# grayhong/self-diagnosing-gan

Measured on AMD Instinct MI355X. Metric: images/sec (G+D step), higher is better.
Workload: dtype f32

## Files before the change

include/diagan_hip.h:

```cpp
#ifndef DIAGAN_HIP_H
#define DIAGAN_HIP_H
#include <stdint.h>
#ifdef __cplusplus
extern "C" {
#endif

#define DIAGAN_OK 0
#define DIAGAN_EINVAL (-1)
#define DIAGAN_EHIP (-2)
#define DIAGAN_EUNSUP (-3)

const char* diagan_last_error(void);
int diagan_abi_version(void);
const char* diagan_target_arch(void);


int diagan_ldr_scores_f64(const double* rec, int T, int64_t N, int64_t row_stride, double* ldr,
                          double* ldrd, double* ldrv, double* ldrm, const double* t_vals, int n_t,
                          double* conf, double floor_val, double ratio, void* workspace,
                          void* stream);

int diagan_ldr_scores_f32(const float* rec, int T, int64_t N, int64_t row_stride, float* ldr,
                          float* ldrd, float* ldrv, float* ldrm, const float* t_vals, int n_t,
                          float* conf, float floor_val, float ratio, void* workspace, void* stream);

int diagan_logit_scatter(const float* logit, const int64_t* idx, int64_t n, void* rec_row,
                         int64_t N, int out_is_f64, int* oob_counter, void* stream);



int diagan_conv_gemm(const float* x, const float* w, float* y, const float* bias,
                     const float* residual, int res_relu, const float* mask_src, float mask_slope,
                     const float* pro_scale, const float* pro_shift, int pro_mode, float out_scale,
                     const float* scale0, const float* scale1, int scale_split,
                     int B, int Hi, int Wi, int Ci, int Ho, int Wo, int Co, int R, int S, int sy,
                     int dr, int off, int up, int Kp, int tile_cfg, float* splitk_ws, int64_t splitk_ws_floats,
                     float* stat_partials, int pro_group_rows, void* stream);
int diagan_conv_gemm_pick_ksplit(int M, int Co, int Kp, int cfg);

int diagan_conv3x3_co4_supported(int Ci, int Co, int R, int S, int sy, int dr, int off, int up);
int diagan_conv3x3_co4(const float* x, const float* w, float* y, const float* bias, const float* residual,
                       const float* pro_scale, const float* pro_shift, int pro_mode, int B, int H, int W, int Ci,
                       int dr, int off, int Kp, int group_imgs, void* stream);

int diagan_conv3x3_ci4_supported(int Ci, int Co, int R, int S, int sy, int dr, int off, int up);
int diagan_conv3x3_ci4(const float* x, const float* w, float* y, const float* bias, float out_scale, const float* scale0,
                       const float* scale1, int scale_split, int B, int H, int W, int Co, int Kp, void* stream);

int diagan_conv3x3_co4_wgrad_supported(int Ci, int Co, int R, int S, int sy, int dr, int off, int up);
int diagan_conv3x3_co4_wgrad_splits(int B, int H);
int diagan_conv3x3_co4_wgrad(const float* dy, const float* x, float* slab, int64_t slab_stride, int64_t bias_off,
                             const float* pro_scale, const float* pro_shift, int pro_mode, int B, int H, int W,
                             int Ci, int Kp, void* stream);

int diagan_conv_gemm_pick_cfg(int M, int Co, int Kp, int allow_split);
int diagan_conv_gemm_tile_rows(int cfg);
int diagan_conv_gemm_tile_cols(int cfg);
int diagan_conv_wino_supported(int Hi, int Wi, int Ci, int Ho, int Wo, int Co, int R, int S, int sy, int dr, int off,
                               int up);
int diagan_conv_wino_pool_supported(int B, int Hi, int Wi, int Ci, int Ho, int Wo, int Co, int R, int S, int sy, int dr,
                                    int off, int up, int pro_mode, int64_t ws_floats);
int diagan_conv_wino_unpool_supported(int B, int Hi, int Wi, int Ci, int Ho, int Wo, int Co, int R, int S, int sy, int dr,
                                      int off, int up, int64_t ws_floats);
int diagan_conv_gemm_set_wino(int mode);
int diagan_conv_gemm_get_wino(void);
int diagan_conv_gemm_set_wino4(int mode);
int diagan_conv_gemm_set_wino4x(int mode);
int diagan_conv_gemm_get_wino4x(void);
int diagan_conv_gemm_set_splitk_fused(int mode);
int diagan_conv_gemm_set_splitk_tickets(int* buf, int64_t slots);
typedef struct diagan_conv_opts {
  int32_t wino, wino4, wino4x, gemm_x3, gemm_x3b, splitk_fused, force_ksplit, tune;
  int32_t* tickets;
  int64_t ticket_slots;
} diagan_conv_opts;
int diagan_conv_gemm_next_opts(const diagan_conv_opts* opts);
int diagan_conv_gemm_pending_opts(diagan_conv_opts* opts);
int diagan_conv_gemm_last_cfg(void);
int diagan_conv_gemm_set_x3(int mode);
int diagan_conv_gemm_get_x3(void);
int diagan_conv_gemm_set_x3b(int mode);
int diagan_conv_gemm_get_x3b(void);
int diagan_conv_gemm_set_x3_pieces(int n);
int diagan_conv_gemm_get_x3_pieces(void);
int diagan_conv_gemm_x3b_force_form(int form);
int diagan_conv_gemm_out_map(int mul, int offy, int offx, int y0, int y1, int x0, int x1, int OH, int OW);
int diagan_conv_gemm_final_cfg(int B, int Hi, int Wi, int Ci, int Ho, int Wo, int Co, int R, int S, int sy, int dr, int off, int up,
                               int Kp, int allow_split, int64_t ws_floats, int pro_group_rows, int pro_mode, int plain_epilogue,
                               int want_stats);
int diagan_conv_wino4_pool_used(int B, int Ho, int Wo, int Ci, int Co, int64_t ws_floats);
int diagan_conv_wino4_upin_supported(int B, int Hi, int Wi, int Ci, int Ho, int Wo, int Co, int R, int S, int sy, int dr,
                                     int off, int up, int64_t ws_floats, int pro_group_rows);
int diagan_conv_gemm_weights_hint(const float* u, int kind, int flip, float scale);
int diagan_conv_gemm_last_weight_format(int* kind, int* flip, float* scale, int64_t* floats, int64_t* launches);
int64_t diagan_wino_weight_blocks(int Co, int Ci);
int diagan_wino_weights_batched(const void* jobs, int n, int blocks, void* stream);
int diagan_conv_gemm_pick_cfg_geom(int B, int Hi, int Wi, int Ci, int Ho, int Wo, int Co, int R, int S, int sy, int dr,
                                   int off, int up, int Kp, int allow_split, int64_t ws_floats);
int diagan_conv_gemm_pick_cfg_grouped(int B, int Hi, int Wi, int Ci, int Ho, int Wo, int Co, int R, int S, int sy, int dr,
                                      int off, int up, int Kp, int allow_split, int64_t ws_floats, int pro_group_rows);
int diagan_conv_gemm_set_stamp_buffer(unsigned long long* buf, int64_t slots);
int diagan_conv_gemm_tune(int force_ksplit, int flags, int lds_delta_bytes);

int diagan_conv_wgrad(const float* dy, const float* x, float* slab, int splits, int segments, int64_t slab_stride,
                      int64_t bias_off, const float* pro_scale, const float* pro_shift, int pro_mode, int B, int Hi, int Wi, int Ci, int Ho,
                      int Wo, int Co, int R, int S, int sy, int dr, int off, int up, int Kp,
                      void* stream);
int diagan_conv_wgrad_splits(int M, int Co, int Kp);
typedef struct {
  const float* dy;
  const float* x;
  float* slab;
  const float* pro_scale;
  const float* pro_shift;
  int64_t slab_stride, bias_off;
  int32_t splits, segments, pro_mode, B, Hi, Wi, Ci, Ho, Wo, Co, R, S, sy, dr, off, up, Kp, pad_;
} diagan_wgrad_job;
int diagan_conv_wgrad_batched(const diagan_wgrad_job* jobs, int n, void* stream);
int diagan_conv_wgrad_batch_max(void);
int diagan_conv_wgrad_batch_class(int Hi, int Wi, int Ci, int Ho, int Wo, int Co, int R, int S, int sy, int dr, int off, int up,
                                  int Kp, int pro_mode);
int diagan_conv_wgrad_uses_wino(int Hi, int Wi, int Ci, int Ho, int Wo, int Co, int R, int S, int sy, int dr, int off,
                                int up, int Kp);
int diagan_conv_wgrad_splits_geom(int B, int Hi, int Wi, int Ci, int Ho, int Wo, int Co, int R, int S, int sy, int dr,
                                  int off, int up, int Kp);
int diagan_conv_wgrad_uses_x3(int B, int Hi, int Wi, int Ci, int Ho, int Wo, int Co, int R, int S, int sy, int dr, int off,
                              int up, int Kp, int pro_mode, int64_t bias_off);
int diagan_conv_wgrad_set_x3(int on);

typedef struct {
  float* slab[2];
  const float* u[2];
  const float* v[2];
  const float* state[2];
  double* partials[2];
  float* grad;
  const float* W;
  int64_t stride;
  int splits, n_elem, n_w, Kp;
  int nctx, first_block;
} diagan_wgrad_layer;
int diagan_wgrad_finish_batched(const void* table_dev, int n_layers, int64_t total_blocks, int any_sn, void* stream);
int diagan_wgrad_finish_block_elems(int splits);

int diagan_wgrad_reduce(const float* slab, int splits, int64_t n_elem, float* out, int accumulate,
                        const float* w, double* dot_partials, void* stream);


int diagan_sn_power_iter(const float* W, float* u_buffer, float* sigma_buffer, float* u_out,
                         float* v_out, float* state, float* work, int Co, int Kp, float eps,
                         int update_buffers, void* stream);

typedef struct {
  const float* W;
  float* u_buf;
  float* sigma_buf;
  float* u_out;
  float* v_out;
  float* state;
  float* work;
  float* Wf;
  float* Wd;
  int Co, Ci, RS, Kp, Kd, pad;
} diagan_sn_layer;
int diagan_sn_prepare_batched(const void* table_dev, int n_layers, int max_Co, int max_Ci, int max_RS,
                              int max_Kp, float eps, int update_buffers, int write_wd, void* stream);
int diagan_pack_batched(const void* table_dev, int n_layers, int max_Co, int max_Ci, int max_RS, int write_wd,
                        void* stream);

int diagan_pack_weights(const float* W, const float* inv_sigma, float* Wf, float* Wd, int Co, int Ci,
                        int RS, int Kp, int Kd, void* stream);
int diagan_pack_oihw(const float* w, float scale, float* Wf, float* Wd, int Co_src, int Ci_src, int R, int S, int Co, int Ci, int Kp,
                     int Kd, void* stream);
int diagan_unpack_oihw(const float* gWp, float scale, float* gw, int Co_src, int Ci_src, int R, int S, int Ci, int Kp, void* stream);
int diagan_parity_weights(const float* w, float* buf, float* gw, int n, int R, int S, int C, int Kp, const int* kp, const int* off,
                          int adjoint, void* stream);


int diagan_sn_grad_fix(const float* G, const double* dot_partials, int nparts, const float* u,
                       const float* v, const float* state, float* grad, int Co, int Kp,
                       int accumulate, void* stream);


int diagan_nchw_to_nhwc(const float* src, float* dst, int B, int C, int H, int W, int Cp, void* stream);
int diagan_nhwc_to_nchw(const float* src, float* dst, int B, int C, int H, int W, int Cp, void* stream);

int diagan_tanh_fwd(const float* x, float* y, int64_t n, void* stream);
int diagan_tanh_bwd(const float* y, const float* g, float* gx, int64_t n, void* stream);

int64_t diagan_colred_workspace(int64_t M, int C);

int diagan_bn_stats(const float* x, int64_t M, int C, const float* gamma, const float* beta, float eps,
                    float momentum, float* running_mean, float* running_var, int training,
                    float* mean_out, float* invstd_out, float* scale_out, float* shift_out,
                    void* workspace, void* stream);
int diagan_bn_stats_grouped(const float* x, int64_t M, int C, int groups, const float* gamma, const float* beta, float eps,
                            float momentum, float* running_mean, float* running_var, float* mean_out, float* invstd_out,
                            float* scale_out, float* shift_out, void* workspace, void* stream);

int diagan_bn_stats_fused(const float* partials, int tiles, int64_t M, int C, const float* gamma, const float* beta,
                          float eps, float momentum, float* running_mean, float* running_var, float* mean_out,
                          float* invstd_out, float* scale_out, float* shift_out, int groups, double* workspace,
                          int64_t workspace_doubles, void* stream);
int diagan_bn_stats_fused_splits(int tiles, int C, int groups);

int diagan_bn_bwd(const float* g, const float* x, int64_t M, int C, const float* scale, const float* shift,
                  const float* mean, const float* invstd, int batch_stats, int relu, float slope,
                  const float* drop, float drop_scale, float* dgamma, float* dbeta,
                  int accumulate_param_grads, const float* residual, float* dx, float* coef,
                  void* workspace, void* stream);

int diagan_colsum(const float* x, int64_t M, int C, float* out, int accumulate, void* workspace, void* stream);

int diagan_upsample2x(const float* x, float* out, int B, int H, int W, int C, int pro_mode,
                      const float* scale, const float* shift, int group_imgs, void* stream);
int diagan_upsample2x_bwd(const float* g, float* out, int B, int H, int W, int C, const float* residual,
                          void* stream);

int diagan_avgpool2(const float* x, float* out, int B, int H, int W, int C, const float* residual, int relu_in,
                    void* stream);
int diagan_boxsum2(const float* x, float* out, int B, int H, int W, int C, int relu_in, void* stream);
int diagan_avgpool2_bwd(const float* g, float* out, int B, int H, int W, int C, const float* residual,
                        void* stream);

int diagan_head_fwd(const float* x, const float* w, const float* inv_sigma, const float* inv_sigma1, int split_b,
                    const float* bias, float* pooled, float* logit, int B, int HW, int C, void* stream);
int diagan_head_bwd(const float* dlogit, const float* w, const float* inv_sigma, const float* inv_sigma1, int split_b,
                    const float* x, const float* pooled, float* gx, float* G, double* dot, float* dbias,
                    int accumulate_bias, int B, int HW, int C, void* stream);

int diagan_act_fwd(const float* x, const float* scale, const float* shift, float slope, const float* drop, float drop_scale,
                   float* out, int64_t M, int C, void* stream);
int diagan_act_bwd(const float* g, const float* x, float slope, const float* drop, float drop_scale, float* out, int64_t n,
                   void* stream);
int diagan_linear1_fwd(const float* x, const float* w, const float* bias, float* logit, int B, int C, void* stream);
int diagan_linear1_wgrad(const float* dlogit, const float* x, float* dw, float* dbias, int B, int C, void* stream);
int diagan_linear1_bwd_input(const float* dlogit, const float* w, float* gx, int B, int C, void* stream);

int diagan_add(const float* a, const float* b, float* out, int64_t n, void* stream);


int diagan_loss_dis(const float* out_real, int n_real, const float* out_fake, int n_fake, int loss_type,
                    int gold, float* d_real, float* d_fake, float* out3, void* stream);
int diagan_loss_gen(const float* out_fake, int n, int k, int loss_type, float* d_fake, float* out1, void* stream);

int diagan_adam_step(float* p, const float* g, float* m, float* v, int64_t n, float lr, float beta1,
                     float beta2, float eps, float bias_correction1, float bias_correction2_sqrt, float grad_scale,
                     void* stream);
int diagan_adam_step_dev(float* p, const float* g, float* m, float* v, int64_t n, const float* hyper8, void* stream);

typedef struct diagan_ctx diagan_ctx;
int diagan_comm_unique_id(void* id128);
int diagan_ctx_create(diagan_ctx** out, const void* id128, int rank, int world, int device);
int diagan_ctx_destroy(diagan_ctx* ctx);
int diagan_ctx_rank(const diagan_ctx* ctx);
int diagan_ctx_world(const diagan_ctx* ctx);
int diagan_allreduce_grads(diagan_ctx* ctx, float* slab, int64_t n, void* stream);
int diagan_allgather_logits(diagan_ctx* ctx, const void* send, void* recv, int64_t n_per_rank, int elem_bytes,
                            void* stream);


int diagan_fused_bias_act(const float* x, const float* bias, const float* refer, float* out, int64_t n,
                          int64_t step_b, int size_b, int act, int grad, float alpha, float scale, void* stream);

int diagan_styled_bias_act(const float* x, const float* demod, const float* noise, const float* strength,
                           const float* bias, float* out, int B, int P, int C, int noise_per_image, float alpha,
                           float scale, void* stream);

int diagan_rowdot_chunks(int B, int P);
int diagan_rowdot(const float* a, const float* b, float* out, float* workspace, int B, int P, int C, void* stream);
int diagan_styled_bias_act_bwd(const float* gy, const float* y, const float* x, const float* demod, const float* noise,
                               float* gx, float* work_d, float* work_b, float* work_s, int B, int P, int C,
                               int noise_per_image, float alpha, float scale, void* stream);
int diagan_styled_bias_act_bwd_finish(const float* work_d, const float* work_b, const float* work_s, float* gd, float* gb, float* gs, int B,
                                      int P, int C, void* stream);

int diagan_small_linear_fwd(const float* x, const float* W, const float* bias, float* out, int B, int K, int C, float scale, float bias_mul,
                            void* stream);
int diagan_small_linear_bwd(const float* g, const float* x, const float* W, float* gW, float* gbias, float* gx, int B, int K, int C,
                            float scale, float bias_mul, void* stream);
int diagan_demod_fwd(const float* s, const float* w, float* d, float* wsq, int B, int Ci, int Co, int taps, float scale2, float eps,
                     void* stream);
int diagan_demod_bwd(const float* gd, const float* d, const float* s, const float* w, const float* wsq, float* gw, float* gs, int B, int Ci,
                     int Co, int taps, float scale2, void* stream);

int diagan_styled_bias_act_mod(const float* x, const float* demod, const float* noise, const float* strength, const float* bias,
                               const float* post, float* out, float* out_mod, int B, int P, int C, int noise_per_image, float alpha,
                               float scale, void* stream);
int diagan_styled_bias_act_mod_bwd(const float* gy, const float* gmod, const float* post, const float* y, const float* x,
                                   const float* demod, const float* noise, float* gx, float* work_d, float* work_b, float* work_s,
                                   float* work_p, int B, int P, int C, int noise_per_image, float alpha, float scale, void* stream);

int diagan_torgb_fwd(const float* x, const float* s, const float* w, const float* bias, float* out, int B, int P, int C, void* stream);
int diagan_torgb_bwd(const float* gy, const float* x, const float* s, const float* w, float* gx, float* work, float* gs, float* gw, int B,
                     int P, int C, void* stream);
int diagan_fromrgb_fwd(const float* x, const float* w, const float* bias, float* y, int B, int P, int C, float wscale, float alpha,
                       float scale, void* stream);
int diagan_fromrgb_bwd(const float* gy, const float* y, const float* x, const float* w, float* gx, float* work, int B, int P, int C,
                       float wscale, float alpha, float scale, void* stream);
int diagan_bias_act_fir(const float* input, const float* bias, const float* kernel, float* out, int major, int in_h, int in_w, int minor,
                        int kernel_h, int kernel_w, int pad_x0, int pad_x1, int pad_y0, int pad_y1, float alpha, float scale,
                        void* stream);
int diagan_bias_act_gate_bwd(const float* gy, const float* z, const float* bias, float* gx, float* work_b, int B, int P, int C,
                             float alpha, float scale, void* stream);
int diagan_fir_gate_bwd(const float* g, const float* kernel, const float* ref, const float* bias, float* gz, float* work_b, int major,
                        int in_h, int in_w, int minor, int kernel_h, int kernel_w, int pad_x0, int pad_x1, int pad_y0, int pad_y1,
                        float alpha, float scale, void* stream);
int diagan_upfirdn2d_add(const float* input, const float* kernel, const float* addend, float* out, int major, int in_h, int in_w, int minor,
                         int kernel_h, int kernel_w, int up_x, int up_y, int down_x, int down_y, int pad_x0, int pad_x1, int pad_y0,
                         int pad_y1, void* stream);
int diagan_bias_act_add(const float* x, const float* bias, const float* addend, float* out, int64_t n, int C, float alpha, float scale,
                        void* stream);
int diagan_fir_styled_act(const float* input, const float* kernel, float* out, int major, int in_h, int in_w, int minor, int kernel_h,
                          int kernel_w, int pad_x0, int pad_x1, int pad_y0, int pad_y1, const float* demod, const float* noise,
                          const float* strength, const float* bias, const float* post, int noise_per_image, float alpha, float scale,
                          void* stream);


int diagan_upfirdn2d(const float* input, const float* kernel, float* out, int major, int in_h, int in_w, int minor,
                     int kernel_h, int kernel_w, int up_x, int up_y, int down_x, int down_y, int pad_x0, int pad_x1,
                     int pad_y0, int pad_y1, int* out_h, int* out_w, void* stream);

int diagan_row_sqnorm(const float* x, float* out, int N, int D, int ld, void* stream);
int diagan_kth_smallest_rows(const float* T, const float* row_add, int rows, int cols, int ld, int k, float* out,
                             void* stream);
int diagan_any_lt_rows(const float* T, const float* row_add, const float* thr_col, const float* thr_row, int rows,
                       int cols, int ld, float* out, void* stream);
int diagan_any_lt_cols(const float* T, const float* row_add, const float* thr_col, const float* thr_row, int rows,
                       int cols, int ld, float* out, void* stream);

int diagan_gemm_f64(const double* A, const double* B, double* C, int M, int N, int K, int lda, int ldb, int ldc, int trans_a,
                    double alpha, double beta, double diag, double* trace_part, void* stream);
int diagan_gemm_f64_tile(void);
int diagan_sum_f64(const double* x, int64_t n, int square, double* out, void* stream);
int diagan_trace_f64(const double* S, int D, int ld, double* out, void* stream);
int diagan_sym_f64(double* S, int D, int ld, double scale, void* stream);
int diagan_scale_diag_f64(const double* src, double* dst, int D, int ld, double alpha, double d, void* stream);
int diagan_fid_term(const double* mu1, const double* mu2, const double* S1, const double* S2, int D, int ld, double* out,
                    void* stream);
int diagan_feat_colsum_chunks(int N);
int diagan_feat_moments(const void* x, int x_f64, int N, int D, int ld, double* mask, double* part, double* count, double* mean,
                        void* stream);
int diagan_feat_center(const void* x, int x_f64, const double* mask, const double* mean, int N, int D, int ld, double* xc, int ldc,
                       void* stream);
int diagan_moments_merge(double* n_run, double* mean_run, double* m2_run, int ld, const double* n_b, const double* mean_b,
                         const double* m2_b, int ldb, int D, void* stream);


int diagan_augment_params(void);
int diagan_augment_workspace(int B, int H, int W, int pad_x1, int pad_x2, int pad_y1, int pad_y2, int backward, int64_t* bytes);
int diagan_augment_forward(const float* img, const double* params, int B, int H, int W, int pad_x1, int pad_x2, int pad_y1,
                           int pad_y2, float* out, void* workspace, void* stream);
int diagan_augment_backward(const float* gout, const double* params, int B, int H, int W, int pad_x1, int pad_x2, int pad_y1,
                            int pad_y2, float* gimg, void* workspace, void* stream);

#ifdef __cplusplus
}
#endif
#endif
```

self-diagnosing-gan_amd/csrc/conv_common.h:

```cpp
#pragma once
#include "common.h"

namespace diagan {

typedef float f32x16 __attribute__((ext_vector_type(16)));
typedef float f32x4 __attribute__((ext_vector_type(4)));

enum ProMode : int {
  PRO_NONE = 0,
  PRO_RELU = 1,
  PRO_AFFINE_RELU = 2,
  PRO_LRELU = 3,
  PRO_AFFINE = 4,
  PRO_BOX = 5,
  PRO_BOX_RELU = 6,
};

struct ConvGeom {
  int B, Hi, Wi, Ci;
  int Ho, Wo, Co;
  int R, S;
  int sy, dr, off, up;
  int K;
  int Kp;
};

__device__ __forceinline__ f32x4 apply_pro(f32x4 v, int mode, const float* __restrict__ scale,
                                           const float* __restrict__ shift, int c) {
  if (mode == PRO_NONE) return v;
  if (mode == PRO_AFFINE_RELU || mode == PRO_AFFINE) {
    const f32x4 sc = *reinterpret_cast<const f32x4*>(scale + c);
    const f32x4 sh = *reinterpret_cast<const f32x4*>(shift + c);
    v = v * sc + sh;
    if (mode == PRO_AFFINE) return v;
  }
  if (mode == PRO_LRELU) {
#pragma unroll
    for (int e = 0; e < 4; ++e) v[e] = v[e] > 0.f ? v[e] : 0.2f * v[e];
    return v;
  }
#pragma unroll
  for (int e = 0; e < 4; ++e) v[e] = fmaxf(v[e], 0.f);
  return v;
}

struct FastDiv {
  unsigned mul, shift, d;
};
static inline FastDiv make_fastdiv(unsigned d) {
  FastDiv f;
  f.d = d;
  if (d == 1) { f.mul = 0; f.shift = 0; return f; }
  unsigned l = 0;
  while ((1u << l) < d) ++l;
  const unsigned long long m = ((1ull << (32 + l)) + d - 1) / d;
  f.mul = (unsigned)(m - (1ull << 32));
  f.shift = l;
  return f;
}
__device__ __forceinline__ f32x4 residual_up2(const float* __restrict__ r, int b, int oy, int ox, int H, int W, int C, int c) {
  const int jy = oy >> 1, jx = ox >> 1;
  const int y0 = (oy & 1) ? jy : max(jy - 1, 0), y1 = (oy & 1) ? min(jy + 1, H - 1) : jy;
  const int x0 = (ox & 1) ? jx : max(jx - 1, 0), x1 = (ox & 1) ? min(jx + 1, W - 1) : jx;
  const float wy0 = (oy & 1) ? 0.75f : 0.25f, wx0 = (ox & 1) ? 0.75f : 0.25f;
  const float wy1 = 1.f - wy0, wx1 = 1.f - wx0;
  const float* base = r + (long)b * H * W * C + c;
  const f32x4 a00 = *reinterpret_cast<const f32x4*>(base + ((long)y0 * W + x0) * C);
  const f32x4 a01 = *reinterpret_cast<const f32x4*>(base + ((long)y0 * W + x1) * C);
  const f32x4 a10 = *reinterpret_cast<const f32x4*>(base + ((long)y1 * W + x0) * C);
  const f32x4 a11 = *reinterpret_cast<const f32x4*>(base + ((long)y1 * W + x1) * C);
  const f32x4 top = wx0 * a00 + wx1 * a01;
  const f32x4 bot = wx0 * a10 + wx1 * a11;
  return wy0 * top + wy1 * bot;
}

__device__ __forceinline__ unsigned fdiv(unsigned n, const FastDiv& f) {
  if (f.d == 1) return n;
  const unsigned t = __umulhi(n, f.mul);
  return (t + ((n - t) >> 1)) >> (f.shift - 1);
}

struct OutMap {
  int mul, offy, offx, y0, y1, x0, x1, OH, OW;
};

struct ConvGemmArgs {
  const float* x;
  const float* w;
  float* y;
  const float* bias;
  const float* residual;
  const float* mask_src;
  const float* pro_scale;
  const float* pro_shift;
  int pro_group_rows;
  float mask_slope;
  float out_scale;
  const float* scale0;
  const float* scale1;
  int scale_split;
  float* stat_partials;
  float* slab;
  int* tickets;
  int ksplit;
  int res_relu;
  int res_up;
  int pro_mode;
  int M;
  ConvGeom g;
  FastDiv dWo, dHo;
  unsigned long long* stamps;
  int tune;
};

struct WgradArgs {
  const float* dy;
  const float* x;
  float* slab;
  const float* pro_scale;
  const float* pro_shift;
  int pro_mode;
  int M;
  int steps_per_split;
  int seg_steps;
  int splits_per_seg;
  long slab_stride;
  long bias_off;
  ConvGeom g;
  FastDiv dWo, dHo;
  int adv_b, adv_y, adv_x;
  int lgW, lgHW;
  int tiles;
  int same;
};

constexpr int WG_BATCH_MAX = 8;
struct WgradBatchArgs {
  int n;
  int blk0[WG_BATCH_MAX];
  int cnt[WG_BATCH_MAX];
  WgradArgs a[WG_BATCH_MAX];
};

constexpr int WT_LDS_F4 = 9 * 8 * 65;
__device__ __forceinline__ bool wino_stage_taps(const float* __restrict__ w, int co0, int c0, int Co, int Ci, int Kp, int flip,
                                                f32x4* __restrict__ sg, f32x4 (&g)[3][3]) {
  const int tid = threadIdx.x;
  {
    const int col = tid >> 3, q = tid & 7;
    const bool ok = co0 + col < Co && c0 + q * 4 < Ci;
    const float* src = w + (long)(co0 + col) * Kp + c0 + q * 4;
    f32x4 v[9];
#pragma unroll
    for (int t = 0; t < 9; ++t) v[t] = ok ? *reinterpret_cast<const f32x4*>(src + (flip ? 8 - t : t) * Ci) : f32x4{0.f, 0.f, 0.f, 0.f};
#pragma unroll
    for (int t = 0; t < 9; ++t) sg[(t * 8 + q) * 65 + col] = v[t];
  }
  __syncthreads();
  const int col = tid & 63, q = tid >> 6;
#pragma unroll
  for (int t = 0; t < 9; ++t) g[t / 3][t % 3] = sg[(t * 8 + q) * 65 + col];
  return c0 + q * 4 < Ci;
}

enum WinoKind : int { WK_F2 = 2, WK_F4 = 40, WK_F4_POOL = 41, WK_F4X = 42, WK_F4X_POOL = 43, WK_GX3 = 50 };
struct WinoJob {
  const float* w;
  float* u;
  int Co, Ci, Kp, kind, flip, blk0;
  float scale;
  int pad_;
};
const float* wino_weights_ready(int kind, int flip, float scale, long floats);

__device__ __forceinline__ int xcd_remap(int bid, int nwg) {
  const int q = nwg >> 3, r = nwg & 7, xcd = bid & 7, slot = bid >> 3;
  return (xcd < r ? xcd * (q + 1) : r * (q + 1) + (xcd - r) * q) + slot;
}

}
```

self-diagnosing-gan_amd/csrc/conv_gemm.hip:

```cpp
#include "conv_common.h"
#include <type_traits>
#include <stdlib.h>
#include <string.h>

extern "C" int diagan_conv_gemm_tile_rows(int cfg);
extern "C" int diagan_conv_gemm_tile_cols(int cfg);
extern "C" int diagan_conv_gemm_pick_ksplit(int M, int Co, int Kp, int cfg);
extern "C" int diagan_conv_gemm_pick_cfg_geom(int B, int Hi, int Wi, int Ci, int Ho, int Wo, int Co, int R, int S, int sy,
                                              int dr, int off, int up, int Kp, int allow_split, int64_t ws_floats);
extern "C" int diagan_conv_gemm_pick_cfg_grouped(int B, int Hi, int Wi, int Ci, int Ho, int Wo, int Co, int R, int S, int sy,
                                                 int dr, int off, int up, int Kp, int allow_split, int64_t ws_floats,
                                                 int pro_group_rows);
extern "C" int diagan_conv_wino_supported(int Hi, int Wi, int Ci, int Ho, int Wo, int Co, int R, int S, int sy, int dr,
                                          int off, int up);

namespace diagan {
int launch_gemm_x3(const ConvGemmArgs& a, float* ws, hipStream_t st);
bool gemm_x3_geom_ok(const ConvGemmArgs& a);
long gemm_x3_ws_floats(int Co, int Kp);
int launch_gemm_x3b(const ConvGemmArgs& a, const OutMap& map, float* ws, hipStream_t st);
bool gemm_x3b_geom_ok(const ConvGemmArgs& a);
long gemm_x3b_ws_floats(int Co, int Kp);
void gemm_x3b_force_form(int form);
int launch_wino(ConvGemmArgs a, float* ws, hipStream_t st);
long wino_ws_floats(int Co, int Ci);
int wino_ksplit(int B, int Ho, int Wo, int Ci, int Co, int allow_split, long ws_floats, int min_wgs);
int launch_wino4(ConvGemmArgs a, float* ws, hipStream_t st);
long wino4_ws_floats(int Co, int Ci);
bool wino4_geom_ok(int Ho, int Wo, int Ci);
int wino4_ksplit(int B, int Ho, int Wo, int Ci, int Co, int allow_split, long ws_floats);
bool wino4_pool_ok(int B, int Ho, int Wo, int Ci, int Co, long ws_floats, bool force);
int launch_wino4_pool(ConvGemmArgs a, float* ws, hipStream_t st);
int launch_wino4_unpool(ConvGemmArgs a, float* ws, hipStream_t st);
bool wino4_upin_ok(int B, int Ho, int Wo, int Ci, int Co, long ws_floats, bool force);
int launch_wino_weights_batched(const WinoJob* jobs, int n, int blocks, hipStream_t st);
int launch_wino4_upin(ConvGemmArgs a, float* ws, hipStream_t st);
void wino4_set_x3(int mode);
int wino4_get_x3();
int launch_wino_pool(ConvGemmArgs a, float* ws, hipStream_t st);
int launch_wino_unpool(ConvGemmArgs a, float* ws, hipStream_t st);
int wino_pool_ksplit(int B, int Ho, int Wo, int Ci, int Co, long slab_floats, int min_wgs);


template <int BM, int BN, int WM, int WN, int BK = 32, int PRO = -1, bool STAMP = false, bool FP = false, int KG = 1>
__global__ __launch_bounds__(256 * KG) void conv_gemm_kernel(const ConvGemmArgs a) {
  constexpr int CH = BK / 4;
  constexpr int RP = 256 / CH;
  constexpr int TM = BM / WM / 32, TN = BN / WN / 32;
  constexpr int AJ = BM / RP, BJ = BN / RP;
  auto swz = [](int row, int q) {
    return BK == 64 ? (q ^ (row & 15)) : BK == 32 ? (q ^ ((row >> 1) & 7)) : (q ^ ((row >> 2) & 3));
  };
  static_assert(WM * WN == 4, "4 waves");
  extern __shared__ __attribute__((aligned(16))) float smem_all[];
  constexpr int STAGE_FLOATS = 2 * (BM + BN) * BK;
  const int kg = KG > 1 ? __builtin_amdgcn_readfirstlane((int)threadIdx.x >> 8) : 0;
  float* const smem = smem_all + kg * STAGE_FLOATS;
  float* As = smem;
  float* Bs = smem + 2 * BM * BK;

  unsigned long long st_t[6] = {0, 0, 0, 0, 0, 0}, st_r0 = 0;
  auto stamp = [&](int i) {
    if constexpr (STAMP) {
      __builtin_amdgcn_sched_barrier(0);
      st_t[i] = __builtin_amdgcn_s_memtime();
      __builtin_amdgcn_sched_barrier(0);
    }
  };
  if constexpr (STAMP) st_r0 = __builtin_amdgcn_s_memrealtime();
  if (a.tune & 1) __builtin_amdgcn_s_setprio(3);
  stamp(0);
  const ConvGeom& g = a.g;
  const int pro_mode = PRO >= 0 ? PRO : a.pro_mode;
  const int tid = KG > 1 ? (threadIdx.x & 255) : threadIdx.x, lane = tid & 63, wave = tid >> 6;
  const int wm = wave / WN, wn = wave % WN;
  const int tiles_n = (g.Co + BN - 1) / BN;
  const int nwg = gridDim.x;
  const int tile = xcd_remap(blockIdx.x, nwg);
  const int m0 = (tile / tiles_n) * BM, n0 = (tile % tiles_n) * BN;

  const int lrow = tid / CH, lq = tid % CH;
  const int ush = g.up >> 1, upm = g.up - 1;
  const int pstep = (g.Ci * 4) >> ush;
  int base[AJ];
  unsigned vmask[AJ];
#pragma unroll
  for (int j = 0; j < AJ; ++j) {
    const int m = m0 + lrow + RP * j;
    base[j] = 0;
    vmask[j] = 0;
    if (m < a.M) {
      const unsigned t = fdiv((unsigned)m, a.dWo);
      const int ox = m - (int)t * g.Wo;
      const unsigned b = fdiv(t, a.dHo);
      const int oy = (int)t - (int)b * g.Ho;
      const int iy0 = oy * g.sy + g.off, ix0 = ox * g.sy + g.off;
      base[j] = (int)b * g.Hi * g.Wi * g.Ci * 4 + (iy0 * g.Wi + ix0) * pstep;
      unsigned mk = 0;
      if (g.up == 1) {
        const int ylo = g.dr > 0 ? max(0, -iy0) : max(0, iy0 - g.Hi + 1);
        const int yhi = g.dr > 0 ? min(g.R - 1, g.Hi - 1 - iy0) : min(g.R - 1, iy0);
        const int xlo = g.dr > 0 ? max(0, -ix0) : max(0, ix0 - g.Wi + 1);
        const int xhi = g.dr > 0 ? min(g.S - 1, g.Wi - 1 - ix0) : min(g.S - 1, ix0);
        if (yhi >= ylo) mk |= (2u << yhi) - (1u << ylo);
        if (xhi >= xlo) mk |= ((2u << xhi) - (1u << xlo)) << 16;
      } else {
        for (int r = 0; r < g.R; ++r) {
          const int yn = iy0 + r * g.dr;
          if (yn >= 0 && (yn & upm) == 0 && (yn >> ush) < g.Hi) mk |= 1u << r;
        }
        for (int q = 0; q < g.S; ++q) {
          const int xn = ix0 + q * g.dr;
          if (xn >= 0 && (xn & upm) == 0 && (xn >> ush) < g.Wi) mk |= 0x10000u << q;
        }
      }
      vmask[j] = mk;
    }
  }
  const int nk_all = g.Kp / BK;
  const int k_per = (nk_all + a.ksplit * KG - 1) / (a.ksplit * KG);
  const int k_begin = min((int)(blockIdx.y * KG + kg) * k_per, nk_all), k_end = min(k_begin + k_per, nk_all);
  int kc, kr, ks;
  {
    const int kflat = k_begin * BK + lq * 4, tap = kflat / g.Ci;
    kc = kflat - tap * g.Ci;
    kr = tap / g.S;
    ks = tap - kr * g.S;
  }
  const int rowstep = g.dr * g.Wi * pstep, colstep = g.dr * pstep;

  const __amdgpu_buffer_rsrc_t xsrc = __builtin_amdgcn_make_buffer_rsrc(
      const_cast<float*>(a.x), 0, (int)((unsigned)g.B * g.Hi * g.Wi * g.Ci * 4u), 0x00020000);
  const __amdgpu_buffer_rsrc_t wsrc = __builtin_amdgcn_make_buffer_rsrc(
      const_cast<float*>(a.w), 0, (int)((unsigned)g.Co * g.Kp * 4u), 0x00020000);
  const bool affine = pro_mode == PRO_AFFINE_RELU || pro_mode == PRO_AFFINE;
  const int pro_group_off = a.pro_group_rows > 0 ? (m0 / a.pro_group_rows) * g.Ci : 0;
  unsigned wbase[BJ];
#pragma unroll
  for (int j = 0; j < BJ; ++j) wbase[j] = ((unsigned)(n0 + lrow + RP * j) * g.Kp + lq * 4) * 4u;

  f32x4 ra[AJ], rb[BJ], psc = {1.f, 1.f, 1.f, 1.f}, psh = {0.f, 0.f, 0.f, 0.f};
  unsigned a_ok = 0;

  const bool ut = (g.Ci % BK) == 0;
  int ukr = 0, uks = 0, ukc = 0;
  unsigned avo[AJ], tap_ok = 0;
  auto tap_setup = [&]() {
    const int toff = ukr * rowstep + uks * colstep + lq * 16;
    const int r_ = min(ukr, 15), s_ = 16 + uks;
    tap_ok = 0;
#pragma unroll
    for (int j = 0; j < AJ; ++j) {
      const unsigned okb = (vmask[j] >> r_) & (vmask[j] >> s_) & 1u;
      avo[j] = (unsigned)(base[j] + toff) | ((okb ^ 1u) << 31);
      tap_ok |= okb << j;
    }
  };
  if (ut) {
    const int kflat0 = k_begin * BK, tap0 = kflat0 / g.Ci;
    ukc = kflat0 - tap0 * g.Ci;
    ukr = tap0 / g.S;
    uks = tap0 - ukr * g.S;
    tap_setup();
  }
  const float* const pro_sc_lane = a.pro_scale ? a.pro_scale + pro_group_off + lq * 4 : nullptr;
  const float* const pro_sh_lane = a.pro_shift ? a.pro_shift + pro_group_off + lq * 4 : nullptr;

  int tapoff = 0, krs = 0, kss = 0;
  auto load_piece = [&](int kk, int p, auto utc) {
    if constexpr (decltype(utc)::value) {
      if (p == 0) {
        a_ok = tap_ok;
        if (affine) {
          psc = *reinterpret_cast<const f32x4*>(pro_sc_lane + ukc);
          psh = *reinterpret_cast<const f32x4*>(pro_sh_lane + ukc);
        }
      }
      if (p < AJ) {
        ra[p] = __builtin_bit_cast(f32x4, __builtin_amdgcn_raw_buffer_load_b128(xsrc, avo[p], ukc * 4, 0));
      } else {
        rb[p - AJ] = __builtin_bit_cast(f32x4, __builtin_amdgcn_raw_buffer_load_b128(wsrc, wbase[p - AJ], kk * (BK * 4), 0));
      }
      if (p == AJ + BJ - 1) {
        ukc += BK;
        if (ukc >= g.Ci) {
          ukc = 0;
          if (++uks == g.S) {
            uks = 0;
            ++ukr;
          }
          tap_setup();
        }
      }
      return;
    }
    if (p == 0) {
      tapoff = kr * rowstep + ks * colstep + kc * 4;
      krs = min(kr, 15);
      kss = 16 + ks;
      a_ok = 0;
      if (affine) {
        const int kcs = min(kc, g.Ci - 4);
        psc = *reinterpret_cast<const f32x4*>(a.pro_scale + pro_group_off + kcs);
        psh = *reinterpret_cast<const f32x4*>(a.pro_shift + pro_group_off + kcs);
      }
    }
    if (p < AJ) {
      const int j = p;
      const unsigned okb = (vmask[j] >> krs) & (vmask[j] >> kss) & 1u;
      const unsigned off = (unsigned)(base[j] + tapoff) | ((okb ^ 1u) << 31);
      ra[j] = __builtin_bit_cast(f32x4, __builtin_amdgcn_raw_buffer_load_b128(xsrc, off, 0, 0));
      a_ok |= okb << j;
    } else {
      const int j = p - AJ;
      rb[j] = __builtin_bit_cast(f32x4, __builtin_amdgcn_raw_buffer_load_b128(wsrc, wbase[j] + (unsigned)kk * (BK * 4u), 0, 0));
    }
    if (p == AJ + BJ - 1) {
      kc += BK;
      if (g.Ci >= BK) {
        const bool w = kc >= g.Ci;
        kc -= w ? g.Ci : 0;
        ks += w ? 1 : 0;
        const bool r = ks == g.S;
        ks = r ? 0 : ks;
        kr += r ? 1 : 0;
      } else {
        const int kflat = (kk + 1) * BK + lq * 4, tap = kflat / g.Ci;
        kc = kflat - tap * g.Ci;
        kr = tap / g.S;
        ks = tap - kr * g.S;
      }
    }
  };
  auto load_tiles = [&](int kk) {
    if (ut) {
#pragma unroll
      for (int p = 0; p < AJ + BJ; ++p) load_piece(kk, p, std::true_type{});
    } else {
#pragma unroll
      for (int p = 0; p < AJ + BJ; ++p) load_piece(kk, p, std::false_type{});
    }
  };
  auto store_piece = [&](int buf, int p) {
    if (p < AJ) {
      const int j = p;
      const int row = lrow + RP * j;
      f32x4 v = ra[j];
      if (pro_mode != PRO_NONE) {
        if (affine) v = v * psc + psh;
        if (pro_mode == PRO_LRELU) {
#pragma unroll
          for (int e = 0; e < 4; ++e) v[e] = v[e] > 0.f ? v[e] : 0.2f * v[e];
        } else if (pro_mode != PRO_AFFINE) {
#pragma unroll
          for (int e = 0; e < 4; ++e) v[e] = fmaxf(v[e], 0.f);
        }
        if (affine) {
          const float keep = (float)((a_ok >> j) & 1u);
          v *= keep;
        }
      }
      *reinterpret_cast<f32x4*>(As + buf * BM * BK + row * BK + (swz(row, lq) << 2)) = v;
    } else {
      const int j = p - AJ;
      const int row = lrow + RP * j;
      *reinterpret_cast<f32x4*>(Bs + buf * BN * BK + row * BK + (swz(row, lq) << 2)) = rb[j];
    }
  };
  auto store_tiles = [&](int buf) {
#pragma unroll
    for (int p = 0; p < AJ + BJ; ++p) store_piece(buf, p);
  };

  f32x16 acc[TM][TN];
#pragma unroll
  for (int i = 0; i < TM; ++i)
#pragma unroll
    for (int j = 0; j < TN; ++j)
#pragma unroll
      for (int e = 0; e < 16; ++e) acc[i][j][e] = 0.f;

  const int fi = lane & 31, fh = lane >> 5;
  int fao[BK / 8], fbo[BK / 8];
#pragma unroll
  for (int u = 0; u < BK / 8; ++u) {
    const int ra_ = wm * (TM * 32) + fi, rb_ = wn * (TN * 32) + fi;
    fao[u] = ra_ * BK + (swz(ra_, 2 * u + fh) << 2);
    fbo[u] = 2 * BM * BK + rb_ * BK + (swz(rb_, 2 * u + fh) << 2);
  }
  const int sto = lrow * BK + (swz(lrow, lq) << 2);

  stamp(1);
  if (k_begin < k_end) {
    load_tiles(k_begin);
    store_tiles(0);
  }
  __syncthreads();

  constexpr int NE = (BK / 8) * 4, NP = AJ + BJ;
  constexpr int PPE = (2 * NP + NE - 1) / NE;
  constexpr int LE = (NP + PPE - 1) / PPE;
  static_assert(2 * LE <= NE, "load and store pieces of a tile must not share an e-step");
  auto kstep = [&](int kk, auto has_next) {
    const int cur = (kk - k_begin) & 1;
    const float* Ac = As + cur * BM * BK;
    const float* Bc = Bs + cur * BN * BK;
    f32x4 fa[2][TM], fb[2][TN];
    auto read_frags = [&](int slot, int u) {
      const int q = 2 * u + fh;
#pragma unroll
      for (int i = 0; i < TM; ++i) {
        const int row = wm * (TM * 32) + i * 32 + fi;
        fa[slot][i] = *reinterpret_cast<const f32x4*>(Ac + row * BK + (swz(row, q) << 2));
      }
#pragma unroll
      for (int j = 0; j < TN; ++j) {
        const int row = wn * (TN * 32) + j * 32 + fi;
        fb[slot][j] = *reinterpret_cast<const f32x4*>(Bc + row * BK + (swz(row, q) << 2));
      }
    };
    if constexpr (FP) read_frags(0, 0);
#pragma unroll
    for (int u = 0; u < BK / 8; ++u) {
      const int fs = FP ? (u & 1) : 0;
      if constexpr (FP) {
        if (u + 1 < BK / 8) read_frags((u + 1) & 1, u + 1);
      } else {
        read_frags(0, u);
      }
#pragma unroll
      for (int e = 0; e < 4; ++e) {
        const int es = u * 4 + e;
        if (decltype(has_next)::value && es < LE) {
#pragma unroll
          for (int pp = 0; pp < PPE; ++pp)
            if (es * PPE + pp < NP) load_piece(kk + 1, es * PPE + pp, std::false_type{});
        }
        if (decltype(has_next)::value && es >= NE - LE) {
          __builtin_amdgcn_sched_barrier(0);
#pragma unroll
          for (int pp = 0; pp < PPE; ++pp)
// ... 281 lines not shown
}
static thread_local OutMap g_map_next = {0, 0, 0, 0, 0, 0, 0, 0, 0};
struct CallOpts {
  int wino, wino4, wino4x, gemm_x3, gemm_x3b, splitk_fused, force_ksplit, tune;
  int* tickets;
  long ticket_slots;
};
static const CallOpts kNoOpts = {-1, -1, -1, -1, -1, -1, 0, -1, nullptr, 0};
static thread_local CallOpts g_opts_next = kNoOpts, g_opts_now = kNoOpts;
static thread_local int g_last_cfg = 0;
int call_opt_wino4x() { return g_opts_now.wino4x; }
static int sel_wino() {
  static const int env = getenv("DIAGAN_WINO") ? atoi(getenv("DIAGAN_WINO")) : 1;
  return g_opts_now.wino >= 0 ? g_opts_now.wino : (g_wino >= 0 ? g_wino : env);
}
static int sel_wino4() { return g_opts_now.wino4 >= 0 ? g_opts_now.wino4 : g_wino4; }
static int sel_force_ksplit() { return g_opts_now.force_ksplit > 0 ? g_opts_now.force_ksplit : g_force_ksplit; }
static bool gemm_x3_on() {
  static const int env = getenv("DIAGAN_GEMM_X3") ? atoi(getenv("DIAGAN_GEMM_X3")) : 1;
  return (g_opts_now.gemm_x3 >= 0 ? g_opts_now.gemm_x3 : (g_gemm_x3 >= 0 ? g_gemm_x3 : env)) != 0;
}
static bool gemm_x3b_on() {
  static const int env = getenv("DIAGAN_GEMM_X3B") ? atoi(getenv("DIAGAN_GEMM_X3B")) : 1;
  return (g_opts_now.gemm_x3b >= 0 ? g_opts_now.gemm_x3b : (g_gemm_x3b >= 0 ? g_gemm_x3b : env)) != 0;
}
static bool x3b_takes(const ConvGemmArgs& a, int cfg, int64_t ws_floats) {
  if (!gemm_x3b_on() || !(cfg == 1 || cfg == 3 || cfg == 5 || cfg == 7 || cfg == 8)) return false;
  const ConvGeom& g = a.g;
  return gemm_x3b_geom_ok(a) && g.Kp >= 128 && g.Co >= 64 && (long)cdiv(a.M, 128) * cdiv(g.Co, 128) >= x3b_min_tiles() &&
         (double)a.M * g.Co * g.Kp >= 4e9 && gemm_x3b_ws_floats(g.Co, g.Kp) <= ws_floats;
}
static int g_splitk_fused = -1;
static int* g_tickets = nullptr;
static long g_ticket_slots = 0;
static int* splitk_tickets(long tiles) {
  static const int env = getenv("DIAGAN_SPLITK_FUSED") ? atoi(getenv("DIAGAN_SPLITK_FUSED")) : 0;
  if (!(g_opts_now.splitk_fused >= 0 ? g_opts_now.splitk_fused : (g_splitk_fused >= 0 ? g_splitk_fused : env))) return nullptr;
  if (g_opts_now.tickets) return tiles <= g_opts_now.ticket_slots ? g_opts_now.tickets : nullptr;
  return (g_tickets && tiles <= g_ticket_slots) ? g_tickets : nullptr;
}

template <int BM, int BN, int WM, int WN, int BK, int PRO, bool STAMP = false, bool FP = false, int KG = 1>
static int launch_one(const ConvGemmArgs& a, hipStream_t st) {
  const int tiles = cdiv(a.M, BM) * cdiv(a.g.Co, BN);
  const size_t lds = (size_t)((long)((size_t)2 * KG * (BM + BN) * BK * sizeof(float)) + g_lds_delta);
  auto kern = conv_gemm_kernel<BM, BN, WM, WN, BK, PRO, STAMP, FP, KG>;
  static FuncAttrLatch latch;
  DG_LDS(latch, kern, lds);
  hipLaunchKernelGGL(kern, dim3(tiles, a.ksplit), dim3(256 * KG), lds, st, a);
  if (a.ksplit > 1) {
    long blocks = ((long)a.M * (a.g.Co / 4) + 255) / 256;
    if (blocks > 4096) blocks = 4096;
    hipLaunchKernelGGL(splitk_epilogue_kernel, dim3((int)blocks), dim3(256), 0, st, a);
  }
  return check_launch("conv_gemm");
}

template <int BM, int BN, int WM, int WN, int BK = 32, bool SPEC = false, bool FP = false, int KG = 1>
static int launch_cfg(const ConvGemmArgs& a, hipStream_t st) {
  if (a.stamps && KG > 1) return set_err(DIAGAN_EUNSUP, "conv_gemm: no stamped build of the two-group kernel");
  if (a.stamps) {
    if (a.pro_mode == PRO_NONE) return launch_one<BM, BN, WM, WN, BK, PRO_NONE, true, FP>(a, st);
    if (a.pro_mode == PRO_RELU) return launch_one<BM, BN, WM, WN, BK, PRO_RELU, true, FP>(a, st);
    return set_err(DIAGAN_EUNSUP, "conv_gemm: the stamped diagnostic kernels exist for prologue modes 0 and 1");
  }
  if (SPEC) {
    switch (a.pro_mode) {
      case PRO_NONE: return launch_one<BM, BN, WM, WN, BK, SPEC ? PRO_NONE : -1, false, FP, KG>(a, st);
      case PRO_RELU: return launch_one<BM, BN, WM, WN, BK, SPEC ? PRO_RELU : -1, false, FP, KG>(a, st);
      case PRO_AFFINE_RELU: return launch_one<BM, BN, WM, WN, BK, SPEC ? PRO_AFFINE_RELU : -1, false, FP, KG>(a, st);
      case PRO_LRELU: return launch_one<BM, BN, WM, WN, BK, SPEC ? PRO_LRELU : -1, false, FP, KG>(a, st);
      default: return launch_one<BM, BN, WM, WN, BK, SPEC ? PRO_AFFINE : -1, false, FP, KG>(a, st);
    }
  }
  return launch_one<BM, BN, WM, WN, BK, -1, false, FP, KG>(a, st);
}

}

using namespace diagan;

static bool split128_enabled() {
  static const bool on = getenv("DIAGAN_SPLIT128") && atoi(getenv("DIAGAN_SPLIT128")) > 0;
  return on;
}

DIAGAN_API int diagan_conv_gemm_pick_cfg(int M, int Co, int Kp, int allow_split) {
  const int small = 7;
  if (Kp <= 256) return small;
  const long t128 = (long)cdiv(M, 128) * cdiv(Co, 128), t64 = (long)cdiv(M, 64) * cdiv(Co, 64);
  if (split128_enabled() && allow_split && (Co & 127) == 0 && t128 <= 256 && diagan_conv_gemm_pick_ksplit(M, Co, Kp, 1) > 1) return 1;
  if (Co <= 64 && Kp >= 256) return M >= 65536 ? 5 : (M >= 32768 ? 8 : 7);
  const long s128 = 256 * 2, s64 = 256 * 4;
  const double q128 = (double)t128 / (double)(cdiv(t128, s128) * s128);
  const double q64 = (double)t64 / (double)(cdiv(t64, s64) * s64);
  const double waste128 = (double)M * Co / ((double)t128 * 128 * 128);
  const double waste64 = (double)M * Co / ((double)t64 * 64 * 64);
  const double bias = 1.08;
  if (bias * q128 * waste128 > q64 * waste64) return 1;
  static const int kg2 = getenv("DIAGAN_KG2") ? atoi(getenv("DIAGAN_KG2")) : 1;
  if (kg2 && t64 <= 256 && Kp >= 16 * 32 && diagan_conv_gemm_pick_ksplit(M, Co, Kp, small) == 1) return 14;
  return small;
}

DIAGAN_API int diagan_conv_gemm_pick_ksplit(int M, int Co, int Kp, int cfg) {
  static const int env_forced = getenv("DIAGAN_KSPLIT") ? atoi(getenv("DIAGAN_KSPLIT")) : 0;
  const int forced = sel_force_ksplit() > 0 ? sel_force_ksplit() : env_forced;
  if (forced > 0 && !(Co & 3)) return forced < Kp / 64 ? forced : (Kp / 64 > 0 ? Kp / 64 : 1);
  if (Co & 3) return 1;
  const int nk = Kp / 32;
  if (cfg == 1) {
    if (!split128_enabled()) return 1;
    const long t128 = (long)cdiv(M, 128) * cdiv(Co, 128);
    if (t128 > 256 || nk < 64) return 1;
    int s = t128 <= 128 ? 4 : 2;
    while (s > 1 && nk / s < 16) --s;
    return s;
  }
  if (cfg != 3 && cfg != 7) return 1;
  const long tiles = (long)cdiv(M, 64) * cdiv(Co, 64);
  if (nk < 16) return 1;
  if (tiles <= 320) {
    if (nk < 64) return 1;
    int s = nk / 24;
    return s > 4 ? 4 : s;
  }
  if (tiles > 512) return 1;
  long sp = 1024 / tiles;
  if (sp > nk / 8) sp = nk / 8;
  return sp < 2 ? 1 : (int)sp;
}

const float* diagan::wino_weights_ready(int kind, int flip, float scale, long floats) {
  g_fmt_last = WinoFormat{nullptr, kind, flip, scale, floats};
  if (g_hint_now.u && g_hint_now.kind == kind && g_hint_now.flip == flip && g_hint_now.scale == scale) return g_hint_now.u;
  ++g_weight_launches;
  return nullptr;
}

DIAGAN_API int diagan_conv_gemm_weights_hint(const float* u, int kind, int flip, float scale) {
  g_hint_next = WinoFormat{u, kind, flip, scale, 0};
  return DIAGAN_OK;
}
DIAGAN_API int diagan_conv_gemm_last_weight_format(int* kind, int* flip, float* scale, int64_t* floats, int64_t* launches) {
  if (kind) *kind = g_fmt_last.kind;
  if (flip) *flip = g_fmt_last.flip;
  if (scale) *scale = g_fmt_last.scale;
  if (floats) *floats = g_fmt_last.floats;
  if (launches) *launches = g_weight_launches;
  return DIAGAN_OK;
}
DIAGAN_API int64_t diagan_wino_weight_blocks(int Co, int Ci) { return (int64_t)cdiv(Ci, 32) * cdiv(Co, 64); }
DIAGAN_API int diagan_wino_weights_batched(const void* jobs, int n, int blocks, void* stream) {
  DG_REQUIRE(jobs && n > 0 && blocks > 0, "wino_weights_batched: bad job table");
  return launch_wino_weights_batched((const WinoJob*)jobs, n, blocks, (hipStream_t)stream);
}

DIAGAN_API int diagan_conv_gemm(const float* x, const float* w, float* y, const float* bias,
                                const float* residual, int res_relu, const float* mask_src, float mask_slope,
                                const float* pro_scale, const float* pro_shift, int pro_mode,
                                float out_scale, const float* scale0, const float* scale1, int scale_split,
                                int B, int Hi, int Wi, int Ci, int Ho, int Wo, int Co,
                                int R, int S, int sy, int dr, int off, int up, int Kp, int tile_cfg,
                                float* splitk_ws, int64_t splitk_ws_floats, float* stat_partials, int pro_group_rows,
                                void* stream) {
  g_hint_now = g_hint_next;
  g_hint_next = WinoFormat{nullptr, 0, 0, 0.f, 0};
  g_fmt_last = WinoFormat{nullptr, 0, 0, 0.f, 0};
  const OutMap map = g_map_next;
  g_map_next = OutMap{0, 0, 0, 0, 0, 0, 0, 0, 0};
  struct OptsScope {
    OptsScope() { g_opts_now = g_opts_next; g_opts_next = kNoOpts; }
    ~OptsScope() { g_opts_now = kNoOpts; }
  } opts_scope;
  g_last_cfg = 0;
  DG_REQUIRE(x && w && y, "conv_gemm: null tensor");
  DG_REQUIRE(B > 0 && Hi > 0 && Wi > 0 && Ho > 0 && Wo > 0 && Co > 0 && R > 0 && S > 0, "conv_gemm: bad dims");
  DG_REQUIRE(Ci > 0 && (Ci & 3) == 0, "conv_gemm: Ci=%d must be a positive multiple of 4 (pad the tensor)", Ci);
  DG_REQUIRE(up == 1 || up == 2, "conv_gemm: up=%d unsupported (1 or 2)", up);
  DG_REQUIRE(dr == 1 || dr == -1, "conv_gemm: dr must be +-1");
  DG_REQUIRE(R <= 15 && S <= 15, "conv_gemm: filter %dx%d larger than 15x15", R, S);
  DG_REQUIRE(Kp % 32 == 0 && Kp >= R * S * Ci, "conv_gemm: Kp=%d must be a multiple of 32 and >= R*S*Ci=%d", Kp, R * S * Ci);
  DG_REQUIRE(pro_mode >= 0 && pro_mode <= 4, "conv_gemm: bad pro_mode %d", pro_mode);
  DG_REQUIRE(!(pro_mode == PRO_AFFINE_RELU || pro_mode == PRO_AFFINE) || (pro_scale && pro_shift),
             "conv_gemm: affine prologue needs scale/shift");
  DG_REQUIRE((long)B * Ho * Wo * Co * 4 < (1L << 31) && (long)B * Hi * Wi * Ci * 4 < (1L << 31) &&
                 (long)Co * Kp * 4 < (1L << 31),
             "conv_gemm: tensors must be smaller than 2 GiB (32-bit buffer offsets)");
  ConvGemmArgs a;
  a.x = x; a.w = w; a.y = y; a.bias = bias; a.residual = residual; a.mask_src = mask_src;
  a.pro_scale = pro_scale; a.pro_shift = pro_shift; a.mask_slope = mask_slope; a.out_scale = out_scale;
  a.scale0 = scale0; a.scale1 = scale1; a.scale_split = scale_split;
  DG_REQUIRE(!scale0 || scale1, "conv_gemm: scale0 and scale1 must be given together");
  DG_REQUIRE(!(stat_partials && mask_src), "conv_gemm: stat_partials (forward statistics) and mask_src (backward mask) are exclusive");
  a.pro_mode = pro_mode; a.M = B * Ho * Wo; a.res_relu = res_relu & 1; a.res_up = (res_relu & 2) ? 1 : (res_relu & 4) ? 2 : 0;
  DG_REQUIRE((res_relu & ~7) == 0 && (res_relu & 6) != 6, "conv_gemm: res_relu=%d (bit 0: relu(residual), bit 1: half-resolution residual, "
             "up-sampled; bit 2: half-resolution residual, un-pooled)", res_relu);
  DG_REQUIRE(a.res_up != 1 || (residual && !(Ho & 1) && !(Wo & 1) && !mask_src && !a.res_relu),
             "conv_gemm: a half-resolution residual needs the tensor, even Ho / Wo, no backward mask and no ReLU on it");
  DG_REQUIRE(a.res_up != 2 || (residual && !(Ho & 1) && !(Wo & 1) && !a.res_relu && !stat_partials),
             "conv_gemm: an un-pooled half-resolution residual needs the tensor, even Ho / Wo, no ReLU on it, no statistics");
  a.g = ConvGeom{B, Hi, Wi, Ci, Ho, Wo, Co, R, S, sy, dr, off, up, R * S * Ci, Kp};
  a.dWo = make_fastdiv((unsigned)Wo);
  a.dHo = make_fastdiv((unsigned)Ho);
  a.stat_partials = stat_partials;
  a.pro_group_rows = pro_group_rows;
  hipStream_t st = (hipStream_t)stream;
  int cfg = tile_cfg != 0 ? tile_cfg
                          : diagan_conv_gemm_pick_cfg_grouped(B, Hi, Wi, Ci, Ho, Wo, Co, R, S, sy, dr, off, up, Kp,
                                                              (splitk_ws && !stat_partials) ? 1 : 0,
                                                              splitk_ws ? splitk_ws_floats : 0, pro_group_rows);
  if (tile_cfg == 0 && splitk_ws && x3b_takes(a, cfg, splitk_ws_floats)) cfg = 17;
  g_last_cfg = cfg;
  if (map.mul != 0) {
    DG_REQUIRE(map.mul > 0 && map.OH > 0 && map.OW > 0 && map.y0 >= 0 && map.x0 >= 0 && map.y1 <= Ho && map.x1 <= Wo &&
                   map.offy >= 0 && map.offx >= 0 && (map.y1 <= map.y0 || map.mul * (map.y1 - 1 - map.y0) + map.offy < map.OH) &&
                   (map.x1 <= map.x0 || map.mul * (map.x1 - 1 - map.x0) + map.offx < map.OW) &&
                   (long)B * map.OH * map.OW * Co * 4 < (1L << 31),
               "conv_gemm: output map (mul %d, off %d/%d, window [%d,%d) x [%d,%d), target %d x %d) does not fit", map.mul, map.offy,
               map.offx, map.y0, map.y1, map.x0, map.x1, map.OH, map.OW);
    DG_REQUIRE(cfg == 17, "conv_gemm: an output map is written by the split-operand kernel only (tile_cfg 17; ask "
               "diagan_conv_gemm_final_cfg first)");
  }
  const int bm = diagan_conv_gemm_tile_rows(cfg);
  DG_REQUIRE(bm > 0, "conv_gemm: unknown tile_cfg %d (0 = auto, 1 = 128x128, 3 = 64x64, 5 = 256x64, 7 = 64x64 with fragment "
             "prefetch, 8 = 128x64 with fragment prefetch, 9 = Winograd F(2x2,3x3), 11 / 12 = Winograd + average pool and its data-gradient, 13 = Winograd F(4x4,3x3), 15 = the same on the bilinear x2 of a half-resolution input; 2, 4, 6, 10 were retired)", tile_cfg);
  DG_REQUIRE(pro_group_rows >= 0 && (pro_group_rows == 0 || (pro_group_rows % bm == 0 && a.M % pro_group_rows == 0)),
             "conv_gemm: pro_group_rows=%d must be a multiple of the %d-row tile and divide M=%d", pro_group_rows, bm, a.M);
  a.slab = splitk_ws;
  a.tickets = nullptr;
  a.ksplit = 1;
  a.tune = g_opts_now.tune >= 0 ? g_opts_now.tune : (g_tune_flags >= 0 ? g_tune_flags : kDefaultTune);
  a.stamps = nullptr;
  if (g_stamps) {
    const long wgs = (long)cdiv(a.M, bm) * cdiv(Co, diagan_conv_gemm_tile_cols(cfg)) * 16;
    DG_REQUIRE(wgs <= g_stamp_slots, "conv_gemm: stamp buffer has %ld slots, this launch may need %ld", g_stamp_slots, wgs);
    a.stamps = g_stamps;
  }
  if (splitk_ws && !stat_partials) {
    const int ks = diagan_conv_gemm_pick_ksplit(a.M, Co, Kp, cfg);
    if (ks > 1 && (int64_t)ks * a.M * Co <= splitk_ws_floats) a.ksplit = ks;
  }
  if (cfg == 11) {
    DG_REQUIRE(diagan_conv_wino_supported(Hi, Wi, Ci, Ho, Wo, Co, R, S, sy, dr, off, up) && dr == 1 && Co % 64 == 0 &&
                   (pro_mode == PRO_NONE || pro_mode == PRO_RELU) && !mask_src && !stat_partials && !a.res_up && pro_group_rows == 0,
               "conv_gemm: tile_cfg 11 (Winograd + average pool) needs a forward 3x3 / stride 1 / pad 1 geometry with even H, W, "
               "Ci %% 8 == 0, Co %% 64 == 0, prologue none / ReLU, no mask, statistics or half-resolution residual");
    if (sel_wino4() != 0 && splitk_ws && wino4_pool_ok(B, Ho, Wo, Ci, Co, (long)splitk_ws_floats, sel_wino4() == 2)) {
      a.ksplit = 1;
      return launch_wino4_pool(a, splitk_ws, st);
    }
    const long wfl = wino_ws_floats(Co, Ci);
    DG_REQUIRE(splitk_ws && splitk_ws_floats >= wfl, "conv_gemm: tile_cfg 11 needs %ld floats of workspace for the transformed weights", wfl);
    int ks = wino_pool_ksplit(B, Ho, Wo, Ci, Co, (long)splitk_ws_floats - wfl, 192);
    if (ks < 1) ks = 1;
    a.ksplit = ks;
    a.slab = splitk_ws + wfl;
    int rc = launch_wino_pool(a, splitk_ws, st);
    if (rc == DIAGAN_OK && ks > 1) {
      ConvGemmArgs e = a;
      e.M = B * (Ho >> 1) * (Wo >> 1);
      e.scale_split = a.scale_split >> 2;
      e.out_scale = a.out_scale;
      long blocks = ((long)e.M * (Co / 4) + 255) / 256;
      if (blocks > 4096) blocks = 4096;
      hipLaunchKernelGGL(splitk_epilogue_kernel, dim3((int)blocks), dim3(256), 0, st, e);
      rc = check_launch("conv_wino_pool split-K epilogue");
    }
    return rc;
  }
  if (cfg == 12) {
    DG_REQUIRE(diagan_conv_wino_supported(Hi, Wi, Ci, Ho, Wo, Co, R, S, sy, dr, off, up) && dr == -1 && Co % 64 == 0 &&
                   pro_mode == PRO_NONE && !stat_partials && !a.res_up && pro_group_rows == 0,
               "conv_gemm: tile_cfg 12 (data-gradient through an average pool, Winograd) needs the data-gradient geometry of a "
               "3x3 / stride 1 / pad 1 layer with even H, W, Ci %% 8 == 0, Co %% 64 == 0, no prologue, statistics or half-resolution residual");
    if (sel_wino4() != 0 && splitk_ws && wino4_pool_ok(B, Ho, Wo, Ci, Co, (long)splitk_ws_floats, sel_wino4() == 2)) {
      a.ksplit = 1;
      return launch_wino4_unpool(a, splitk_ws, st);
    }
    const long wfl = wino_ws_floats(Co, Ci);
    DG_REQUIRE(splitk_ws && splitk_ws_floats >= wfl, "conv_gemm: tile_cfg 12 needs %ld floats of workspace for the transformed weights", wfl);
    long slab_tiles = ((long)splitk_ws_floats - wfl) / 4;
    int ks = wino_pool_ksplit(B, Ho, Wo, Ci, Co, slab_tiles, 192);
    if (ks < 1) ks = 1;
    a.ksplit = ks;
    a.slab = splitk_ws + wfl;
    int rc = launch_wino_unpool(a, splitk_ws, st);
    if (rc == DIAGAN_OK && ks > 1) {
      long blocks = ((long)a.M * (Co / 4) + 255) / 256;
      if (blocks > 4096) blocks = 4096;
      hipLaunchKernelGGL(splitk_epilogue_kernel, dim3((int)blocks), dim3(256), 0, st, a);
      rc = check_launch("conv_wino_unpool split-K epilogue");
    }
    return rc;
  }
  if (cfg == 15) {
    DG_REQUIRE(diagan_conv_wino_supported(Hi, Wi, Ci, Ho, Wo, Co, R, S, sy, dr, off, up) && dr == 1 && wino4_geom_ok(Ho, Wo, Ci) &&
                   !mask_src && (pro_group_rows == 0 || pro_group_rows % 512 == 0),
               "conv_gemm: tile_cfg 15 (Winograd F(4x4,3x3) on an up-sampled input) needs a forward 3x3 / stride 1 / pad 1 geometry, "
               "H and W multiples of 4, Ci %% 8 == 0, no backward mask, prologue groups of whole 512-row tiles");
    const long wfl = wino4_ws_floats(Co, Ci);
    DG_REQUIRE(splitk_ws && splitk_ws_floats >= wfl, "conv_gemm: tile_cfg 15 needs %ld floats of workspace for the transformed weights", wfl);
    a.ksplit = 1;
    return launch_wino4_upin(a, splitk_ws, st);
  }
  if (cfg == 13) {
    DG_REQUIRE(diagan_conv_wino_supported(Hi, Wi, Ci, Ho, Wo, Co, R, S, sy, dr, off, up) && wino4_geom_ok(Ho, Wo, Ci),
               "conv_gemm: tile_cfg 13 (Winograd F(4x4,3x3)) needs a 3x3 / stride 1 / pad 1 geometry, H and W multiples of 4, Ci %% 8 == 0");
    const long wfl = wino4_ws_floats(Co, Ci);
    DG_REQUIRE(splitk_ws && splitk_ws_floats >= wfl, "conv_gemm: tile_cfg 13 needs %ld floats of workspace for the transformed weights", wfl);
    int ks = 1;
    if (tile_cfg == 0 && !stat_partials) {
      ks = wino4_ksplit(B, Ho, Wo, Ci, Co, 1, (long)splitk_ws_floats);
      if (ks < 1) ks = 1;
    } else if (sel_force_ksplit() > 1 && !stat_partials && wfl + (long)sel_force_ksplit() * a.M * Co <= splitk_ws_floats && Ci / 8 / sel_force_ksplit() >= 1) {
      ks = sel_force_ksplit();
    }
    a.ksplit = ks;
    a.slab = splitk_ws + wfl;
    int rc = launch_wino4(a, splitk_ws, st);
    if (rc == DIAGAN_OK && ks > 1) {
      long blocks = ((long)a.M * (Co / 4) + 255) / 256;
      if (blocks > 4096) blocks = 4096;
      hipLaunchKernelGGL(splitk_epilogue_kernel, dim3((int)blocks), dim3(256), 0, st, a);
      rc = check_launch("conv_wino4 split-K epilogue");
    }
    return rc;
  }
  if (cfg == 9) {
    DG_REQUIRE(diagan_conv_wino_supported(Hi, Wi, Ci, Ho, Wo, Co, R, S, sy, dr, off, up),
               "conv_gemm: tile_cfg 9 (Winograd F(2x2,3x3)) needs a 3x3 / stride 1 / pad 1 geometry, even H and W, Ci %% 8 == 0");
    DG_REQUIRE(splitk_ws && splitk_ws_floats >= wino_ws_floats(Co, Ci),
               "conv_gemm: tile_cfg 9 needs %ld floats of workspace for the transformed weights", wino_ws_floats(Co, Ci));
    const long wfl = wino_ws_floats(Co, Ci);
    int ks = 1;
    if (tile_cfg == 0 && !stat_partials) {
      ks = wino_ksplit(B, Ho, Wo, Ci, Co, 1, (long)splitk_ws_floats, 192);
      if (ks < 1) ks = 1;
    } else if (sel_force_ksplit() > 1 && !stat_partials && wfl + (long)sel_force_ksplit() * a.M * Co <= splitk_ws_floats &&
               Ci / 16 / sel_force_ksplit() >= 1) {
      ks = sel_force_ksplit();
    }
    a.ksplit = ks;
    a.slab = splitk_ws + wfl;
    if (ks > 1) a.tickets = splitk_tickets((long)cdiv(a.M / 4, 64) * cdiv(Co, 64));
    int rc = launch_wino(a, splitk_ws, st);
    if (rc == DIAGAN_OK && ks > 1 && !a.tickets) {
      long blocks = ((long)a.M * (Co / 4) + 255) / 256;
      if (blocks > 4096) blocks = 4096;
      hipLaunchKernelGGL(splitk_epilogue_kernel, dim3((int)blocks), dim3(256), 0, st, a);
      rc = check_launch("conv_wino split-K epilogue");
    }
    return rc;
  }
  DG_REQUIRE(!a.res_up, "conv_gemm: a half-resolution residual is added by the Winograd kernel only (tile_cfg 9; ask "
             "diagan_conv_gemm_pick_cfg_geom first)");
  if (cfg == 16 || (cfg == 14 && tile_cfg == 0 && R == 3 && S == 3 && gemm_x3_on() && gemm_x3_geom_ok(a) && splitk_ws &&
                    gemm_x3_ws_floats(Co, Kp) <= splitk_ws_floats)) {
    DG_REQUIRE(gemm_x3_geom_ok(a) && splitk_ws && gemm_x3_ws_floats(Co, Kp) <= splitk_ws_floats,
               "conv_gemm: tile_cfg 16 (split-operand implicit GEMM) needs stride 1, no up-sampling, Ci %% 32 == 0, an even number of "
               "32-channel K-steps, Kp == R*S*Ci, prologue none / ReLU, no statistics, and %ld floats of workspace", gemm_x3_ws_floats(Co, Kp));
    a.ksplit = 1;
    g_last_cfg = 16;
    return launch_gemm_x3(a, splitk_ws, st);
  }
  if (cfg == 17) {
    DG_REQUIRE(gemm_x3b_geom_ok(a) && splitk_ws && gemm_x3b_ws_floats(Co, Kp) <= splitk_ws_floats,
               "conv_gemm: tile_cfg 17 (split-operand implicit GEMM, 128 x 128 tiles) needs a gather without up-sampling, Ci %% 32 == 0, "
               "Kp == R*S*Ci, prologue none / ReLU / leaky ReLU, a plain epilogue (out_scale, bias, residual) and %ld floats of workspace",
               gemm_x3b_ws_floats(Co, Kp));
    a.ksplit = 1;
    return launch_gemm_x3b(a, map, splitk_ws, st);
  }
  switch (cfg) {
    case 1: return launch_cfg<128, 128, 2, 2, 32, true>(a, st);
    case 3: return launch_cfg<64, 64, 2, 2, 32, true>(a, st);
    case 5: return launch_cfg<256, 64, 4, 1, 32, true>(a, st);
    case 7: return launch_cfg<64, 64, 2, 2, 32, true, true>(a, st);
    case 8: return launch_cfg<128, 64, 2, 2, 32, true, true>(a, st);
    case 14: return launch_cfg<64, 64, 2, 2, 32, true, true, 2>(a, st);
    default: return set_err(DIAGAN_EINVAL, "conv_gemm: unknown tile_cfg %d", tile_cfg);
  }
}

DIAGAN_API int diagan_conv_gemm_tile_rows(int cfg) {
  switch (cfg) { case 1: case 8: case 17: return 128; case 3: case 7: case 14: case 16: return 64; case 5: case 9: case 11: case 12: return 256; case 13: case 15: return 512; default: return 0; }
}
DIAGAN_API int diagan_conv_gemm_tile_cols(int cfg) {
  switch (cfg) { case 1: case 11: case 12: case 17: return 128; case 3: case 5: case 7: case 8: case 9: case 13: case 14: case 15: case 16: return 64; default: return 0; }
}

DIAGAN_API int diagan_conv_wino_supported(int Hi, int Wi, int Ci, int Ho, int Wo, int Co, int R, int S, int sy, int dr,
                                          int off, int up) {
  return R == 3 && S == 3 && sy == 1 && up == 1 && ((dr == 1 && off == -1) || (dr == -1 && off == 1)) && Hi == Ho &&
         Wi == Wo && !(Ho & 1) && !(Wo & 1) && (Ci & 7) == 0 && (Co & 3) == 0;
}

DIAGAN_API int diagan_conv_wino_pool_supported(int B, int Hi, int Wi, int Ci, int Ho, int Wo, int Co, int R, int S, int sy,
                                               int dr, int off, int up, int pro_mode, int64_t ws_floats) {
  static const int pool_env = getenv("DIAGAN_WINO_POOL") ? atoi(getenv("DIAGAN_WINO_POOL")) : 1;
  const int wino = sel_wino();
  if (!wino || !pool_env || dr != 1 || Co % 64 != 0 || Ci < 16 || !(pro_mode == PRO_NONE || pro_mode == PRO_RELU)) return 0;
  if (!diagan_conv_wino_supported(Hi, Wi, Ci, Ho, Wo, Co, R, S, sy, dr, off, up)) return 0;
  const long wfl = wino_ws_floats(Co, Ci);
  if (ws_floats < wfl) return 0;
  return wino_pool_ksplit(B, Ho, Wo, Ci, Co, (long)ws_floats - wfl, 192) > 0 ? 1 : 0;
}

DIAGAN_API int diagan_conv_wino_unpool_supported(int B, int Hi, int Wi, int Ci, int Ho, int Wo, int Co, int R, int S, int sy,
                                                 int dr, int off, int up, int64_t ws_floats) {
  static const int pool_env = getenv("DIAGAN_WINO_POOL") ? atoi(getenv("DIAGAN_WINO_POOL")) : 1;
  const int wino = sel_wino();
  if (!wino || !pool_env || dr != -1 || Co % 64 != 0 || Ci < 16) return 0;
  if (!diagan_conv_wino_supported(Hi, Wi, Ci, Ho, Wo, Co, R, S, sy, dr, off, up)) return 0;
  const long wfl = wino_ws_floats(Co, Ci);
  if (ws_floats < wfl) return 0;
  return wino_pool_ksplit(B, Ho, Wo, Ci, Co, ((long)ws_floats - wfl) / 4, 192) > 0 ? 1 : 0;
}

static int pick_cfg_geom_impl(int B, int Hi, int Wi, int Ci, int Ho, int Wo, int Co, int R, int S, int sy, int dr, int off,
                              int up, int Kp, int allow_split, int64_t ws_floats, bool allow_w4);
DIAGAN_API int diagan_conv_gemm_pick_cfg_geom(int B, int Hi, int Wi, int Ci, int Ho, int Wo, int Co, int R, int S, int sy,
                                              int dr, int off, int up, int Kp, int allow_split, int64_t ws_floats) {
  return pick_cfg_geom_impl(B, Hi, Wi, Ci, Ho, Wo, Co, R, S, sy, dr, off, up, Kp, allow_split, ws_floats, true);
}
static int pick_cfg_geom_impl(int B, int Hi, int Wi, int Ci, int Ho, int Wo, int Co, int R, int S, int sy, int dr, int off,
                              int up, int Kp, int allow_split, int64_t ws_floats, bool allow_w4) {
  const int wino = sel_wino();
  static const int min_wgs = getenv("DIAGAN_WINO_MIN_WGS") ? atoi(getenv("DIAGAN_WINO_MIN_WGS")) : 192;
  if (wino && diagan_conv_wino_supported(Hi, Wi, Ci, Ho, Wo, Co, R, S, sy, dr, off, up) &&
      ws_floats >= wino_ws_floats(Co, Ci) && Ci >= 16) {
    static const int wsplit = getenv("DIAGAN_WINO_SPLIT") ? atoi(getenv("DIAGAN_WINO_SPLIT")) : 1;
    static const int w4_env = getenv("DIAGAN_WINO4") ? atoi(getenv("DIAGAN_WINO4")) : 1;
    static const int w4_min_ci = getenv("DIAGAN_WINO4_MIN_CI") ? atoi(getenv("DIAGAN_WINO4_MIN_CI")) : 64;
    if (allow_w4 && w4_env && sel_wino4() != 0 && wino4_geom_ok(Ho, Wo, Ci) && Ci >= w4_min_ci && ws_floats >= wino4_ws_floats(Co, Ci) &&
        wino4_ksplit(B, Ho, Wo, Ci, Co, wsplit ? allow_split : 0, (long)ws_floats) > 0)
      return 13;
    if (wino_ksplit(B, Ho, Wo, Ci, Co, wsplit ? allow_split : 0, (long)ws_floats, min_wgs) > 0) return 9;
  }
  return diagan_conv_gemm_pick_cfg(B * Ho * Wo, Co, Kp, allow_split);
}

DIAGAN_API int diagan_conv_gemm_pick_cfg_grouped(int B, int Hi, int Wi, int Ci, int Ho, int Wo, int Co, int R, int S, int sy,
                                                 int dr, int off, int up, int Kp, int allow_split, int64_t ws_floats,
                                                 int pro_group_rows) {
  int cfg = diagan_conv_gemm_pick_cfg_geom(B, Hi, Wi, Ci, Ho, Wo, Co, R, S, sy, dr, off, up, Kp, allow_split, ws_floats);
  if (cfg == 13 && pro_group_rows > 0 && pro_group_rows % 512 != 0)
    cfg = pick_cfg_geom_impl(B, Hi, Wi, Ci, Ho, Wo, Co, R, S, sy, dr, off, up, Kp, allow_split, ws_floats, false);
  if (pro_group_rows > 0 && pro_group_rows % diagan_conv_gemm_tile_rows(cfg) != 0) {
    cfg = diagan_conv_gemm_pick_cfg(B * Ho * Wo, Co, Kp, allow_split);
    if (pro_group_rows % diagan_conv_gemm_tile_rows(cfg) != 0) cfg = 3;
  }
  return cfg;
}

DIAGAN_API int diagan_conv_gemm_get_wino(void) { return g_wino; }
DIAGAN_API int diagan_conv_gemm_set_wino(int mode) {
  DG_REQUIRE(mode >= -1 && mode <= 1, "set_wino: -1, 0 or 1");
  g_wino = mode;
  return DIAGAN_OK;
}

DIAGAN_API int diagan_conv_wino4_pool_used(int B, int Ho, int Wo, int Ci, int Co, int64_t ws_floats) {
  return sel_wino4() != 0 && wino4_pool_ok(B, Ho, Wo, Ci, Co, (long)ws_floats, sel_wino4() == 2) ? 1 : 0;
}

DIAGAN_API int diagan_conv_wino4_upin_supported(int B, int Hi, int Wi, int Ci, int Ho, int Wo, int Co, int R, int S, int sy, int dr,
                                                int off, int up, int64_t ws_floats, int pro_group_rows) {
  const int wino = sel_wino();
  if (!wino || sel_wino4() == 0 || dr != 1 || !diagan_conv_wino_supported(Hi, Wi, Ci, Ho, Wo, Co, R, S, sy, dr, off, up)) return 0;
  if (pro_group_rows > 0 && pro_group_rows % 512 != 0) return 0;
  return wino4_upin_ok(B, Ho, Wo, Ci, Co, (long)ws_floats, sel_wino4() == 2) ? 1 : 0;
}

DIAGAN_API int diagan_conv_gemm_set_wino4(int mode) {
  DG_REQUIRE(mode >= -1 && mode <= 2, "set_wino4: -1, 0, 1 or 2 (2: also the pooled launches of any size -- tests)");
  g_wino4 = mode;
  return DIAGAN_OK;
}

DIAGAN_API int diagan_conv_gemm_set_wino4x(int mode) {
  DG_REQUIRE(mode >= -1 && mode <= 1, "set_wino4x: -1, 0 or 1");
  wino4_set_x3(mode);
  return DIAGAN_OK;
}
DIAGAN_API int diagan_conv_gemm_get_wino4x(void) { return wino4_get_x3(); }
DIAGAN_API int diagan_conv_gemm_set_x3(int mode) {
  DG_REQUIRE(mode >= -1 && mode <= 1, "set_x3: -1, 0 or 1");
  g_gemm_x3 = mode;
  return DIAGAN_OK;
}
DIAGAN_API int diagan_conv_gemm_get_x3(void) { return gemm_x3_on() ? 1 : 0; }
DIAGAN_API int diagan_conv_gemm_set_x3b(int mode) {
  DG_REQUIRE(mode >= -1 && mode <= 1, "set_x3b: -1, 0 or 1");
  g_gemm_x3b = mode;
  return DIAGAN_OK;
}
DIAGAN_API int diagan_conv_gemm_get_x3b(void) { return gemm_x3b_on() ? 1 : 0; }
namespace diagan { void x3_set_pieces(int n); int x3_pieces(); }
DIAGAN_API int diagan_conv_gemm_set_x3_pieces(int n) {
  diagan::x3_set_pieces(n);
  return DIAGAN_OK;
}
DIAGAN_API int diagan_conv_gemm_get_x3_pieces(void) { return diagan::x3_pieces(); }
DIAGAN_API int diagan_conv_gemm_x3b_force_form(int form) {
  DG_REQUIRE(form >= 0 && form <= 2, "x3b_force_form: 0, 1 or 2");
  gemm_x3b_force_form(form);
  return DIAGAN_OK;
}
DIAGAN_API int diagan_conv_gemm_out_map(int mul, int offy, int offx, int y0, int y1, int x0, int x1, int OH, int OW) {
  g_map_next = OutMap{mul, offy, offx, y0, y1, x0, x1, OH, OW};
  return DIAGAN_OK;
}
DIAGAN_API int diagan_conv_gemm_final_cfg(int B, int Hi, int Wi, int Ci, int Ho, int Wo, int Co, int R, int S, int sy, int dr,
                                          int off, int up, int Kp, int allow_split, int64_t ws_floats, int pro_group_rows,
                                          int pro_mode, int plain_epilogue, int want_stats) {
  struct PendingScope {
    CallOpts saved;
    PendingScope() : saved(g_opts_now) { g_opts_now = g_opts_next; }
    ~PendingScope() { g_opts_now = saved; }
  } pending_scope;
  int cfg = diagan_conv_gemm_pick_cfg_grouped(B, Hi, Wi, Ci, Ho, Wo, Co, R, S, sy, dr, off, up, Kp, allow_split, ws_floats,
                                              pro_group_rows);
  ConvGemmArgs a = {};
  a.pro_mode = pro_mode;
  a.M = B * Ho * Wo;
  a.g = ConvGeom{B, Hi, Wi, Ci, Ho, Wo, Co, R, S, sy, dr, off, up, R * S * Ci, Kp};
  a.pro_group_rows = pro_group_rows;
  static float dummy;
  a.stat_partials = want_stats ? &dummy : nullptr;
  a.mask_src = plain_epilogue ? nullptr : &dummy;
  if (ws_floats > 0 && x3b_takes(a, cfg, ws_floats)) return 17;
  a.mask_src = nullptr;
  if (cfg == 14 && R == 3 && S == 3 && gemm_x3_on() && gemm_x3_geom_ok(a) && ws_floats >= gemm_x3_ws_floats(Co, Kp)) return 16;
  return cfg;
}
DIAGAN_API int diagan_conv_gemm_set_splitk_fused(int mode) {
  DG_REQUIRE(mode >= -1 && mode <= 1, "set_splitk_fused: -1, 0 or 1");
  g_splitk_fused = mode;
  return DIAGAN_OK;
}
DIAGAN_API int diagan_conv_gemm_set_splitk_tickets(int* buf, int64_t slots) {
  DG_REQUIRE((buf && slots > 0) || (!buf && slots == 0), "set_splitk_tickets: a buffer with its slot count, or NULL and 0");
  g_tickets = buf;
  g_ticket_slots = (long)slots;
  return DIAGAN_OK;
}
struct diagan_conv_opts {
  int32_t wino, wino4, wino4x, gemm_x3, gemm_x3b, splitk_fused, force_ksplit, tune;
  int32_t* tickets;
  int64_t ticket_slots;
};
static_assert(sizeof(diagan_conv_opts) == 48, "diagan_conv_opts layout");
DIAGAN_API int diagan_conv_gemm_next_opts(const diagan_conv_opts* o) {
  if (!o) {
    g_opts_next = kNoOpts;
    return DIAGAN_OK;
  }
  DG_REQUIRE(o->wino >= -1 && o->wino <= 1 && o->wino4 >= -1 && o->wino4 <= 2 && o->wino4x >= -1 && o->wino4x <= 1 && o->gemm_x3 >= -1 &&
                 o->gemm_x3 <= 1 && o->gemm_x3b >= -1 && o->gemm_x3b <= 1 && o->splitk_fused >= -1 && o->splitk_fused <= 1 &&
                 o->force_ksplit >= 0 && o->tune >= -1,
             "conv_gemm_next_opts: a field out of range (-1 = process default; force_ksplit 0 = the launch policy)");
  DG_REQUIRE(!o->tickets || o->ticket_slots > 0, "conv_gemm_next_opts: a ticket buffer needs its slot count");
  g_opts_next = CallOpts{o->wino, o->wino4, o->wino4x, o->gemm_x3, o->gemm_x3b, o->splitk_fused, o->force_ksplit, o->tune, o->tickets,
                         (long)o->ticket_slots};
  return DIAGAN_OK;
}
DIAGAN_API int diagan_conv_gemm_pending_opts(diagan_conv_opts* o) {
  DG_REQUIRE(o, "conv_gemm_pending_opts: null");
  const CallOpts& c = g_opts_next;
  *o = diagan_conv_opts{c.wino, c.wino4, c.wino4x, c.gemm_x3, c.gemm_x3b, c.splitk_fused, c.force_ksplit, c.tune, c.tickets,
                        (int64_t)c.ticket_slots};
  return DIAGAN_OK;
}
DIAGAN_API int diagan_conv_gemm_last_cfg(void) { return g_last_cfg; }

DIAGAN_API int diagan_conv_gemm_set_stamp_buffer(unsigned long long* buf, int64_t slots) {
  g_stamps = buf;
  g_stamp_slots = buf ? (long)slots : 0;
  return DIAGAN_OK;
}
DIAGAN_API int diagan_conv_gemm_tune(int force_ksplit, int flags, int lds_delta_bytes) {
  g_force_ksplit = force_ksplit;
  g_tune_flags = flags;
  g_lds_delta = lds_delta_bytes;
  return DIAGAN_OK;
}
```

self-diagnosing-gan_amd/csrc/conv_wino4.hip:

```cpp
#include "conv_common.h"
#include <type_traits>
#include "wino_weights.h"

namespace diagan {

typedef float f32x2 __attribute__((ext_vector_type(2)));

constexpr int W4T = 32;
constexpr int W4N = 64;
constexpr int W4K = 8;
constexpr int W4_PS = 132;
constexpr int W4_VSTAGE = 84 * W4_PS;
constexpr int W4_U = 72 * 256;
#ifndef W4_ROW_AT
#define W4_ROW_AT 3
#endif
#ifndef W4_COL_AT
#define W4_COL_AT 5
#endif
#ifndef W4_DMA_IMM
#define W4_DMA_IMM 1
#endif
#ifndef W4_ULOAD_POOLED
#define W4_ULOAD_POOLED 0
#endif
#ifndef W4_PRO_LDS
#define W4_PRO_LDS 1
#endif
#ifndef W4_ULOAD
#define W4_ULOAD 1
#endif
#ifndef W4_PRIO_B
#define W4_PRIO_B 0
#endif
#ifndef W4_PRIO_ALT
#define W4_PRIO_ALT 0
#endif
#ifndef W4_ROW_AT2
#define W4_ROW_AT2 W4_ROW_AT
#endif
#ifndef W4_COL_AT2
#define W4_COL_AT2 W4_COL_AT
#endif
static_assert((2 * W4_VSTAGE + W4_U) * 4 <= 163840 && 36 * 32 * 32 <= 2 * W4_VSTAGE + W4_U,
              "162 432 bytes of the CU's 163 840; the epilogue's 36 x 32 x 32 floats fit inside");

#ifndef X3_ABL
#define X3_ABL 0
#endif
constexpr int X3_SP = 512;
constexpr int X3_SI = 3 * X3_SP + 16;
constexpr int X3_SJ = 6 * X3_SI + 16;
constexpr int X3_VSTAGE = 6 * X3_SJ;
constexpr int X3_RING = 4 * X3_UNIT;
constexpr int X3_LDS = 2 * X3_VSTAGE + 8 * X3_RING;
static_assert(X3_LDS <= 163840 && 36 * 32 * 32 * 4 <= X3_LDS, "161 088 bytes of the CU's 163 840; the epilogue's exchange image fits inside");
constexpr int x3_gmax(int u) { return (3 * (u + 1)) / 2 + 5; }
constexpr int x3_gneed(int v) { return (3 * (v + 1) + 1) / 2 - 1; }
constexpr int x3_vm_younger(int NS, int ph, bool hn, int NX, int load_at, int row_at, int kind, int s) {
  int seq[256] = {};
  for (int i = 0; i < 256; ++i) seq[i] = -1000;
  int n = 0, seqx = -1000;
  const int t = 4 + ph;
  for (int tt = t - 2; tt <= t; ++tt) {
    const bool h = tt < t ? true : hn;
    const int last = x3_gneed(NS * tt + NS - 1);
    if (tt == t && kind == 0 && s == -1) return n - seq[x3_gneed(NS * tt) - x3_gmax(NS * (t - 2) - 1)] - 1;
    for (int ss = 0; ss < NS; ++ss) {
      const int u = NS * tt + ss;
      if (h && ss == load_at) {
        n += NX;
        seqx = n - 1;
      }
      if (ss + 1 < NS && tt == t && kind == 0 && s == ss) return n - seq[x3_gneed(u + 1) - x3_gmax(NS * (t - 2) - 1)] - 1;
      for (int g = x3_gmax(u - 1) + 1; g <= x3_gmax(u); ++g)
        if (h || g <= last) seq[g - x3_gmax(NS * (t - 2) - 1)] = n++;
      if (ss == row_at && h && tt == t && kind == 1) return n - seqx - 1;
    }
  }
  return -1;
}
template <int I, int N, typename F>
__device__ __forceinline__ void static_for(F&& f) {
  if constexpr (I < N) {
    f(std::integral_constant<int, I>{});
    static_for<I + 1, N>(f);
  }
}
template <int... V>
constexpr int x3_seq_at(std::integer_sequence<int, V...>, int i) {
  const int v[] = {V...};
  return v[i];
}
template <int N>
__device__ __forceinline__ void x3_wait_vm() {
  static_assert(N >= 0 && N < 48, "vmcnt bookkeeping of the X3 schedule");
  asm volatile("s_waitcnt vmcnt(%0)" ::"n"(N) : "memory");
}

template <int MODE>
__global__ __launch_bounds__(512) void wino4_weight_kernel(const float* __restrict__ w, float* __restrict__ ug, int Co, int Ci,
                                                           int Kp, int flip, float wscale) {
  __shared__ f32x4 sg[WT_LDS_F4];
  wino4_weight_body<MODE>(w, ug, Co, Ci, Kp, flip, wscale, blockIdx.x, blockIdx.y, sg);
}
template <int MODE>
__global__ __launch_bounds__(512) void wino4x_weight_kernel(const float* __restrict__ w, float* __restrict__ ug, int Co, int Ci,
                                                            int Kp, int flip, float wscale) {
  __shared__ f32x4 sg[WT_LDS_F4];
  wino4x_weight_body<MODE>(w, ug, Co, Ci, Kp, flip, wscale, blockIdx.x, blockIdx.y, sg);
}

__global__ __launch_bounds__(512) void wino_weights_batched_kernel(const WinoJob* __restrict__ jobs, int n) {
  __shared__ f32x4 sg[WT_LDS_F4];
  int j = 0;
  while (j + 1 < n && (int)blockIdx.x >= jobs[j + 1].blk0) ++j;
  const WinoJob job = jobs[j];
  const int lb = blockIdx.x - job.blk0, nbx = (job.Ci + 31) >> 5;
  if (job.kind == WK_GX3) gx3_weight_job(job.w, job.u, job.Co, job.Kp, lb, nbx * ((job.Co + 63) >> 6));
  else if (job.kind == WK_F4X) wino4x_weight_body<0>(job.w, job.u, job.Co, job.Ci, job.Kp, job.flip, job.scale, lb % nbx, lb / nbx, sg);
  else if (job.kind == WK_F4X_POOL) wino4x_weight_body<1>(job.w, job.u, job.Co, job.Ci, job.Kp, job.flip, job.scale, lb % nbx, lb / nbx, sg);
  else if (job.kind == WK_F4) wino4_weight_body<0>(job.w, job.u, job.Co, job.Ci, job.Kp, job.flip, job.scale, lb % nbx, lb / nbx, sg);
  else if (job.kind == WK_F4_POOL) wino4_weight_body<1>(job.w, job.u, job.Co, job.Ci, job.Kp, job.flip, job.scale, lb % nbx, lb / nbx, sg);
  else wino_weight_body(job.w, job.u, job.Co, job.Ci, job.Kp, job.flip, lb % nbx, lb / nbx, sg);
}

struct W4Consts {
  float m1, p1, m2, p2, m4, p4, m5, p3;
};
__device__ __forceinline__ W4Consts w4_consts() {
  W4Consts k = {-1.f, 1.f, -2.f, 2.f, -4.f, 4.f, -5.f, 3.f};
  asm volatile("" : "+s"(k.m1), "+s"(k.p1), "+s"(k.m2), "+s"(k.p2), "+s"(k.m4), "+s"(k.p4), "+s"(k.m5), "+s"(k.p3));
  return k;
}
template <typename V>
__device__ __forceinline__ void w4_bt(V* d, const W4Consts& k) {
  const V t0 = d[0] * k.p4 + (d[2] * k.m5 + d[4]);
  const V t5 = d[1] * k.p4 + (d[3] * k.m5 + d[5]);
  const V a = d[2] * k.m4 + d[4], b = d[1] * k.m4 + d[3], c = d[2] * k.m1 + d[4], e = d[1] * k.m1 + d[3];
  d[0] = t0;
  d[1] = b * k.p1 + a;
  d[2] = b * k.m1 + a;
  d[3] = e * k.p2 + c;
  d[4] = e * k.m2 + c;
  d[5] = t5;
}

__device__ __forceinline__ void w4_bt_dup(const f32x4* d, f32x4* t, const W4Consts& k) {
  const f32x4 e = d[1] * k.m1 + d[2], f = d[1] * k.m4 + d[2];
  t[0] = d[0] * k.p4 + (d[1] * k.m5 + d[2]);
  t[1] = f * k.p2;
  t[2] = f32x4{0.f, 0.f, 0.f, 0.f};
  t[3] = e * k.p2 + e;
  t[4] = e * k.m1;
  t[5] = d[1] * k.p4 + (d[2] * k.m5 + d[3]);
}

template <typename V>
__device__ __forceinline__ void w4_up(const V* d, V* t, const W4Consts& k, float f0, float f5) {
  t[0] = (d[0] * k.p3 + d[1]) * f0;
  t[1] = d[1] * k.p3 + d[0];
  t[2] = d[1] * k.p3 + d[2];
  t[3] = d[2] * k.p3 + d[1];
  t[4] = d[2] * k.p3 + d[3];
  t[5] = (d[3] * k.p3 + d[2]) * f5;
  w4_bt(t, k);
}

#ifdef DIAGAN_WINO_ABLATE
#define W4_ON(bit) (!(a.tune & (bit)))
#else
#define W4_ON(bit) true
#endif

template <int PRO, int MODE = 0, bool X3 = false, int LEFT = 0>
__global__ __launch_bounds__(512) void conv_wino4_kernel(const ConvGemmArgs a, const float* __restrict__ ug) {
  using MD = W4M<MODE>;
  constexpr int NS = MD::NS, NI = MD::NI;
#ifdef DIAGAN_W4_STAMP
  const unsigned long long t_kernel = __builtin_amdgcn_s_memtime();
#endif
  constexpr bool POOL = MODE == 1, UNPOOL = MODE == 2, UPIN = MODE == 3;
  extern __shared__ __attribute__((aligned(16))) float smem[];
  const ConvGeom& g = a.g;
  const int tid = threadIdx.x, lane = tid & 63, wave = __builtin_amdgcn_readfirstlane(tid >> 6);
  if (W4_PRIO_B > 0 && wave >= 4) __builtin_amdgcn_s_setprio(W4_PRIO_B);
  const int tiles_n = (g.Co + W4N - 1) / W4N;
  const int tile = xcd_remap(blockIdx.x, gridDim.x);
  const int t0 = (tile / tiles_n) * W4T, nb = tile % tiles_n, n0 = nb * W4N;
  const int TW = g.Wo >> 2, TH = g.Ho >> 2;
  const int MT = g.B * TH * TW;
  const int nk = g.Ci / W4K;
  const int k_per = (nk + a.ksplit - 1) / a.ksplit;
  const int k_begin = blockIdx.y * k_per, k_end = min(k_begin + k_per, nk);
  constexpr bool affine = PRO == PRO_AFFINE_RELU || PRO == PRO_AFFINE;

  const int lr = tid & 7, lq = (tid >> 3) & 1, lt = tid >> 4;
  const int ur = lr >> 1, uc = lr & 1;
  const bool ract = UPIN || lr < (UNPOOL ? 4 : 6);
  const bool cact = lr < 6 && !(MD::pooled && lr == 2);
  unsigned off[NI];
  int kbound[NI];
  float ex0 = 1.f, ex5 = 1.f, ey0 = 1.f, ey5 = 1.f;
  {
    const int gt = t0 + lt;
    const bool tv = gt < MT && ract;
    const unsigned q1 = fdiv((unsigned)(tv ? gt : 0), a.dWo);
    const int tx = (tv ? gt : 0) - (int)q1 * TW;
    const unsigned b = fdiv(q1, a.dHo);
    const int ty = (int)q1 - (int)b * TH;
    const bool half = UNPOOL || UPIN;
    const int Hx = half ? g.Hi >> 1 : g.Hi, Wx = half ? g.Wi >> 1 : g.Wi;
    if (UPIN) {
      const int iy = min(max(2 * ty - 1 + ur, 0), Hx - 1);
      const int rowbase = ((int)b * Hx + iy) * Wx;
#pragma unroll
      for (int c = 0; c < NI; ++c) {
        const int ix = min(max(2 * tx - 1 + c, 0), Wx - 1);
        off[c] = tv ? (unsigned)((rowbase + ix) * g.Ci * 4 + lq * 16 + uc * 8) : 0x80000000u;
        kbound[c] = 0x7fffffff;
      }
      ex0 = tx == 0 ? 0.f : 1.f;
      ex5 = tx == TW - 1 ? 0.f : 1.f;
      ey0 = ty == 0 ? 0.f : 1.f;
      ey5 = ty == TH - 1 ? 0.f : 1.f;
    } else {
    const int iy = (UNPOOL ? 2 : 4) * ty - 1 + lr, ix0 = (UNPOOL ? 2 : 4) * tx - 1;
    const bool rv = tv && iy >= 0 && iy < Hx;
    const int rowbase = (((int)b * Hx + iy) * Wx + ix0) * g.Ci * 4 + lq * 16;
#pragma unroll
    for (int c = 0; c < NI; ++c) {
      const bool ok = rv && ix0 + c >= 0 && ix0 + c < Wx;
      off[c] = ok ? (unsigned)(rowbase + c * ((X3_ABL & 128) ? 32 : g.Ci * 4)) : 0x80000000u;
      kbound[c] = ok ? 0x7fffffff : 0;
    }
    }
  }
  typedef int i32x4 __attribute__((ext_vector_type(4)));
  i32x4 xsrc;
  {
    const unsigned long long xb = (unsigned long long)a.x;
    xsrc[0] = __builtin_amdgcn_readfirstlane((int)(unsigned)xb);
    xsrc[1] = __builtin_amdgcn_readfirstlane((int)((unsigned)(xb >> 32) & 0xffffu));
    xsrc[2] = __builtin_amdgcn_readfirstlane((int)((unsigned)g.B * g.Hi * g.Wi * g.Ci * ((UNPOOL || UPIN) ? 1u : 4u)));
    xsrc[3] = 0x00020000;
  }
  const int pro_group_off = a.pro_group_rows > 0 ? ((t0 * 16) / a.pro_group_rows) * g.Ci : 0;
  i32x4 scsrc = xsrc, shsrc = xsrc;
  const unsigned poff = (unsigned)(pro_group_off + lq * 4 + (UPIN ? uc * 2 : 0)) * 4u;
  if (affine) {
    const unsigned long long sb = (unsigned long long)a.pro_scale, hb = (unsigned long long)a.pro_shift;
    scsrc[0] = __builtin_amdgcn_readfirstlane((int)(unsigned)sb);
    scsrc[1] = __builtin_amdgcn_readfirstlane((int)((unsigned)(sb >> 32) & 0xffffu));
    shsrc[0] = __builtin_amdgcn_readfirstlane((int)(unsigned)hb);
    shsrc[1] = __builtin_amdgcn_readfirstlane((int)((unsigned)(hb >> 32) & 0xffffu));
    scsrc[2] = shsrc[2] = 0x7fffffff;
  }
  float* const vrow = smem + (UPIN ? (lq * 42 + ur) * W4_PS + lt * 4 + uc * 2
                                   : (ract ? (lq * 42 + lr) * W4_PS + lt * 4 : (1 << 22)));
  float* const vcol = smem + (cact ? (lq * 42 + 7 * lr) * W4_PS + lt * 4 : (1 << 22));
  char* const sm8 = reinterpret_cast<char*>(smem);
  const unsigned vrow3 = UPIN ? ur * X3_SI + lt * 16 + lq * 8 + uc * X3_SP
                              : (ract ? lr * X3_SI + lt * 16 + lq * 8 : (1u << 24));
  const unsigned vcol3 = cact ? lr * X3_SJ + lt * 16 + lq * 8 : (1u << 24);

  float* const ulds = smem + 2 * W4_VSTAGE;
  const float* ublock = ug + (long)nb * nk * MD::U_FLOATS + ((wave & 3) * 2 + (wave >> 2)) * NS * 256;
  float* const uslot = ulds + wave * NS * 256;

#if W4_DMA_IMM
#define W4_DMA_CASE(u)                                                                                                   \
  case u:                                                                                                                \
    __builtin_amdgcn_global_load_lds((const __attribute__((address_space(1))) void*)(up + 4 * 256),                     \
                                     (__attribute__((address_space(3))) void*)(uslot + 4 * 256), 16, ((u) - 4) * 1024, 0); \
    break;
  f32x4 uprobe = {0.f, 0.f, 0.f, 0.f};
  auto issue_u = [&](int kk, int s) {
    const float* up = ublock + (long)kk * MD::U_FLOATS + lane * 4;
    if (X3_ABL & 512) {
      asm volatile("global_load_dwordx4 %0, %1, off" : "+v"(uprobe) : "v"(up + s * 256) : "memory");
      return;
    }
    switch (s) {
      W4_DMA_CASE(0) W4_DMA_CASE(1) W4_DMA_CASE(2) W4_DMA_CASE(3) W4_DMA_CASE(4) W4_DMA_CASE(5) W4_DMA_CASE(6) W4_DMA_CASE(7)
      default:
        __builtin_amdgcn_global_load_lds((const __attribute__((address_space(1))) void*)(up + s * 256),
                                         (__attribute__((address_space(3))) void*)(uslot + s * 256), 16, 0, 0);
    }
  };
#undef W4_DMA_CASE
#else
  auto issue_u = [&](int kk, int s) {
    const float* up = ublock + (long)kk * MD::U_FLOATS + s * 256 + lane * 4;
    __builtin_amdgcn_global_load_lds((const __attribute__((address_space(1))) void*)up,
                                     (__attribute__((address_space(3))) void*)(uslot + s * 256), 16, 0, 0);
  };
#endif
  const W4Consts kc = w4_consts();
  constexpr bool PRO_LDS = W4_ULOAD && W4_PRO_LDS && !X3 && (!MD::pooled || LEFT > 0) && affine;
  float* const pls = smem + 2 * W4_VSTAGE;
  int x_kk = 0;
  f32x4 ra[6], psc = {1.f, 1.f, 1.f, 1.f}, psh = {0.f, 0.f, 0.f, 0.f};
  f32x2 rb[4], psc2 = {1.f, 1.f}, psh2 = {0.f, 0.f};
#pragma unroll
  for (int c = NI; c < 6; ++c) ra[c] = f32x4{0.f, 0.f, 0.f, 0.f};
  auto issue_x = [&](int kk) __attribute__((always_inline)) {
    const int soff = __builtin_amdgcn_readfirstlane(kk * (W4K * 4));
    x_kk = kk;
    if (UPIN) {
#pragma unroll
      for (int c = 0; c < 4; ++c)
        asm volatile("buffer_load_dwordx2 %0, %1, %2, %3 offen" : "=v"(rb[c]) : "v"(off[c]), "s"(xsrc), "s"(soff) : "memory");
      if (affine && !PRO_LDS) {
        asm volatile("buffer_load_dwordx2 %0, %1, %2, %3 offen" : "=v"(psc2) : "v"(poff), "s"(scsrc), "s"(soff) : "memory");
        asm volatile("buffer_load_dwordx2 %0, %1, %2, %3 offen" : "=v"(psh2) : "v"(poff), "s"(shsrc), "s"(soff) : "memory");
      }
      return;
    }
#pragma unroll
    for (int c = 0; c < NI; ++c)
      asm volatile("buffer_load_dwordx4 %0, %1, %2, %3 offen" : "=v"(ra[c]) : "v"(off[c]), "s"(xsrc), "s"(soff) : "memory");
    if (affine && !PRO_LDS) {
      asm volatile("buffer_load_dwordx4 %0, %1, %2, %3 offen" : "=v"(psc) : "v"(poff), "s"(scsrc), "s"(soff) : "memory");
      asm volatile("buffer_load_dwordx4 %0, %1, %2, %3 offen" : "=v"(psh) : "v"(poff), "s"(shsrc), "s"(soff) : "memory");
    }
  };
#define W4_WAIT_IN(n)                                                                                            \
  case n:                                                                                                        \
    if (UPIN)                                                                                                    \
      asm volatile("s_waitcnt vmcnt(" #n ")"                                                                     \
                   : "+v"(rb[0]), "+v"(rb[1]), "+v"(rb[2]), "+v"(rb[3]), "+v"(psc2), "+v"(psh2)::"memory");        \
    else                                                                                                         \
      asm volatile("s_waitcnt vmcnt(" #n ")"                                                                     \
                   : "+v"(ra[0]), "+v"(ra[1]), "+v"(ra[2]), "+v"(ra[3]), "+v"(ra[4]), "+v"(ra[5]), "+v"(psc), "+v"(psh)::"memory"); \
    break;
  auto wait_inputs = [&](int n) {
    switch (n) {
      W4_WAIT_IN(0) W4_WAIT_IN(1) W4_WAIT_IN(2) W4_WAIT_IN(3) W4_WAIT_IN(4) W4_WAIT_IN(5) W4_WAIT_IN(6) W4_WAIT_IN(7) W4_WAIT_IN(8)
      W4_WAIT_IN(9)
      default:
        if (UPIN) asm volatile("s_waitcnt vmcnt(0)" : "+v"(rb[0]), "+v"(rb[1]), "+v"(rb[2]), "+v"(rb[3]), "+v"(psc2), "+v"(psh2)::"memory");
        else asm volatile("s_waitcnt vmcnt(0)" : "+v"(ra[0]), "+v"(ra[1]), "+v"(ra[2]), "+v"(ra[3]), "+v"(ra[4]), "+v"(ra[5]), "+v"(psc), "+v"(psh)::"memory");
    }
  };
#undef W4_WAIT_IN
  auto row_pass = [&](int stage) __attribute__((always_inline)) {
    if (PRO_LDS) {
      const float* pr = pls + x_kk * W4K + lq * 4 + (UPIN ? uc * 2 : 0);
      if (UPIN) {
        psc2 = *reinterpret_cast<const f32x2*>(pr);
        psh2 = *reinterpret_cast<const f32x2*>(pr + g.Ci);
      } else {
        psc = *reinterpret_cast<const f32x4*>(pr);
        psh = *reinterpret_cast<const f32x4*>(pr + g.Ci);
      }
    }
    if (UPIN) {
#pragma unroll
      for (int c = 0; c < 4; ++c) {
        f32x2 v = rb[c];
        if (affine) v = v * psc2 + psh2;
        if (PRO == PRO_RELU || PRO == PRO_AFFINE_RELU) {
#pragma unroll
          for (int e = 0; e < 2; ++e) v[e] = __int_as_float(max(__float_as_int(v[e]), 0));
        } else if (PRO == PRO_LRELU) {
#pragma unroll
          for (int e = 0; e < 2; ++e) {
            const float q = v[e], q2 = 0.2f * q;
            asm("v_max_f32 %0, %1, %2" : "=v"(v[e]) : "v"(q), "v"(q2));
          }
        }
        rb[c] = v;
      }
      f32x2 t[6];
      w4_up(rb, t, kc, ex0, ex5);
      if (X3) {
        unsigned o = vrow3 + stage * X3_VSTAGE;
#pragma unroll
        for (int j = 0; j < 6; ++j) {
          *reinterpret_cast<f32x2*>(sm8 + o) = t[j];
          o += X3_SJ;
          asm volatile("" : "+v"(o));
        }
        return;
      }
      float* vs = vrow + stage * W4_VSTAGE;
#pragma unroll
      for (int j = 0; j < 6; ++j) *reinterpret_cast<f32x2*>(vs + j * 7 * W4_PS) = t[j];
      return;
    }
#pragma unroll
    for (int c = 0; c < NI; ++c) {
      f32x4 v = ra[c];
      if (PRO != PRO_NONE) {
        if (affine) v = v * psc + psh;
#pragma unroll
        for (int e = 0; e < 4; ++e) {
          const float q = v[e];
          float r;
          if (PRO == PRO_LRELU) {
            const float q2 = 0.2f * q;
            asm("v_max_f32 %0, %1, %2" : "=v"(r) : "v"(q), "v"(q2));
          } else if (PRO == PRO_RELU) {
            r = __int_as_float(max(__float_as_int(q), 0));
          } else if (PRO == PRO_AFFINE_RELU) {
            asm("v_med3_i32 %0, %1, 0, %2" : "=v"(r) : "v"(q), "v"(kbound[c]));
          } else {
            r = kbound[c] ? q : 0.f;
          }
          v[e] = r;
        }
      }
      ra[c] = v;
    }
    f32x4 t[6];
    if (UNPOOL) w4_bt_dup(ra, t, kc);
    else {
#pragma unroll
      for (int c = 0; c < 6; ++c) t[c] = ra[c];
      w4_bt(t, kc);
    }
    if (X3) {
      unsigned o = vrow3 + stage * X3_VSTAGE;
#pragma unroll
// ... 396 lines not shown
  };
  if constexpr (X3) {
    using I0 = std::integral_constant<int, 0>;
    using I1 = std::integral_constant<int, 1>;
    using I2 = std::integral_constant<int, 2>;
    using I3 = std::integral_constant<int, 3>;
    auto kloop3 = [&](auto place) __attribute__((always_inline)) {
      int kk = k_begin;
      for (; kk + 4 < k_end; kk += 4) {
        kstep3(kk, I0{}, std::true_type{}, ugrp, place);
        kstep3(kk + 1, I1{}, std::true_type{}, ugrp, place);
        kstep3(kk + 2, I2{}, std::true_type{}, ugrp, place);
        kstep3(kk + 3, I3{}, std::true_type{}, ugrp, place);
        ugrp += 4 * NS * X3_UNIT;
      }
      if (k_begin < k_end) {
        kstep3(kk, I0{}, std::true_type{}, ugrp, place);
        kstep3(kk + 1, I1{}, std::true_type{}, ugrp, place);
        kstep3(kk + 2, I2{}, std::true_type{}, ugrp, place);
        kstep3(kk + 3, I3{}, std::false_type{}, ugrp, place);
      }
    };
    if (std::is_same<PlA, PlB>::value || wave < 4) kloop3(PlA{});
    else kloop3(PlB{});
  } else if constexpr (ULOAD) {
    using P0 = std::integral_constant<int, 0>;
    using P1 = std::integral_constant<int, 1>;
    using P2 = std::integral_constant<int, 2>;
    if (NS % 3 == 0) {
      for (int kk = k_begin; kk + 1 < k_end; ++kk) kstep_ul(kk, std::true_type{}, P0{});
      if (k_begin < k_end) kstep_ul(k_end - 1, std::false_type{}, P0{});
    } else {
      int kk = k_begin;
      for (; kk + 3 < k_end; kk += 3) {
        kstep_ul(kk, std::true_type{}, P0{});
        kstep_ul(kk + 1, std::true_type{}, P1{});
        kstep_ul(kk + 2, std::true_type{}, P2{});
      }
      if (LEFT == 1) kstep_ul(kk, std::false_type{}, P0{});
      else {
        kstep_ul(kk, std::true_type{}, P0{});
        kstep_ul(kk + 1, std::false_type{}, P1{});
      }
    }
  } else {
  using RowA = std::integral_constant<int, W4_ROW_AT>;
  using ColA = std::integral_constant<int, W4_COL_AT>;
  using RowB = std::integral_constant<int, W4_ROW_AT2>;
  using ColB = std::integral_constant<int, W4_COL_AT2>;
  using PN = std::integral_constant<int, -1>;
  using PA = std::integral_constant<int, (W4_PRIO_ALT > 0) ? 0 : -1>;
  using PB = std::integral_constant<int, (W4_PRIO_ALT > 0) ? 1 : -1>;
  if ((W4_ROW_AT2 == W4_ROW_AT && W4_COL_AT2 == W4_COL_AT && W4_PRIO_ALT == 0) || wave < 4) {
    for (int kk = k_begin; kk + 1 < k_end; ++kk) kstep(kk, std::true_type{}, RowA{}, ColA{}, PA{});
  } else {
    for (int kk = k_begin; kk + 1 < k_end; ++kk) kstep(kk, std::true_type{}, RowB{}, ColB{}, PB{});
  }
  if (W4_PRIO_ALT > 0) __builtin_amdgcn_s_setprio(0);
  if (k_begin < k_end) kstep(k_end - 1, std::false_type{}, RowA{}, ColA{}, PN{});
  }

#ifdef DIAGAN_W4_STAMP
  if (a.stamps && lane == 0) {
    unsigned long long* o = a.stamps + (((size_t)blockIdx.y * gridDim.x + blockIdx.x) * 8 + wave) * 16;
    for (int i = 0; i < 12; ++i) o[i] = tacc[i];
    o[12] = __builtin_amdgcn_s_memtime() - t_entry;
    o[13] = k_end - k_begin;
    o[14] = t_entry - t_kernel;
  }
  const unsigned long long t_epi = __builtin_amdgcn_s_memtime();
#endif
#ifdef DIAGAN_WINO_ABLATE
  if (a.tune & 512) {
    if (acc[0][0] == 123.456f) a.y[0] = acc[1][3] + acc[5][5] + acc[8][7];
    return;
  }
#endif
  if (X3_ABL & 512) {
    asm volatile("s_waitcnt vmcnt(0)" : "+v"(uprobe)::"memory");
    if (uprobe[0] == 123.456f) a.y[0] = uprobe[1];
  }
  const float sc0 = a.scale0 ? a.scale0[0] : a.out_scale, sc1 = a.scale1 ? a.scale1[0] : a.out_scale;
  const int split = a.scale0 ? (POOL ? a.scale_split >> 2 : a.scale_split) : 0x7fffffff;
  const bool raw = a.ksplit > 1;
  const bool hr = !raw && a.residual != nullptr, hm = !raw && a.mask_src != nullptr, hs = !raw && a.stat_partials != nullptr;
  const int Mout = POOL ? a.M >> 2 : a.M;
  float* ydst = raw ? a.slab + (long)blockIdx.y * Mout * g.Co : a.y;
  const float rfloor = a.res_relu ? 0.f : -__builtin_huge_valf();
  const int et = tid >> 4, eq = (tid >> 1) & 7, eh = tid & 1;
  const int gt = t0 + et;
  const bool tv = gt < MT;
  const unsigned q1 = fdiv((unsigned)(tv ? gt : 0), a.dWo);
  const int tx = (tv ? gt : 0) - (int)q1 * TW;
  const unsigned eb = fdiv(q1, a.dHo);
  const int ty = (int)q1 - (int)eb * TH;
  const int Hy = POOL ? g.Ho >> 1 : g.Ho, Wy = POOL ? g.Wo >> 1 : g.Wo;
  const int oy0 = (POOL ? 2 * ty + eh : 4 * ty + 2 * eh), ox0 = (POOL ? 2 : 4) * tx;
  const int prow0 = ((int)eb * Hy + oy0) * Wy + ox0;
  const float scv = (prow0 < split ? sc0 : sc1) * (MD::pooled ? 0.25f : 1.f);
  const int ybytes = (int)((unsigned)Mout * (unsigned)g.Co * 4u);
  const __amdgpu_buffer_rsrc_t ysrc = __builtin_amdgcn_make_buffer_rsrc(ydst, 0, ybytes, 0x00020000);
  const __amdgpu_buffer_rsrc_t rsrc =
      __builtin_amdgcn_make_buffer_rsrc(const_cast<float*>(a.residual), 0, hr && !a.res_up ? ybytes : 0, 0x00020000);
  const __amdgpu_buffer_rsrc_t msrc = __builtin_amdgcn_make_buffer_rsrc(const_cast<float*>(a.mask_src), 0, hm ? ybytes : 0, 0x00020000);
  const int pixb = g.Co * 4, rowb = Wy * pixb;
#ifdef DIAGAN_W4_STAMP
  unsigned eacc[10] = {0, 0, 0, 0, 0, 0, 0, 0, 0, 0};
  unsigned long long elast = t_epi;
  auto etick = [&](int i) {
    const unsigned long long now = __builtin_amdgcn_s_memtime();
    eacc[i] += (unsigned)(now - elast);
    elast = now;
  };
#define W4_ETICK(i) etick(i)
#else
#define W4_ETICK(i)
#endif
  float* ss = smem;
  f32x4 cs1[2] = {{0.f, 0.f, 0.f, 0.f}, {0.f, 0.f, 0.f, 0.f}}, cs2[2] = {{0.f, 0.f, 0.f, 0.f}, {0.f, 0.f, 0.f, 0.f}};
  const f32x4 z4 = {0.f, 0.f, 0.f, 0.f};
  auto xidx = [&](int i, int j) { return MD::pooled ? 5 * (i < 2 ? i : i - 1) + (j < 2 ? j : j - 1) : 6 * i + j; };
#pragma unroll
  for (int p = 0; p < 2; ++p) {
    W4_ETICK(p == 0 ? 0 : 9);
    if (nh == p) {
#pragma unroll
      for (int s = 0; s < NS; ++s) {
        const int fx = MD::pooled ? w4p_start(grp) + s : 6 * (fi0 + s / 3) + fj0 + s % 3;
        if (!MD::pooled || s < w4p_count(grp)) {
#pragma unroll
          for (int e = 0; e < 16; ++e) {
            const int m = 8 * (e >> 2) + 4 * kh + (e & 3);
            ss[(fx * 32 + m) * 32 + fi] = acc[s][e];
          }
        }
      }
    }
#ifdef DIAGAN_W4_STAMP
    asm volatile("s_waitcnt lgkmcnt(0)" ::: "memory");
#endif
    W4_ETICK(1 + 4 * p);
    __syncthreads();
    W4_ETICK(2 + 4 * p);
    const int n = n0 + p * 32 + eq * 4;
    const bool ok = tv && n < g.Co;
    const unsigned voff = ok ? (unsigned)(prow0 * g.Co + n) * 4u : 0x80000000u;
    f32x4 bv = z4;
    if (!raw && a.bias && ok) bv = *reinterpret_cast<const f32x4*>(a.bias + n);
    if (POOL) {
      f32x4 sj[6];
#pragma unroll
      for (int j = 0; j < 6; ++j) {
        if (j == 2) continue;
        f32x4 m[6];
#pragma unroll
        for (int i = 0; i < 6; ++i)
          if (i != 2) m[i] = *reinterpret_cast<const f32x4*>(ss + (xidx(i, j) * 32 + et) * 32 + eq * 4);
        sj[j] = eh ? (2.f * m[1] + 12.f * m[3]) + (m[5] - 4.f * m[4]) : (m[0] + 2.f * m[1]) + (3.f * m[3] - m[4]);
      }
      f32x4 y2[2];
      y2[0] = (sj[0] + 2.f * sj[1]) + (3.f * sj[3] - sj[4]);
      y2[1] = (2.f * sj[1] + 12.f * sj[3]) + (sj[5] - 4.f * sj[4]);
#pragma unroll
      for (int bc = 0; bc < 2; ++bc) {
        const int soff = bc * pixb;
        f32x4 y = raw ? y2[bc] * 0.25f : y2[bc] * scv + bv;
        if (hr) {
          f32x4 r = __builtin_bit_cast(f32x4, __builtin_amdgcn_raw_buffer_load_b128(rsrc, voff, soff, 0));
#pragma unroll
          for (int e = 0; e < 4; ++e) r[e] = fmaxf(r[e], rfloor);
          y += r;
        }
        __builtin_amdgcn_raw_buffer_store_b128(__builtin_bit_cast(__attribute__((ext_vector_type(4))) unsigned, y), ysrc, voff, soff, 0);
      }
    } else {
    f32x4 sr[2][6];
#pragma unroll
    for (int j = 0; j < 6; ++j) {
      if (UNPOOL && j == 2) {
        sr[0][j] = sr[1][j] = z4;
        continue;
      }
      f32x4 m[6];
#pragma unroll
      for (int i = 0; i < 6; ++i)
        m[i] = (UNPOOL && i == 2) ? z4 : *reinterpret_cast<const f32x4*>(ss + (xidx(i, j) * 32 + et) * 32 + eq * 4);
      const f32x4 pp = m[1] + m[2], qq = m[1] - m[2], rr = m[3] + m[4], tt = m[3] - m[4];
      if (eh == 0) {
        sr[0][j] = m[0] + pp + rr;
        sr[1][j] = qq + 2.f * tt;
      } else {
        sr[0][j] = pp + 4.f * rr;
        sr[1][j] = qq + 8.f * tt + m[5];
      }
    }
#pragma unroll
    for (int ar = 0; ar < 2; ++ar) {
      const f32x4* s6 = sr[ar];
      const f32x4 pp = s6[1] + s6[2], qq = s6[1] - s6[2], rr = s6[3] + s6[4], tt = s6[3] - s6[4];
      f32x4 y4[4];
      y4[0] = s6[0] + pp + rr;
      y4[1] = qq + 2.f * tt;
      y4[2] = pp + 4.f * rr;
      y4[3] = qq + 8.f * tt + s6[5];
      f32x4 rup[8];
      if (hr && a.res_up == 2 && ok) {
        const float* rb = a.residual + (((long)eb * (g.Ho >> 1) + (oy0 >> 1)) * (g.Wo >> 1) + (ox0 >> 1)) * g.Co + n;
        rup[0] = 0.25f * *reinterpret_cast<const f32x4*>(rb);
        rup[1] = 0.25f * *reinterpret_cast<const f32x4*>(rb + g.Co);
      } else if (hr && a.res_up && ok) {
        const int Hh = g.Ho >> 1, Wh = g.Wo >> 1, jy = oy0 >> 1, jx = ox0 >> 1;
        const int y0 = ar ? jy : max(jy - 1, 0), y1 = ar ? min(jy + 1, Hh - 1) : jy;
        const int xx[4] = {max(jx - 1, 0), jx, jx + 1, min(jx + 2, Wh - 1)};
        const float* rb = a.residual + ((long)eb * Hh * Wh) * g.Co + n;
#pragma unroll
        for (int q = 0; q < 4; ++q) {
          rup[q] = *reinterpret_cast<const f32x4*>(rb + ((long)y0 * Wh + xx[q]) * g.Co);
          rup[4 + q] = *reinterpret_cast<const f32x4*>(rb + ((long)y1 * Wh + xx[q]) * g.Co);
        }
      }
#pragma unroll
      for (int bc = 0; bc < 4; ++bc) {
        const int soff = ar * rowb + bc * pixb;
        f32x4 y = raw ? (UNPOOL ? y4[bc] * 0.25f : y4[bc]) : y4[bc] * scv + bv;
        if (hr) {
          f32x4 r;
          if (a.res_up == 2) {
            r = rup[bc >> 1];
          } else if (a.res_up) {
            const int c0 = bc == 0 ? 0 : (bc == 3 ? 2 : 1);
            const float wy0 = ar ? 0.75f : 0.25f, wx0 = (bc & 1) ? 0.75f : 0.25f, wy1 = 1.f - wy0, wx1 = 1.f - wx0;
            const f32x4 top = wx0 * rup[c0] + wx1 * rup[c0 + 1];
            const f32x4 bot = wx0 * rup[4 + c0] + wx1 * rup[4 + c0 + 1];
            r = wy0 * top + wy1 * bot;
          } else {
            r = __builtin_bit_cast(f32x4, __builtin_amdgcn_raw_buffer_load_b128(rsrc, voff, soff, 0));
#pragma unroll
            for (int e = 0; e < 4; ++e) r[e] = fmaxf(r[e], rfloor);
          }
          y += r;
        }
        if (hm) {
          const f32x4 mk = __builtin_bit_cast(f32x4, __builtin_amdgcn_raw_buffer_load_b128(msrc, voff, soff, 0));
#pragma unroll
          for (int e = 0; e < 4; ++e) y[e] = mk[e] > 0.f ? y[e] : y[e] * a.mask_slope;
        }
#ifdef DIAGAN_WINO_ABLATE
        if (!W4_ON(1024)) {
          if (y[0] == 123.456f) ydst[0] = y[1];
        } else
#endif
        __builtin_amdgcn_raw_buffer_store_b128(__builtin_bit_cast(__attribute__((ext_vector_type(4))) unsigned, y), ysrc, voff, soff, 0);
        if (hs && ok) {
          cs1[p] += y;
          cs2[p] += y * y;
        }
      }
    }
    }
    W4_ETICK(3 + 4 * p);
    __syncthreads();
    W4_ETICK(4 + 4 * p);
  }
  if (hs) {
    float* red = smem;
#pragma unroll
    for (int p = 0; p < 2; ++p) {
#pragma unroll
      for (int e = 0; e < 4; ++e) {
        float v1 = cs1[p][e], v2 = cs2[p][e];
        v1 += __shfl_xor(v1, 1, 64);
        v2 += __shfl_xor(v2, 1, 64);
        v1 += __shfl_xor(v1, 16, 64);
        v2 += __shfl_xor(v2, 16, 64);
        v1 += __shfl_xor(v1, 32, 64);
        v2 += __shfl_xor(v2, 32, 64);
        cs1[p][e] = v1;
        cs2[p][e] = v2;
      }
      if ((lane & 0x31) == 0) {
        *reinterpret_cast<f32x4*>(red + ((wave * 2 + p) * 2 + 0) * 32 + eq * 4) = cs1[p];
        *reinterpret_cast<f32x4*>(red + ((wave * 2 + p) * 2 + 1) * 32 + eq * 4) = cs2[p];
      }
    }
    __syncthreads();
    if (tid < 128) {
      const int which = tid >> 6, col = tid & 63, p = col >> 5, c32 = col & 31;
      float t = 0.f;
#pragma unroll
      for (int w = 0; w < 8; ++w) t += red[((w * 2 + p) * 2 + which) * 32 + c32];
      if (n0 + col < g.Co) a.stat_partials[(long)(tile / tiles_n) * 2 * g.Co + which * g.Co + n0 + col] = t;
    }
  }
#ifdef DIAGAN_W4_STAMP
  if (a.stamps && lane == 0) {
    unsigned long long* o = a.stamps + (((size_t)blockIdx.y * gridDim.x + blockIdx.x) * 8 + wave) * 16;
    o[15] = __builtin_amdgcn_s_memtime() - t_epi;
    unsigned long long* o2 = a.stamps + ((size_t)gridDim.y * gridDim.x * 8 + ((size_t)blockIdx.y * gridDim.x + blockIdx.x) * 8 + wave) * 16;
    for (int i = 0; i < 10; ++i) o2[i] = eacc[i];
  }
#endif
}

template <int PRO, int MODE = 0, bool X3 = false, int LEFT = 0>
static int launch_wino4_pro(const ConvGemmArgs& a, const float* ug, hipStream_t st) {
  const int MT = a.g.B * (a.g.Ho >> 2) * (a.g.Wo >> 2);
  const int wgs = cdiv(MT, W4T) * cdiv(a.g.Co, W4N);
  const size_t lds = X3 ? (size_t)X3_LDS : (size_t)(2 * W4_VSTAGE + W4M<MODE>::U_FLOATS) * sizeof(float);
  auto kern = conv_wino4_kernel<PRO, MODE, X3, LEFT>;
  static FuncAttrLatch latch;
  DG_LDS(latch, kern, lds);
  hipLaunchKernelGGL(kern, dim3(wgs, a.ksplit), dim3(512), lds, st, a, ug);
  return check_launch("conv_wino4");
}

static int g_wino4x = -1;
void wino4_set_x3(int mode) { g_wino4x = mode; }
int call_opt_wino4x();
int wino4_get_x3() {
  static const int env = getenv("DIAGAN_WINO4_X3") ? atoi(getenv("DIAGAN_WINO4_X3")) : 0;
  const int c = call_opt_wino4x();
  return c >= 0 ? c : (g_wino4x >= 0 ? g_wino4x : env);
}
static long x3_floats(long fp32_floats) { return wino4_get_x3() > 0 ? fp32_floats + fp32_floats / 2 : fp32_floats; }
long wino4_ws_floats(int Co, int Ci) { return x3_floats((long)cdiv(Co, W4N) * W4N * Ci * 36); }
static bool wino4_x3_ok(const ConvGemmArgs& a) {
  const int nk = a.g.Ci / W4K, ks = a.ksplit > 0 ? a.ksplit : 1;
  return wino4_get_x3() > 0 && (a.g.Ci % 32) == 0 && nk % ks == 0 && (nk / ks) % 4 == 0;
}

template <int WM>
static const float* wino4_weights(const ConvGemmArgs& a, float* ws, int flip, float scale, long floats, hipStream_t st, bool x3 = false) {
  const int kind = x3 ? (WM ? WK_F4X_POOL : WK_F4X) : (WM ? WK_F4_POOL : WK_F4);
  if (const float* ready = wino_weights_ready(kind, flip, scale, floats)) return ready;
  const ConvGeom& g = a.g;
  if (x3)
    hipLaunchKernelGGL(wino4x_weight_kernel<WM>, dim3(cdiv(g.Ci, 32), cdiv(g.Co, W4N)), dim3(512), 0, st, a.w, ws, g.Co, g.Ci, g.Kp, flip,
                       scale);
  else
  hipLaunchKernelGGL(wino4_weight_kernel<WM>, dim3(cdiv(g.Ci, 32), cdiv(g.Co, W4N)), dim3(512), 0, st, a.w, ws, g.Co, g.Ci, g.Kp, flip,
                     scale);
  return ws;
}

int launch_wino_weights_batched(const WinoJob* jobs, int n, int blocks, hipStream_t st) {
  hipLaunchKernelGGL(wino_weights_batched_kernel, dim3(blocks), dim3(512), 0, st, jobs, n);
  return check_launch("wino_weights_batched");
}

bool wino4_geom_ok(int Ho, int Wo, int Ci) { return !(Ho & 3) && !(Wo & 3) && (Ci & 7) == 0; }

static int wino4_ksplit_impl(int B, int Ho, int Wo, int Ci, int Co, int allow_split, long ws_floats, double bar);
int wino4_ksplit(int B, int Ho, int Wo, int Ci, int Co, int allow_split, long ws_floats) {
  return wino4_ksplit_impl(B, Ho, Wo, Ci, Co, allow_split, ws_floats, 1.05);
}
static int wino4_ksplit_impl(int B, int Ho, int Wo, int Ci, int Co, int allow_split, long ws_floats, double bar) {
  const long wgs4 = (long)cdiv((long)B * (Ho >> 2) * (Wo >> 2), W4T) * cdiv(Co, W4N);
  const long wgs2 = (long)cdiv((long)B * (Ho >> 1) * (Wo >> 1), 64) * cdiv(Co, 64);
  auto fill = [](long w) { return (double)w / (256.0 * ((w + 255) / 256)); };
  if (wgs4 >= 192) {
    const bool can2 = allow_split && wgs4 <= 512 && Ci >= 512 && wino4_ws_floats(Co, Ci) + 2L * B * Ho * Wo * Co <= ws_floats;
    const double f1 = fill(wgs4), f2 = can2 ? 0.93 * fill(2 * wgs4) : 0.0;
    const double f = f2 > f1 ? f2 : f1;
    if (1.27 * f / (wgs2 >= 192 ? fill(wgs2) : 1.0) < bar) return 0;
    return f2 > f1 ? 2 : 1;
  }
  if (allow_split && wgs4 * 2 >= 192 && Ci >= 256 && wino4_ws_floats(Co, Ci) + 2L * B * Ho * Wo * Co <= ws_floats) return 2;
  return 0;
}

int launch_wino4(ConvGemmArgs a, float* ws, hipStream_t st) {
  const ConvGeom& g = a.g;
  a.dWo = make_fastdiv((unsigned)(g.Wo >> 2));
  a.dHo = make_fastdiv((unsigned)(g.Ho >> 2));
  const long f32 = (long)cdiv(g.Co, W4N) * W4N * g.Ci * 36;
  if (wino4_x3_ok(a)) {
    const float* ug = wino4_weights<0>(a, ws, g.dr < 0 ? 1 : 0, 1.f, f32 + f32 / 2, st, true);
    switch (a.pro_mode) {
      case PRO_NONE: return launch_wino4_pro<PRO_NONE, 0, true>(a, ug, st);
      case PRO_RELU: return launch_wino4_pro<PRO_RELU, 0, true>(a, ug, st);
      case PRO_AFFINE_RELU: return launch_wino4_pro<PRO_AFFINE_RELU, 0, true>(a, ug, st);
      case PRO_LRELU: return launch_wino4_pro<PRO_LRELU, 0, true>(a, ug, st);
      default: return launch_wino4_pro<PRO_AFFINE, 0, true>(a, ug, st);
    }
  }
  const float* ug = wino4_weights<0>(a, ws, g.dr < 0 ? 1 : 0, 1.f, f32, st);
  switch (a.pro_mode) {
    case PRO_NONE: return launch_wino4_pro<PRO_NONE>(a, ug, st);
    case PRO_RELU: return launch_wino4_pro<PRO_RELU>(a, ug, st);
    case PRO_AFFINE_RELU: return launch_wino4_pro<PRO_AFFINE_RELU>(a, ug, st);
    case PRO_LRELU: return launch_wino4_pro<PRO_LRELU>(a, ug, st);
    default: return launch_wino4_pro<PRO_AFFINE>(a, ug, st);
  }
}

bool wino4_pool_ok(int B, int Ho, int Wo, int Ci, int Co, long ws_floats, bool force) {
  static const int env = getenv("DIAGAN_WINO4_POOL") ? atoi(getenv("DIAGAN_WINO4_POOL")) : 1;
  static const int w4 = getenv("DIAGAN_WINO4") ? atoi(getenv("DIAGAN_WINO4")) : 1;
  static const int min_wgs = getenv("DIAGAN_WINO4_POOL_MIN_WGS") ? atoi(getenv("DIAGAN_WINO4_POOL_MIN_WGS")) : 192;
  if (!env || !w4 || !wino4_geom_ok(Ho, Wo, Ci) || (Co & 3) || Ci < 32) return false;
  const long wgs = (long)cdiv((long)B * (Ho >> 2) * (Wo >> 2), W4T) * cdiv(Co, W4N);
  return (force || wgs >= min_wgs) && x3_floats((long)cdiv(Co, W4N) * W4N * Ci * 28) <= ws_floats;
}

int launch_wino4_pool(ConvGemmArgs a, float* ws, hipStream_t st) {
  const ConvGeom& g = a.g;
  a.dWo = make_fastdiv((unsigned)(g.Wo >> 2));
  a.dHo = make_fastdiv((unsigned)(g.Ho >> 2));
  const float* ug = wino4_weights<1>(a, ws, 0, 1.f, (long)cdiv(g.Co, W4N) * W4N * g.Ci * 28, st);
#if W4_ULOAD && W4_ULOAD_POOLED
  const int left = (g.Ci / W4K) % 3;
  if (left == 1) return a.pro_mode == PRO_RELU ? launch_wino4_pro<PRO_RELU, 1, false, 1>(a, ug, st) : launch_wino4_pro<PRO_NONE, 1, false, 1>(a, ug, st);
  if (left == 2) return a.pro_mode == PRO_RELU ? launch_wino4_pro<PRO_RELU, 1, false, 2>(a, ug, st) : launch_wino4_pro<PRO_NONE, 1, false, 2>(a, ug, st);
#endif
  return a.pro_mode == PRO_RELU ? launch_wino4_pro<PRO_RELU, 1>(a, ug, st) : launch_wino4_pro<PRO_NONE, 1>(a, ug, st);
}

int launch_wino4_unpool(ConvGemmArgs a, float* ws, hipStream_t st) {
  const ConvGeom& g = a.g;
  a.dWo = make_fastdiv((unsigned)(g.Wo >> 2));
  a.dHo = make_fastdiv((unsigned)(g.Ho >> 2));
  const float* ug = wino4_weights<1>(a, ws, 1, 1.f, (long)cdiv(g.Co, W4N) * W4N * g.Ci * 28, st);
#if W4_ULOAD && W4_ULOAD_POOLED
  const int left = (g.Ci / W4K) % 3;
  if (left == 1) return launch_wino4_pro<PRO_NONE, 2, false, 1>(a, ug, st);
  if (left == 2) return launch_wino4_pro<PRO_NONE, 2, false, 2>(a, ug, st);
#endif
  return launch_wino4_pro<PRO_NONE, 2>(a, ug, st);
}

bool wino4_upin_ok(int B, int Ho, int Wo, int Ci, int Co, long ws_floats, bool force) {
  static const int env = getenv("DIAGAN_WINO4_UPIN") ? atoi(getenv("DIAGAN_WINO4_UPIN")) : 1;
  static const int w4 = getenv("DIAGAN_WINO4") ? atoi(getenv("DIAGAN_WINO4")) : 1;
  if (!env || !w4 || !wino4_geom_ok(Ho, Wo, Ci) || (Co & 3) || wino4_ws_floats(Co, Ci) > ws_floats) return false;
  return force || (Ci >= 64 && wino4_ksplit_impl(B, Ho, Wo, Ci, Co, 0, ws_floats, 0.93) == 1);
}

int launch_wino4_upin(ConvGemmArgs a, float* ws, hipStream_t st) {
  const ConvGeom& g = a.g;
  a.dWo = make_fastdiv((unsigned)(g.Wo >> 2));
  a.dHo = make_fastdiv((unsigned)(g.Ho >> 2));
  const long f32 = (long)cdiv(g.Co, W4N) * W4N * g.Ci * 36;
  if (wino4_x3_ok(a)) {
    const float* ug = wino4_weights<0>(a, ws, 0, 0.0625f, f32 + f32 / 2, st, true);
    switch (a.pro_mode) {
      case PRO_NONE: return launch_wino4_pro<PRO_NONE, 3, true>(a, ug, st);
      case PRO_RELU: return launch_wino4_pro<PRO_RELU, 3, true>(a, ug, st);
      case PRO_AFFINE_RELU: return launch_wino4_pro<PRO_AFFINE_RELU, 3, true>(a, ug, st);
      case PRO_LRELU: return launch_wino4_pro<PRO_LRELU, 3, true>(a, ug, st);
      default: return launch_wino4_pro<PRO_AFFINE, 3, true>(a, ug, st);
    }
  }
  const float* ug = wino4_weights<0>(a, ws, 0, 0.0625f, f32, st);
  switch (a.pro_mode) {
    case PRO_NONE: return launch_wino4_pro<PRO_NONE, 3>(a, ug, st);
    case PRO_RELU: return launch_wino4_pro<PRO_RELU, 3>(a, ug, st);
    case PRO_AFFINE_RELU: return launch_wino4_pro<PRO_AFFINE_RELU, 3>(a, ug, st);
    case PRO_LRELU: return launch_wino4_pro<PRO_LRELU, 3>(a, ug, st);
    default: return launch_wino4_pro<PRO_AFFINE, 3>(a, ug, st);
  }
}

}
```

self-diagnosing-gan_amd/csrc/wino_weights.h:

```cpp
#pragma once
#include "conv_common.h"

namespace diagan {

__device__ __forceinline__ void wino_weight_body(const float* __restrict__ w, float* __restrict__ ug, int Co, int Ci, int Kp, int flip,
                                                 int bx, int by, f32x4* __restrict__ sg) {
  f32x4 g[3][3];
  if (!wino_stage_taps(w, by * 64, bx * 32, Co, Ci, Kp, flip, sg, g)) return;
  const int col = threadIdx.x & 63, c = bx * 32 + (threadIdx.x >> 6) * 4;
  f32x4 t[4][3];
#pragma unroll
  for (int s = 0; s < 3; ++s) {
    t[0][s] = g[0][s];
    t[1][s] = 0.5f * (g[0][s] + g[1][s] + g[2][s]);
    t[2][s] = 0.5f * (g[0][s] - g[1][s] + g[2][s]);
    t[3][s] = g[2][s];
  }
  const int ks = c >> 3, kq = (c >> 2) & 1;
  float* base = ug + ((long)by * (Ci >> 3) + ks) * (16 * 2 * 64 * 4);
#pragma unroll
  for (int i = 0; i < 4; ++i) {
    f32x4 u[4];
    u[0] = t[i][0];
    u[1] = 0.5f * (t[i][0] + t[i][1] + t[i][2]);
    u[2] = 0.5f * (t[i][0] - t[i][1] + t[i][2]);
    u[3] = t[i][2];
    const float sg = i == 3 ? -1.f : 1.f;
#pragma unroll
    for (int j = 0; j < 4; ++j) {
      float* plane = base + ((i * 4 + j) * 2 + kq) * 256;
      const f32x4 v = u[j] * sg;
      *reinterpret_cast<f32x4*>(plane + col * 4) = v;
    }
  }
}


template <int MODE> struct W4M {
  static constexpr bool pooled = MODE == 1 || MODE == 2;
  static constexpr bool upin = MODE == 3;
  static constexpr int NS = pooled ? 7 : 9;
  static constexpr int U_FLOATS = 8 * NS * 256;
  static constexpr int NI = (MODE == 2 || MODE == 3) ? 4 : 6;
};
__host__ __device__ __forceinline__ int w4p_start(int g) { return g == 0 ? 0 : 7 + 6 * (g - 1); }
__host__ __device__ __forceinline__ int w4p_count(int g) { return g == 0 ? 7 : 6; }
__host__ __device__ __forceinline__ int w4p_freq(int v) { return v < 2 ? v : v + 1; }

typedef unsigned u32x2 __attribute__((ext_vector_type(2)));
constexpr int X3_UNIT = 1536;
__device__ __forceinline__ void x3_split(const f32x4& v, u32x2& p0, u32x2& p1, u32x2& p2) {
  unsigned x[4], r[4], q[4];
#pragma unroll
  for (int e = 0; e < 4; ++e) x[e] = __float_as_uint(v[e]);
  p0[0] = __builtin_amdgcn_perm(x[1], x[0], 0x07060302u);
  p0[1] = __builtin_amdgcn_perm(x[3], x[2], 0x07060302u);
#pragma unroll
  for (int e = 0; e < 4; ++e) r[e] = __float_as_uint(v[e] - __uint_as_float(x[e] & 0xffff0000u));
  p1[0] = __builtin_amdgcn_perm(r[1], r[0], 0x07060302u);
  p1[1] = __builtin_amdgcn_perm(r[3], r[2], 0x07060302u);
#pragma unroll
  for (int e = 0; e < 4; ++e) q[e] = __float_as_uint(__uint_as_float(r[e]) - __uint_as_float(r[e] & 0xffff0000u));
  p2[0] = __builtin_amdgcn_perm(q[1], q[0], 0x07060302u);
  p2[1] = __builtin_amdgcn_perm(q[3], q[2], 0x07060302u);
}

__device__ __forceinline__ void gx3_split_quad(const float* __restrict__ w, unsigned short* __restrict__ wx, long quad, long plane) {
  const f32x4 v = *reinterpret_cast<const f32x4*>(w + quad * 4);
  u32x2 p0, p1, p2;
  x3_split(v, p0, p1, p2);
  *reinterpret_cast<u32x2*>(wx + quad * 4) = p0;
  *reinterpret_cast<u32x2*>(wx + plane + quad * 4) = p1;
  *reinterpret_cast<u32x2*>(wx + 2 * plane + quad * 4) = p2;
}

__device__ __forceinline__ void gx3_weight_job(const float* __restrict__ w, float* __restrict__ u, int Co, int Kp, int lb, int nblk) {
  const long quads = (long)Co * Kp / 4, plane = quads * 4;
  const long per = (quads + nblk - 1) / nblk;
  const long q1 = min(quads, (long)(lb + 1) * per);
  for (long i = (long)lb * per + threadIdx.x; i < q1; i += 512) gx3_split_quad(w, reinterpret_cast<unsigned short*>(u), i, plane);
}


template <int MODE>
__device__ __forceinline__ void wino4x_weight_body(const float* __restrict__ w, float* __restrict__ ug, int Co, int Ci, int Kp, int flip,
                                                   float wscale, int bx, int by, f32x4* __restrict__ sg) {
  f32x4 g[3][3];
  const int nb = by;
  if (!wino_stage_taps(w, nb * 64, bx * 32, Co, Ci, Kp, flip, sg, g)) return;
  if (wscale != 1.f) {
#pragma unroll
    for (int t = 0; t < 9; ++t) g[t / 3][t % 3] *= wscale;
  }
  const int col = threadIdx.x & 63, c = bx * 32 + (threadIdx.x >> 6) * 4;
  constexpr float k4 = 0.25f, k6 = 1.f / 6.f, k12 = 1.f / 12.f, k24 = 1.f / 24.f;
  auto gt = [&](const f32x4& g0, const f32x4& g1, const f32x4& g2, f32x4* o) {
    o[0] = k4 * g0;
    o[1] = -k6 * (g0 + g1 + g2);
    o[2] = -k6 * (g0 - g1 + g2);
    o[3] = k24 * g0 + k12 * g1 + k6 * g2;
    o[4] = k24 * g0 - k12 * g1 + k6 * g2;
    o[5] = g2;
  };
  f32x4 t[3][6];
#pragma unroll
  for (int s = 0; s < 3; ++s) gt(g[0][s], g[1][s], g[2][s], t[s]);
  constexpr int NS = W4M<MODE>::NS;
  const int nk = Ci >> 3, ks = c >> 3, kh = (c >> 2) & 1, nh = col >> 5, n = col & 31;
  char* base = reinterpret_cast<char*>(ug) + (long)nb * 8 * nk * NS * X3_UNIT + n * 16 + kh * 8;
#pragma unroll
  for (int i = 0; i < 6; ++i) {
    f32x4 u[6];
    gt(t[0][i], t[1][i], t[2][i], u);
#pragma unroll
    for (int j = 0; j < 6; ++j) {
      int grp, slot;
      if (MODE == 0) {
        grp = (i / 3) * 2 + j / 3;
        slot = (i % 3) * 3 + j % 3;
      } else {
        if (i == 2 || j == 2) continue;
        const int l = 5 * (i < 2 ? i : i - 1) + (j < 2 ? j : j - 1);
        grp = l < 7 ? 0 : 1 + (l - 7) / 6;
        slot = l - w4p_start(grp);
      }
      u32x2 p0, p1, p2;
      x3_split(u[j], p0, p1, p2);
      char* d = base + ((long)((grp + 4 * nh) * nk + ks) * NS + slot) * X3_UNIT;
      *reinterpret_cast<u32x2*>(d) = p0;
      *reinterpret_cast<u32x2*>(d + 512) = p1;
      *reinterpret_cast<u32x2*>(d + 1024) = p2;
    }
  }
}

template <int MODE>
__device__ __forceinline__ void wino4_weight_body(const float* __restrict__ w, float* __restrict__ ug, int Co, int Ci, int Kp, int flip,
                                                  float wscale, int bx, int by, f32x4* __restrict__ sg) {
  f32x4 g[3][3];
  const int nb = by;
  if (!wino_stage_taps(w, nb * 64, bx * 32, Co, Ci, Kp, flip, sg, g)) return;
  if (wscale != 1.f) {
#pragma unroll
    for (int t = 0; t < 9; ++t) g[t / 3][t % 3] *= wscale;
  }
  const int col = threadIdx.x & 63, c = bx * 32 + (threadIdx.x >> 6) * 4;
  constexpr float k4 = 0.25f, k6 = 1.f / 6.f, k12 = 1.f / 12.f, k24 = 1.f / 24.f;
  auto gt = [&](const f32x4& g0, const f32x4& g1, const f32x4& g2, f32x4* o) {
    o[0] = k4 * g0;
    o[1] = -k6 * (g0 + g1 + g2);
    o[2] = -k6 * (g0 - g1 + g2);
    o[3] = k24 * g0 + k12 * g1 + k6 * g2;
    o[4] = k24 * g0 - k12 * g1 + k6 * g2;
    o[5] = g2;
  };
  f32x4 t[3][6];
#pragma unroll
  for (int s = 0; s < 3; ++s) gt(g[0][s], g[1][s], g[2][s], t[s]);
  const int nk = Ci >> 3, ks = c >> 3, kh = (c >> 2) & 1, nh = col >> 5, n = col & 31;
  float* base = ug + ((long)nb * nk + ks) * W4M<MODE>::U_FLOATS + (kh * 32 + n) * 4;
#pragma unroll
  for (int i = 0; i < 6; ++i) {
    f32x4 u[6];
    gt(t[0][i], t[1][i], t[2][i], u);
#pragma unroll
    for (int j = 0; j < 6; ++j) {
      if (MODE == 0) {
        const int unit = ((((i / 3) * 2 + j / 3) * 2 + nh) * 9) + (i % 3) * 3 + j % 3;
        *reinterpret_cast<f32x4*>(base + unit * 256) = u[j];
      } else if (i != 2 && j != 2) {
        const int l = 5 * (i < 2 ? i : i - 1) + (j < 2 ? j : j - 1);
        const int gq = l < 7 ? 0 : 1 + (l - 7) / 6, sl = l - w4p_start(gq);
        *reinterpret_cast<f32x4*>(base + ((gq * 2 + nh) * 7 + sl) * 256) = u[j];
      }
    }
  }
}


}
```

self-diagnosing-gan_amd/diagan/ops/conv.py:

```python
import torch

from diagan import _native as nat

P, I, F, I64 = nat.c_void_p, nat.c_int, nat.c_f32, nat.c_i64
nat.register("diagan_conv_gemm", [P, P, P, P, P, I, P, F, P, P, I, F, P, P, I] + [I] * 15 + [P, I64, P, I, P])
nat.register("diagan_conv_gemm_pick_ksplit", [I, I, I, I])
nat.register("diagan_conv_gemm_pick_cfg", [I, I, I, I])
nat.register("diagan_conv_wino_supported", [I] * 12)
nat.register("diagan_conv_gemm_set_wino", [I])
nat.register("diagan_conv_gemm_get_wino", [])
nat.register("diagan_conv_gemm_set_wino4", [I])
nat.register("diagan_conv_gemm_set_splitk_fused", [I])
nat.register("diagan_conv_gemm_set_splitk_tickets", [P, I64])
nat.register("diagan_conv_gemm_next_opts", [P])
nat.register("diagan_conv_gemm_pending_opts", [P])
nat.register("diagan_conv_gemm_last_cfg", [])
nat.register("diagan_conv_gemm_set_x3", [I])
nat.register("diagan_conv_gemm_get_x3", [])
nat.register("diagan_conv_gemm_set_x3b", [I])
nat.register("diagan_conv_gemm_get_x3b", [])
nat.register("diagan_conv_gemm_x3b_force_form", [I])
nat.register("diagan_conv_gemm_out_map", [I] * 9)
nat.register("diagan_conv_gemm_final_cfg", [I] * 15 + [I64] + [I] * 4)
nat.register("diagan_conv_wgrad_batched", [P, I, P])
nat.register("diagan_conv_wgrad_batch_max", [])
nat.register("diagan_conv_wgrad_batch_class", [I] * 14)
nat.register("diagan_conv_gemm_set_wino4x", [I])
nat.register("diagan_conv_gemm_get_wino4x", [])
nat.register("diagan_conv_wino4_pool_used", [I] * 5 + [I64])
nat.register("diagan_conv_wino4_upin_supported", [I] * 13 + [I64, I])
nat.register("diagan_conv_gemm_weights_hint", [P, I, I, F])
nat.register("diagan_conv_gemm_last_weight_format", [P, P, P, P, P])
nat.register("diagan_wino_weight_blocks", [I, I])
nat.register("diagan_wino_weights_batched", [P, I, I, P])
nat.register("diagan_conv_wgrad_uses_wino", [I] * 13)
nat.register("diagan_conv_wgrad_splits_geom", [I] * 14)
nat.register("diagan_conv_gemm_set_x3_pieces", [I])
nat.register("diagan_conv_gemm_get_x3_pieces", [])
nat.register("diagan_conv_wgrad_uses_x3", [I] * 15 + [I64])
nat.register("diagan_conv_wgrad_set_x3", [I])
nat.register("diagan_conv_gemm_pick_cfg_geom", [I] * 15 + [I64])
nat.register("diagan_conv_gemm_pick_cfg_grouped", [I] * 15 + [I64, I])
nat.register("diagan_conv_gemm_tile_rows", [I])
nat.register("diagan_conv_wino_pool_supported", [I] * 14 + [I64])
nat.register("diagan_conv_wino_unpool_supported", [I] * 13 + [I64])
nat.register("diagan_conv_gemm_tile_cols", [I])
nat.register("diagan_conv_gemm_set_stamp_buffer", [P, I64])
nat.register("diagan_conv_gemm_tune", [I, I, I])
nat.register("diagan_conv3x3_co4_supported", [I] * 8)
nat.register("diagan_conv3x3_co4", [P, P, P, P, P, P, P, I, I, I, I, I, I, I, I, I, P])
nat.register("diagan_conv3x3_ci4_supported", [I] * 8)
nat.register("diagan_conv3x3_ci4", [P, P, P, P, F, P, P, I, I, I, I, I, I, P])
nat.register("diagan_conv3x3_co4_wgrad_supported", [I] * 8)
nat.register("diagan_conv3x3_co4_wgrad_splits", [I, I])
nat.register("diagan_conv3x3_co4_wgrad", [P, P, P, I64, I64, P, P, I, I, I, I, I, I, P])
nat.register("diagan_conv_wgrad", [P, P, P, I, I, I64, I64, P, P, I] + [I] * 14 + [P])
nat.register("diagan_pack_batched", [P, I, I, I, I, I, P])
nat.register("diagan_wgrad_finish_batched", [P, I, I64, I, P])
nat.register("diagan_wgrad_finish_block_elems", [I])
nat.register("diagan_conv_wgrad_splits", [I, I, I])
nat.register("diagan_wgrad_reduce", [P, I, I64, P, I, P, P, P])
nat.register("diagan_sn_power_iter", [P, P, P, P, P, P, P, I, I, F, I, P])
nat.register("diagan_sn_prepare_batched", [P, I, I, I, I, I, F, I, I, P])
nat.register("diagan_pack_weights", [P, P, P, P, I, I, I, I, I, P])
nat.register("diagan_sn_grad_fix", [P, P, I, P, P, P, P, I, I, I, P])

PRO_NONE, PRO_RELU, PRO_AFFINE_RELU, PRO_LRELU, PRO_AFFINE = 0, 1, 2, 3, 4
PRO_BOX, PRO_BOX_RELU = 5, 6
TILE_SHAPES = {1: (128, 128, 2, 2, 32, False), 2: (128, 64, 2, 2, 32, False), 3: (64, 64, 2, 2, 32, False),
               4: (128, 64, 4, 1, 32, False), 5: (256, 64, 4, 1, 32, False), 6: (64, 64, 2, 2, 64, False),
               7: (64, 64, 2, 2, 32, True), 8: (128, 64, 2, 2, 32, True), 14: (64, 64, 2, 2, 32, True)}


def gemm_kernel_name(cfg, mode, Co=128, w4pool=False, Ci=0, RS=9, mapped=False):
    if cfg in (11, 12) and w4pool:
        return f"conv_wino4_kernel<{mode if cfg == 11 else 0},{cfg - 10},false>"
    if cfg == 9:
        return f"conv_wino_kernel<{mode}>"
    if cfg in (13, 15):
        x3 = "true" if (nat.fn("diagan_conv_gemm_get_wino4x")() > 0 and Ci % 32 == 0) else "false"
        return f"conv_wino4_kernel<{mode},{0 if cfg == 13 else 3},{x3}>"
    if cfg == 11:
        return f"conv_wino_pool_kernel<{mode},false,{2 if Co % 128 == 0 else 1}>"
    if cfg == 12:
        return f"conv_wino_pool_kernel<0,true,{2 if Co % 128 == 0 else 1}>"
    if cfg == 17:
        return f"conv_gemm_x3b_kernel<{mode},{'true' if mapped else 'false'}>"
    if cfg == 16:
        return f"conv_gemm_x3_kernel<{mode}>"
    bm, bn, wm, wn, bk, fp = TILE_SHAPES[cfg]
    kg = ",2" if cfg == 14 else ",1"
    return f"conv_gemm_kernel<{bm},{bn},{wm},{wn},{bk},{mode},false,{'true' if fp else 'false'}{kg}>"


class KernelTimer:

    def __init__(self, only=None):
        self.records = []
        self.only = only

    def wants_any(self):
        return self.only is None or len(self.only) > 0

    def begin(self, name=None):
        if self.only is not None and name not in self.only:
            return None
        ev = torch.cuda.Event(enable_timing=True)
        ev.record()
        return ev

    def end(self, name, flop, start, shape=None):
        stop = torch.cuda.Event(enable_timing=True)
        stop.record()
        self.records.append((name, flop, start, stop, shape))

    def summary(self):
        out = {}
        for name, flop, s, e, _ in self.records:
            d = out.setdefault(name, dict(launches=0, flop=0.0, seconds=0.0))
            d['launches'] += 1
            d['flop'] += flop
            d['seconds'] += s.elapsed_time(e) * 1e-3
        return out

    def by_shape(self):
        out = {}
        for name, flop, s, e, shape in self.records:
            d = out.setdefault((name,) + tuple(shape or ()), dict(launches=0, flop=0.0, seconds=0.0))
            d['launches'] += 1
            d['flop'] += flop
            d['seconds'] += s.elapsed_time(e) * 1e-3
        return out


TIMER = None
_NAME_CACHE = {}


import ctypes as _ct
import os as _os

WINO_BATCH = _os.environ.get("DIAGAN_WINO_BATCH", "1") != "0"


class WinoWeights:
    __slots__ = ("w_of", "Co", "Ci", "Kp", "fmt", "u", "ready", "used")

    def __init__(self, w_of, Co, Ci, Kp):
        self.w_of, self.Co, self.Ci, self.Kp = w_of, Co, Ci, Kp
        self.fmt, self.u, self.ready, self.used = None, None, None, False


_LWF = (_ct.c_int(), _ct.c_int(), _ct.c_float(), _ct.c_int64(), _ct.c_int64())
_LWF_REFS = tuple(_ct.byref(v) for v in _LWF)


def last_weight_format():
    nat.fn("diagan_conv_gemm_last_weight_format")(*_LWF_REFS)
    k, f, sc, n, cnt = _LWF
    return (k.value, f.value, sc.value, n.value), cnt.value


class WinoWeightBatch:

    def __init__(self):
        self.sites = []
        self._table_key, self._tables = None, None

    def site(self, w_of, Co, Ci, Kp):
        s = WinoWeights(w_of, Co, Ci, Kp)
        self.sites.append(s)
        return s

    def prepare(self, version):
        if not WINO_BATCH:
            return
        import numpy as np
        todo = [s for s in self.sites if s.fmt is not None and s.fmt[0] and s.used and s.ready != version]
        if not todo:
            return
        key = tuple((id(s), s.fmt, s.w_of().data_ptr()) for s in todo)
        if key != self._table_key:
            desc = np.dtype([('w', np.uint64), ('u', np.uint64), ('i', np.int32, 6), ('scale', np.float32), ('pad', np.int32)])
            tab, blk = np.zeros(len(todo), dtype=desc), 0
            for j, s in enumerate(todo):
                w = s.w_of()
                if s.u is None or s.u.numel() != s.fmt[3] or s.u.device != w.device:
                    s.u = torch.empty(s.fmt[3], dtype=torch.float32, device=w.device)
                tab[j]['w'], tab[j]['u'] = w.data_ptr(), s.u.data_ptr()
                tab[j]['i'] = [s.Co, s.Ci, s.Kp, s.fmt[0], s.fmt[1], blk]
                tab[j]['scale'] = s.fmt[2]
                blk += nat.fn("diagan_wino_weight_blocks")(s.Co, s.Ci)
            dev_tab = torch.from_numpy(tab.view(np.uint8).copy()).to(todo[0].w_of().device)
            self._table_key, self._tables = key, (dev_tab, len(todo), blk)
        tab, n, blocks = self._tables
        nat.call("diagan_wino_weights_batched", nat.ptr(tab), n, blocks, nat.current_stream())
        for s in todo:
            s.ready = version


def _hint(wsite, version):
    if wsite is not None and WINO_BATCH and wsite.u is not None and wsite.ready == version and wsite.fmt is not None:
        nat.call("diagan_conv_gemm_weights_hint", wsite.u.data_ptr(), wsite.fmt[0], wsite.fmt[1], wsite.fmt[2])


def _learn(wsite):
    if wsite is not None and WINO_BATCH:
        fmt, _ = last_weight_format()
        wsite.used = True
        if fmt != wsite.fmt:
            wsite.fmt, wsite.ready = fmt, None


def set_winograd(mode):
    nat.call("diagan_conv_gemm_set_wino", -1 if mode is None else (1 if mode else 0))


def set_winograd4x(mode):
    nat.call("diagan_conv_gemm_set_wino4x", -1 if mode is None else (1 if mode else 0))


def set_winograd4(mode):
    nat.call("diagan_conv_gemm_set_wino4", -1 if mode is None else (2 if mode == 'force-pool' else (1 if mode else 0)))


def round_up(x, m):
    return (x + m - 1) // m * m


class Geom:

    def __init__(self, kind, Ci, Co, R, S, stride=1, pad=0):
        assert kind in ('conv', 'convT')
        self.kind, self.Ci, self.Co, self.R, self.S, self.stride, self.pad = kind, Ci, Co, R, S, stride, pad
        self.Kp = round_up(R * S * Ci, 32)
        self.Kd = round_up(R * S * Co, 32)

    def out_hw(self, Hi, Wi):
        if self.kind == 'conv':
            return ((Hi + 2 * self.pad - self.R) // self.stride + 1,
                    (Wi + 2 * self.pad - self.S) // self.stride + 1)
        return ((Hi - 1) * self.stride - 2 * self.pad + self.R, (Wi - 1) * self.stride - 2 * self.pad + self.S)

    def fwd_params(self):
        return (self.stride, 1, -self.pad, 1) if self.kind == 'conv' else (1, -1, self.pad, self.stride)

    def dgrad_params(self):
        return (1, -1, self.pad, self.stride) if self.kind == 'conv' else (self.stride, 1, -self.pad, 1)


def _pro3(pro):
    if pro is None:
        return PRO_NONE, None, None
    if len(pro) > 3 and pro[3]:
        raise RuntimeError("grouped BatchNorm prologues exist for the forward kernels only")
    return tuple(pro)[:3]


def set_gemm_x3(on):
    nat.call("diagan_conv_gemm_set_x3", -1 if on is None else (1 if on else 0))
    nat.call("diagan_conv_gemm_set_x3b", -1 if on is None else (1 if on else 0))


def set_gemm_x3b(on):
    nat.call("diagan_conv_gemm_set_x3b", -1 if on is None else (1 if on else 0))


def set_x3_pieces(n):
    nat.call("diagan_conv_gemm_set_x3_pieces", 0 if n is None else int(n))


def set_wgrad_x3(on):
    nat.call("diagan_conv_wgrad_set_x3", -1 if on is None else (int(on) if on else 0))


def wgrad_uses_x3(geom, B, Hi, Wi, Ho, Wo, mode=0, bias_off=-1):
    sy, dr, off, up = geom.fwd_params()
    return bool(nat.fn("diagan_conv_wgrad_uses_x3")(B, Hi, Wi, geom.Ci, Ho, Wo, geom.Co, geom.R, geom.S, sy, dr, off, up, geom.Kp,
                                                    mode, bias_off))


_TICKETS = {}


def set_splitk_fused(on):
    nat.call("diagan_conv_gemm_set_splitk_fused", -1 if on is None else (1 if on else 0))
    if on:
        dev = torch.cuda.current_device()
        if dev not in _TICKETS:
            _TICKETS[dev] = torch.zeros(1 << 16, dtype=torch.int32, device=torch.device('cuda', dev))
        nat.call("diagan_conv_gemm_set_splitk_tickets", _TICKETS[dev].data_ptr(), _TICKETS[dev].numel())
    else:
        nat.call("diagan_conv_gemm_set_splitk_tickets", None, 0)


class ConvOpts(_ct.Structure):
    _fields_ = [(n, _ct.c_int32) for n in ("wino", "wino4", "wino4x", "gemm_x3", "gemm_x3b", "splitk_fused", "force_ksplit", "tune")] + \
               [("tickets", _ct.c_void_p), ("ticket_slots", _ct.c_int64)]


def next_opts(tickets=None, **fields):
    o = ConvOpts(-1, -1, -1, -1, -1, -1, 0, -1, None, 0)
    for k, v in fields.items():
        setattr(o, k, int(v))
    if tickets is not None:
        o.tickets, o.ticket_slots = tickets.data_ptr(), tickets.numel()
    nat.call("diagan_conv_gemm_next_opts", _ct.byref(o))


def pending_opts():
    o = ConvOpts()
    nat.call("diagan_conv_gemm_pending_opts", _ct.byref(o))
    return o


def _opts_key(o):
    return tuple(getattr(o, n) for n, _ in ConvOpts._fields_[:8])


def _without_wino(o):
    m = ConvOpts.from_buffer_copy(o)
    m.wino, m.wino4 = 0, 0
    return m


def last_cfg():
    return nat.fn("diagan_conv_gemm_last_cfg")()


def wg_x_shape(x, pro):
    B, H, W, Ci = x.shape
    if pro is not None and int(pro[0]) >= PRO_BOX:
        return B, H + 1, W + 1, Ci
    return B, H, W, Ci


def _chk(t, name):
    if t is None:
        return
    if not (t.is_cuda and t.dtype == torch.float32 and t.is_contiguous()):
        raise RuntimeError(f"{name}: expected a contiguous CUDA float32 tensor, got "
                           f"{t.dtype} {t.device} contiguous={t.is_contiguous()}")


def _gemm(x, w, out, geo_params, R, S, Kp, bias, residual, mask_src, mask_slope, pro, out_scale, tile_cfg,
          res_relu=False, row_scale=None, want_stats=False, wino=True, res_up=False, pool=False, unpool=False, up_in=False,
          wsite=None, wversion=None, res_unpool=False, out_map=None):
    B, Hi, Wi, Ci = x.shape
    _, Ho, Wo, Co = out.shape
    if out_map is not None:
        Ho, Wo = out_map[9], out_map[10]
    if up_in:
        Hi, Wi, tile_cfg = 2 * Hi, 2 * Wi, 15
        if pool or unpool or mask_src is not None:
            raise RuntimeError("conv_gemm: the up-sampled-input launch takes no pooling and no backward mask")
    if unpool:
        Hi, Wi, tile_cfg = 2 * Hi, 2 * Wi, 12
    if pool:
        Ho, Wo, tile_cfg = 2 * Ho, 2 * Wo, 11
        if want_stats or res_up or mask_src is not None:
            raise RuntimeError("conv_gemm: the pooled launch takes no statistics, mask or half-resolution residual")
    mode, scale, shift, group_imgs = (tuple(pro) + (0,))[:4] if pro is not None else (PRO_NONE, None, None, 0)
    for t, n in ((x, 'x'), (w, 'w'), (out, 'out'), (bias, 'bias'), (residual, 'residual'),
                 (mask_src, 'mask_src'), (scale, 'pro_scale'), (shift, 'pro_shift')):
        _chk(t, n)
    if w.shape != (Co, Kp):
        raise RuntimeError(f"conv_gemm: packed weight shape {tuple(w.shape)} != ({Co}, {Kp})")
    for t, n in ((residual, 'residual'), (mask_src, 'mask_src')):
        want = (B, Ho // 2, Wo // 2, Co) if ((res_up or res_unpool) and n == 'residual') else tuple(out.shape)
        if t is not None and tuple(t.shape) != want:
            raise RuntimeError(f"conv_gemm: {n} shape {tuple(t.shape)} != {want}")
    if (res_up or res_unpool) and (residual is None or res_relu or not wino or (res_up and res_unpool)):
        raise RuntimeError("conv_gemm: res_up / res_unpool need a half-resolution residual, no ReLU on it, and the Winograd kernel")
    sy, dr, off, up = geo_params
    stats = None
    if (mask_src is None and row_scale is None and out_scale == 1.0 and not res_relu and tile_cfg == 0 and not res_unpool
            and not want_stats and nat.fn("diagan_conv3x3_co4_supported")(Ci, Co, R, S, sy, dr, off, up)):
        t0 = TIMER.begin("conv3x3_co4_kernel") if TIMER is not None else None
        nat.call("diagan_conv3x3_co4", nat.ptr(x), nat.ptr(w), nat.ptr(out), nat.ptr(bias), nat.ptr(residual),
                 nat.ptr(scale), nat.ptr(shift), mode, B, Hi, Wi, Ci, dr, off, Kp, group_imgs, nat.current_stream())
        if t0 is not None:
            TIMER.end("conv3x3_co4_kernel", 2.0 * B * Ho * Wo * Co * R * S * Ci, t0,
                      (B * Ho * Wo, Co, R * S * Ci, f"pro{mode}"))
        return out
    if (mode == PRO_NONE and residual is None and mask_src is None and not res_relu and tile_cfg == 0 and not want_stats
            and nat.fn("diagan_conv3x3_ci4_supported")(Ci, Co, R, S, sy, dr, off, up)):
        t0 = TIMER.begin("conv3x3_ci4_kernel") if TIMER is not None else None
        nat.call("diagan_conv3x3_ci4", nat.ptr(x), nat.ptr(w), nat.ptr(out), nat.ptr(bias), out_scale,
                 nat.ptr(row_scale[0]) if row_scale else None, nat.ptr(row_scale[1]) if row_scale else None,
                 (B // 2) * Ho * Wo if row_scale else 0, B, Hi, Wi, Co, Kp, nat.current_stream())
        if t0 is not None:
            TIMER.end("conv3x3_ci4_kernel", 2.0 * B * Ho * Wo * Co * R * S * Ci, t0, (B * Ho * Wo, Co, R * S * Ci, "pro0"))
        return out
    ws = _splitk_ws(x.device)
    if tile_cfg == 0 and not wino:
        if want_stats:
            tile_cfg = nat.fn("diagan_conv_gemm_pick_cfg")(B * Ho * Wo, Co, Kp, 0)
        else:
            nat.call("diagan_conv_gemm_next_opts", _ct.byref(_without_wino(pending_opts())))
    if want_stats:
        M = B * Ho * Wo
        cfg = tile_cfg or nat.fn("diagan_conv_gemm_pick_cfg_grouped")(B, Hi, Wi, Ci, Ho, Wo, Co, R, S, sy, dr, off, up, Kp, 0,
                                                                       ws.numel(), group_imgs * Ho * Wo)
        bm = nat.fn("diagan_conv_gemm_tile_rows")(cfg)
        tiles = (M + bm - 1) // bm
        stats = (torch.empty((tiles, 2, Co), dtype=torch.float32, device=x.device), tiles)
        tile_cfg = cfg
    kname = None
    if TIMER is not None and TIMER.wants_any():
        key = (tile_cfg, B, Hi, Wi, Ci, Ho, Wo, Co, R, S, sy, dr, off, up, Kp, mode, want_stats, group_imgs, out_map is not None,
               mask_src is None, row_scale is None, res_relu, res_up, res_unpool, _opts_key(pending_opts()))
        kname = _NAME_CACHE.get(key)
        modes = (nat.fn("diagan_conv_gemm_get_wino")(), nat.fn("diagan_conv_gemm_get_wino4x")(), nat.fn("diagan_conv_gemm_get_x3")(),
                 nat.fn("diagan_conv_gemm_get_x3b")())
        if kname is None or _NAME_CACHE.get('modes') != modes:
            if _NAME_CACHE.get('modes') != modes:
                _NAME_CACHE.clear()
                _NAME_CACHE['modes'] = modes
            allow = 0 if want_stats else 1
            plain = mask_src is None and row_scale is None and not res_relu and not res_up and not res_unpool
            kname = gemm_kernel_name(tile_cfg or nat.fn("diagan_conv_gemm_final_cfg")(
                B, Hi, Wi, Ci, Ho, Wo, Co, R, S, sy, dr, off, up, Kp, allow, ws.numel(), group_imgs * Ho * Wo, mode,
                1 if plain else 0, 1 if want_stats else 0), mode, Co,
                w4pool=tile_cfg in (11, 12) and bool(nat.fn("diagan_conv_wino4_pool_used")(B, Ho, Wo, Ci, Co, ws.numel())), Ci=Ci, RS=R * S,
                mapped=out_map is not None)
            _NAME_CACHE[key] = kname
    t0 = TIMER.begin(kname) if TIMER is not None else None
    _hint(wsite, wversion)
    if out_map is not None:
        nat.call("diagan_conv_gemm_out_map", *out_map[:9])
    nat.call("diagan_conv_gemm", nat.ptr(x), nat.ptr(w), nat.ptr(out), nat.ptr(bias), nat.ptr(residual),
             (1 if res_relu else 0) | (2 if res_up else 0) | (4 if res_unpool else 0), nat.ptr(mask_src), mask_slope, nat.ptr(scale), nat.ptr(shift), mode, out_scale,
             nat.ptr(row_scale[0]) if row_scale else None, nat.ptr(row_scale[1]) if row_scale else None,
             (B // 2) * Ho * Wo if row_scale else 0,
             B, Hi, Wi, Ci, Ho, Wo, Co, R, S, sy, dr, off, up, Kp, tile_cfg, nat.ptr(ws), ws.numel(),
             nat.ptr(stats[0]) if stats else None, group_imgs * Ho * Wo, nat.current_stream())
    _learn(wsite)
    if t0 is not None:
        TIMER.end(kname, 2.0 * B * Ho * Wo * Co * R * S * Ci, t0,
                  (B * Ho * Wo, Co, R * S * Ci, f"pro{mode}{'+res' if residual is not None else ''}"
                                               f"{'+mask' if mask_src is not None else ''}{'+up' if up > 1 else ''}"))
    return (out, stats) if want_stats else out


_skws = {}


def _splitk_ws(dev):
    w = _skws.get(dev.index)
    if w is None:
        w = torch.empty(64 << 20, dtype=torch.float32, device=dev)
        _skws[dev.index] = w
    return w


def res_up_fused(geom, B, Hi, Wi, want_stats=False, group_imgs=0):
    Ho, Wo = geom.out_hw(Hi, Wi)
    sy, dr, off, up = geom.fwd_params()
    ws = _splitk_ws(torch.device('cuda', torch.cuda.current_device()))
    return nat.fn("diagan_conv_gemm_pick_cfg_grouped")(B, Hi, Wi, geom.Ci, Ho, Wo, geom.Co, geom.R, geom.S, sy, dr, off,
                                                       up, geom.Kp, 0 if want_stats else 1, ws.numel(),
                                                       group_imgs * Ho * Wo) in (9, 13)


def upin_fused(geom, B, Hl, Wl, group_imgs=0):
    Hi, Wi = 2 * Hl, 2 * Wl
    Ho, Wo = geom.out_hw(Hi, Wi)
    sy, dr, off, up = geom.fwd_params()
    ws = _splitk_ws(torch.device('cuda', torch.cuda.current_device()))
    return bool(nat.fn("diagan_conv_wino4_upin_supported")(B, Hi, Wi, geom.Ci, Ho, Wo, geom.Co, geom.R, geom.S, sy, dr, off, up,
                                                           ws.numel(), group_imgs * Ho * Wo))


def pool_fused(geom, B, Hi, Wi, pro=None):
    Ho, Wo = geom.out_hw(Hi, Wi)
    sy, dr, off, up = geom.fwd_params()
    mode = pro[0] if pro is not None else PRO_NONE
    ws = _splitk_ws(torch.device('cuda', torch.cuda.current_device()))
    return bool(nat.fn("diagan_conv_wino_pool_supported")(B, Hi, Wi, geom.Ci, Ho, Wo, geom.Co, geom.R, geom.S, sy, dr, off, up,
                                                          mode, ws.numel()))


def conv_fwd(geom, x, wf, bias=None, residual=None, pro=None, out=None, tile_cfg=0, res_relu=False, row_scale=None,
             want_stats=False, out_scale=1.0, wino=True, res_up=False, pool=False, up_in=False, wsite=None, wversion=None,
             out_map=None):
    B, Hi, Wi, Ci = x.shape
    if Ci != geom.Ci:
        raise RuntimeError(f"conv_fwd: input has {Ci} channels, layer expects {geom.Ci}")
    Ho, Wo = geom.out_hw(2 * Hi, 2 * Wi) if up_in else geom.out_hw(Hi, Wi)
    if pool:
        Ho, Wo = Ho // 2, Wo // 2
    if out_map is not None:
        if out is None:
            raise RuntimeError("conv_fwd: an output map needs the target tensor")
        out_map = tuple(out_map) + (out.shape[1], out.shape[2], Ho, Wo)
    if out is None:
        out = torch.empty((B, Ho, Wo, geom.Co), dtype=torch.float32, device=x.device)
    return _gemm(x, wf, out, geom.fwd_params(), geom.R, geom.S, geom.Kp, bias, residual, None, 0.0, pro, out_scale,
                 tile_cfg, res_relu=res_relu, row_scale=row_scale, want_stats=want_stats, wino=wino, res_up=res_up, pool=pool,
                 up_in=up_in, wsite=wsite, wversion=wversion, out_map=out_map)


def out_map_ok(geom, B, Hi, Wi, pro=None, wino=True):
    Ho, Wo = geom.out_hw(Hi, Wi)
    sy, dr, off, up = geom.fwd_params()
    ws = _splitk_ws(torch.device('cuda', torch.cuda.current_device()))
    mode = pro[0] if pro is not None else PRO_NONE
    pend = None if wino else pending_opts()
    if pend is not None:
        nat.call("diagan_conv_gemm_next_opts", _ct.byref(_without_wino(pend)))
    try:
        return nat.fn("diagan_conv_gemm_final_cfg")(B, Hi, Wi, geom.Ci, Ho, Wo, geom.Co, geom.R, geom.S, sy, dr, off, up, geom.Kp, 1,
                                                   ws.numel(), 0, mode, 1, 0) == 17
    finally:
        if pend is not None:
            nat.call("diagan_conv_gemm_next_opts", _ct.byref(pend))


def conv_dgrad(geom, dy, wd, in_hw, residual=None, mask_src=None, mask_slope=0.0, out=None, tile_cfg=0,
               row_scale=None, wino=True, unpool=False, wsite=None, wversion=None, res_unpool=False):
    B, Ho, Wo, Co = dy.shape
    if Co != geom.Co:
# ... 290 lines not shown
```

Measured before the change: 5323.

## Add 128-column Winograd F(4,3) conv kernel with new weight layout

Adds a new Winograd F(4x4,3x3) forward convolution kernel that computes 128 output channels per workgroup over 16 tiles. It uses a dedicated transformed-weight layout, software-pipelined input transforms interleaved with MFMA, and fused stat partials reduced through tickets. It is enabled by default (env default 1) for plain and upsampled-input convs when Co%128==0 and there is no split-K or x3 path. The wider N tile is meant to improve input-transform reuse and reduce redundant transforms, at the cost of large LDS use and heavy register pressure.

```diff
diff --git a/include/diagan_hip.h b/include/diagan_hip.h
--- a/include/diagan_hip.h
+++ b/include/diagan_hip.h
@@ -67,6 +67,9 @@
 int diagan_conv_gemm_set_wino4(int mode);
 int diagan_conv_gemm_set_wino4x(int mode);
 int diagan_conv_gemm_get_wino4x(void);
+int diagan_conv_gemm_set_wino4n(int mode);
+int diagan_conv_gemm_get_wino4n(void);
+int diagan_conv_gemm_last_wino4n(void);
 int diagan_conv_gemm_set_splitk_fused(int mode);
 int diagan_conv_gemm_set_splitk_tickets(int* buf, int64_t slots);
 typedef struct diagan_conv_opts {
diff --git a/self-diagnosing-gan_amd/csrc/conv_common.h b/self-diagnosing-gan_amd/csrc/conv_common.h
--- a/self-diagnosing-gan_amd/csrc/conv_common.h
+++ b/self-diagnosing-gan_amd/csrc/conv_common.h
@@ -163,7 +163,7 @@
   return c0 + q * 4 < Ci;
 }
 
-enum WinoKind : int { WK_F2 = 2, WK_F4 = 40, WK_F4_POOL = 41, WK_F4X = 42, WK_F4X_POOL = 43, WK_GX3 = 50 };
+enum WinoKind : int { WK_F2 = 2, WK_F4 = 40, WK_F4_POOL = 41, WK_F4X = 42, WK_F4X_POOL = 43, WK_F4N = 44, WK_GX3 = 50 };
 struct WinoJob {
   const float* w;
   float* u;
diff --git a/self-diagnosing-gan_amd/csrc/conv_gemm.hip b/self-diagnosing-gan_amd/csrc/conv_gemm.hip
--- a/self-diagnosing-gan_amd/csrc/conv_gemm.hip
+++ b/self-diagnosing-gan_amd/csrc/conv_gemm.hip
@@ -37,6 +37,11 @@
 int launch_wino4_upin(ConvGemmArgs a, float* ws, hipStream_t st);
 void wino4_set_x3(int mode);
 int wino4_get_x3();
+void wino4_set_n128(int mode);
+int wino4_get_n128();
+int wino4_last_n128();
+bool wino4_n128_takes(int Ci, int Co, int ks, bool x3);
+void wino4_note_ws(long floats);
 int launch_wino_pool(ConvGemmArgs a, float* ws, hipStream_t st);
 int launch_wino_unpool(ConvGemmArgs a, float* ws, hipStream_t st);
 int wino_pool_ksplit(int B, int Ho, int Wo, int Ci, int Co, long slab_floats, int min_wgs);
@@ -924,6 +929,7 @@
     const long wfl = wino4_ws_floats(Co, Ci);
     DG_REQUIRE(splitk_ws && splitk_ws_floats >= wfl, "conv_gemm: tile_cfg 15 needs %ld floats of workspace for the transformed weights", wfl);
     a.ksplit = 1;
+    wino4_note_ws((long)splitk_ws_floats);
     return launch_wino4_upin(a, splitk_ws, st);
   }
   if (cfg == 13) {
@@ -940,6 +946,7 @@
     }
     a.ksplit = ks;
     a.slab = splitk_ws + wfl;
+    wino4_note_ws((long)splitk_ws_floats);
     int rc = launch_wino4(a, splitk_ws, st);
     if (rc == DIAGAN_OK && ks > 1) {
       long blocks = ((long)a.M * (Co / 4) + 255) / 256;
@@ -1107,6 +1114,13 @@
   return DIAGAN_OK;
 }
 DIAGAN_API int diagan_conv_gemm_get_wino4x(void) { return wino4_get_x3(); }
+DIAGAN_API int diagan_conv_gemm_set_wino4n(int mode) {
+  DG_REQUIRE(mode >= -1 && mode <= 1, "set_wino4n: -1, 0 or 1");
+  wino4_set_n128(mode);
+  return DIAGAN_OK;
+}
+DIAGAN_API int diagan_conv_gemm_get_wino4n(void) { return wino4_get_n128(); }
+DIAGAN_API int diagan_conv_gemm_last_wino4n(void) { return wino4_last_n128(); }
 DIAGAN_API int diagan_conv_gemm_set_x3(int mode) {
   DG_REQUIRE(mode >= -1 && mode <= 1, "set_x3: -1, 0 or 1");
   g_gemm_x3 = mode;
diff --git a/self-diagnosing-gan_amd/csrc/conv_wino4.hip b/self-diagnosing-gan_amd/csrc/conv_wino4.hip
--- a/self-diagnosing-gan_amd/csrc/conv_wino4.hip
+++ b/self-diagnosing-gan_amd/csrc/conv_wino4.hip
@@ -111,6 +111,12 @@
   wino4x_weight_body<MODE>(w, ug, Co, Ci, Kp, flip, wscale, blockIdx.x, blockIdx.y, sg);
 }
 
+__global__ __launch_bounds__(512) void wino4n_weight_kernel(const float* __restrict__ w, float* __restrict__ ug, int Co, int Ci, int Kp,
+                                                            int flip, float wscale) {
+  __shared__ f32x4 sg[WT_LDS_F4];
+  wino4n_weight_body(w, ug, Co, Ci, Kp, flip, wscale, blockIdx.x, blockIdx.y, sg);
+}
+
 __global__ __launch_bounds__(512) void wino_weights_batched_kernel(const WinoJob* __restrict__ jobs, int n) {
   __shared__ f32x4 sg[WT_LDS_F4];
   int j = 0;
@@ -120,6 +126,7 @@
   if (job.kind == WK_GX3) gx3_weight_job(job.w, job.u, job.Co, job.Kp, lb, nbx * ((job.Co + 63) >> 6));
   else if (job.kind == WK_F4X) wino4x_weight_body<0>(job.w, job.u, job.Co, job.Ci, job.Kp, job.flip, job.scale, lb % nbx, lb / nbx, sg);
   else if (job.kind == WK_F4X_POOL) wino4x_weight_body<1>(job.w, job.u, job.Co, job.Ci, job.Kp, job.flip, job.scale, lb % nbx, lb / nbx, sg);
+  else if (job.kind == WK_F4N) wino4n_weight_body(job.w, job.u, job.Co, job.Ci, job.Kp, job.flip, job.scale, lb % nbx, lb / nbx, sg);
   else if (job.kind == WK_F4) wino4_weight_body<0>(job.w, job.u, job.Co, job.Ci, job.Kp, job.flip, job.scale, lb % nbx, lb / nbx, sg);
   else if (job.kind == WK_F4_POOL) wino4_weight_body<1>(job.w, job.u, job.Co, job.Ci, job.Kp, job.flip, job.scale, lb % nbx, lb / nbx, sg);
   else wino_weight_body(job.w, job.u, job.Co, job.Ci, job.Kp, job.flip, lb % nbx, lb / nbx, sg);
@@ -1122,6 +1129,507 @@
 #endif
 }
 
+#ifndef W4N_ROW_AT
+#define W4N_ROW_AT 5
+#endif
+#ifndef W4N_COL_AT
+#define W4N_COL_AT 10
+#endif
+constexpr int W4NT = 16, W4NN = 128, W4NK = 16;
+constexpr int W4N_PS = 68;
+constexpr int W4N_VSTAGE = 4 * 42 * W4N_PS;
+constexpr int W4N_XS = 68;
+constexpr int W4N_XCH = 36 * W4NT * W4N_XS;
+static_assert(W4N_XCH * 4 <= 163840, "the epilogue's exchange image fits the CU's LDS");
+
+template <int PRO, int MODE>
+__global__ __launch_bounds__(512) void conv_wino4n_kernel(const ConvGemmArgs a, const float* __restrict__ ug) {
+  static_assert(MODE == 0 || MODE == 3, "the 128-column shape runs the plain and the up-sampled-input convolution");
+  constexpr bool UPIN = MODE == 3;
+  constexpr int NI = UPIN ? 4 : 6;
+#ifdef DIAGAN_W4_STAMP
+  const unsigned long long t_kernel = __builtin_amdgcn_s_memtime();
+#endif
+  extern __shared__ __attribute__((aligned(16))) float smem[];
+  const ConvGeom& g = a.g;
+  const int tid = threadIdx.x, lane = tid & 63, wave = __builtin_amdgcn_readfirstlane(tid >> 6);
+  const int tiles_n = g.Co / W4NN;
+  const int tile = xcd_remap(blockIdx.x, gridDim.x);
+  const int t0 = (tile / tiles_n) * W4NT, nb = tile % tiles_n, n0 = nb * W4NN;
+  const int TW = g.Wo >> 2, TH = g.Ho >> 2;
+  const int MT = g.B * TH * TW;
+  const int nk = g.Ci / W4NK;
+  constexpr bool affine = PRO == PRO_AFFINE_RELU || PRO == PRO_AFFINE;
+
+  const int lr = tid & 7, lq = (tid >> 3) & 3, lt = tid >> 5;
+  const int ur = lr >> 1, uc = lr & 1;
+  const bool ract = UPIN || lr < 6;
+  const bool cact = lr < 6;
+  unsigned off[NI];
+  int kbound[NI];
+  float ex0 = 1.f, ex5 = 1.f, ey0 = 1.f, ey5 = 1.f;
+  {
+    const int gt = t0 + lt;
+    const bool tv = gt < MT && ract;
+    const unsigned q1 = fdiv((unsigned)(tv ? gt : 0), a.dWo);
+    const int tx = (tv ? gt : 0) - (int)q1 * TW;
+    const unsigned b = fdiv(q1, a.dHo);
+    const int ty = (int)q1 - (int)b * TH;
+    const int Hx = UPIN ? g.Hi >> 1 : g.Hi, Wx = UPIN ? g.Wi >> 1 : g.Wi;
+    if (UPIN) {
+      const int iy = min(max(2 * ty - 1 + ur, 0), Hx - 1);
+      const int rowbase = ((int)b * Hx + iy) * Wx;
+#pragma unroll
+      for (int c = 0; c < NI; ++c) {
+        const int ix = min(max(2 * tx - 1 + c, 0), Wx - 1);
+        off[c] = tv ? (unsigned)((rowbase + ix) * g.Ci * 4 + lq * 16 + uc * 8) : 0x80000000u;
+        kbound[c] = 0x7fffffff;
+      }
+      ex0 = tx == 0 ? 0.f : 1.f;
+      ex5 = tx == TW - 1 ? 0.f : 1.f;
+      ey0 = ty == 0 ? 0.f : 1.f;
+      ey5 = ty == TH - 1 ? 0.f : 1.f;
+    } else {
+      const int iy = 4 * ty - 1 + lr, ix0 = 4 * tx - 1;
+      const bool rv = tv && iy >= 0 && iy < Hx;
+      const int rowbase = (((int)b * Hx + iy) * Wx + ix0) * g.Ci * 4 + lq * 16;
+#pragma unroll
+      for (int c = 0; c < NI; ++c) {
+        const bool ok = rv && ix0 + c >= 0 && ix0 + c < Wx;
+        off[c] = ok ? (unsigned)(rowbase + c * g.Ci * 4) : 0x80000000u;
+        kbound[c] = ok ? 0x7fffffff : 0;
+      }
+    }
+  }
+  typedef int i32x4 __attribute__((ext_vector_type(4)));
+  i32x4 xsrc;
+  {
+    const unsigned long long xb = (unsigned long long)a.x;
+    xsrc[0] = __builtin_amdgcn_readfirstlane((int)(unsigned)xb);
+    xsrc[1] = __builtin_amdgcn_readfirstlane((int)((unsigned)(xb >> 32) & 0xffffu));
+    xsrc[2] = __builtin_amdgcn_readfirstlane((int)((unsigned)g.B * g.Hi * g.Wi * g.Ci * (UPIN ? 1u : 4u)));
+    xsrc[3] = 0x00020000;
+  }
+  const int pro_group_off = a.pro_group_rows > 0 ? ((t0 * 16) / a.pro_group_rows) * g.Ci : 0;
+  float* const pls = smem + 2 * W4N_VSTAGE;
+  float* const vrow = smem + (UPIN ? (lq * 42 + ur) * W4N_PS + lt * 4 + uc * 2
+                                   : (ract ? (lq * 42 + lr) * W4N_PS + lt * 4 : (1 << 22)));
+  float* const vcol = smem + (cact ? (lq * 42 + 7 * lr) * W4N_PS + lt * 4 : (1 << 22));
+  float* const vcw = smem + (cact ? ((lq & 1) * 42 + 7 * lr) * W4N_PS + lt * 4 + 2 * (lq >> 1) : (1 << 22));
+  const W4Consts kc = w4_consts();
+
+  int x_kk = 0;
+  f32x4 ra[6], psc = {1.f, 1.f, 1.f, 1.f}, psh = {0.f, 0.f, 0.f, 0.f};
+  f32x2 rb[4], psc2 = {1.f, 1.f}, psh2 = {0.f, 0.f};
+#pragma unroll
+  for (int c = NI; c < 6; ++c) ra[c] = f32x4{0.f, 0.f, 0.f, 0.f};
+  auto issue_x = [&](int kk) __attribute__((always_inline)) {
+    const int soff = __builtin_amdgcn_readfirstlane(kk * (W4NK * 4));
+    x_kk = kk;
+    if (UPIN) {
+#pragma unroll
+      for (int c = 0; c < 4; ++c)
+        asm volatile("buffer_load_dwordx2 %0, %1, %2, %3 offen" : "=v"(rb[c]) : "v"(off[c]), "s"(xsrc), "s"(soff) : "memory");
+      return;
+    }
+#pragma unroll
+    for (int c = 0; c < NI; ++c)
+      asm volatile("buffer_load_dwordx4 %0, %1, %2, %3 offen" : "=v"(ra[c]) : "v"(off[c]), "s"(xsrc), "s"(soff) : "memory");
+  };
+  auto wait_inputs0 = [&]() {
+    if (UPIN) asm volatile("s_waitcnt vmcnt(0)" : "+v"(rb[0]), "+v"(rb[1]), "+v"(rb[2]), "+v"(rb[3])::"memory");
+    else asm volatile("s_waitcnt vmcnt(0)" : "+v"(ra[0]), "+v"(ra[1]), "+v"(ra[2]), "+v"(ra[3]), "+v"(ra[4]), "+v"(ra[5])::"memory");
+  };
+  auto row_pass = [&](int stage) __attribute__((always_inline)) {
+    if (affine) {
+      const float* pr = pls + x_kk * W4NK + lq * 4 + (UPIN ? uc * 2 : 0);
+      if (UPIN) {
+        psc2 = *reinterpret_cast<const f32x2*>(pr);
+        psh2 = *reinterpret_cast<const f32x2*>(pr + g.Ci);
+      } else {
+        psc = *reinterpret_cast<const f32x4*>(pr);
+        psh = *reinterpret_cast<const f32x4*>(pr + g.Ci);
+      }
+    }
+    if (UPIN) {
+#pragma unroll
+      for (int c = 0; c < 4; ++c) {
+        f32x2 v = rb[c];
+        if (affine) v = v * psc2 + psh2;
+        if (PRO == PRO_RELU || PRO == PRO_AFFINE_RELU) {
+#pragma unroll
+          for (int e = 0; e < 2; ++e) v[e] = __int_as_float(max(__float_as_int(v[e]), 0));
+        } else if (PRO == PRO_LRELU) {
+#pragma unroll
+          for (int e = 0; e < 2; ++e) {
+            const float q = v[e], q2 = 0.2f * q;
+            asm("v_max_f32 %0, %1, %2" : "=v"(v[e]) : "v"(q), "v"(q2));
+          }
+        }
+        rb[c] = v;
+      }
+      f32x2 t[6];
+      w4_up(rb, t, kc, ex0, ex5);
+      float* vs = vrow + stage * W4N_VSTAGE;
+#pragma unroll
+      for (int j = 0; j < 6; ++j) *reinterpret_cast<f32x2*>(vs + j * 7 * W4N_PS) = t[j];
+      return;
+    }
+#pragma unroll
+    for (int c = 0; c < NI; ++c) {
+      f32x4 v = ra[c];
+      if (PRO != PRO_NONE) {
+        if (affine) v = v * psc + psh;
+#pragma unroll
+        for (int e = 0; e < 4; ++e) {
+          const float q = v[e];
+          float r;
+          if (PRO == PRO_LRELU) {
+            const float q2 = 0.2f * q;
+            asm("v_max_f32 %0, %1, %2" : "=v"(r) : "v"(q), "v"(q2));
+          } else if (PRO == PRO_RELU) {
+            r = __int_as_float(max(__float_as_int(q), 0));
+          } else if (PRO == PRO_AFFINE_RELU) {
+            asm("v_med3_i32 %0, %1, 0, %2" : "=v"(r) : "v"(q), "v"(kbound[c]));
+          } else {
+            r = kbound[c] ? q : 0.f;
+          }
+          v[e] = r;
+        }
+      }
+      ra[c] = v;
+    }
+    f32x4 t[6];
+#pragma unroll
+    for (int c = 0; c < 6; ++c) t[c] = ra[c];
+    w4_bt(t, kc);
+    float* vs = vrow + stage * W4N_VSTAGE;
+#pragma unroll
+    for (int j = 0; j < 6; ++j) *reinterpret_cast<f32x4*>(vs + j * 7 * W4N_PS) = t[j];
+  };
+  auto col_pass = [&](int stage) __attribute__((always_inline)) {
+    float* vs = vcol + stage * W4N_VSTAGE;
+    f32x4 d[6];
+#pragma unroll
+    for (int i = 0; i < (UPIN ? 4 : 6); ++i) d[i] = *reinterpret_cast<const f32x4*>(vs + i * W4N_PS);
+    if (UPIN) {
+      f32x4 t[6];
+      w4_up(d, t, kc, ey0, ey5);
+#pragma unroll
+      for (int i = 0; i < 6; ++i) d[i] = t[i];
+    } else {
+      w4_bt(d, kc);
+    }
+    float* w0 = vcw + stage * W4N_VSTAGE;
+#pragma unroll
+    for (int i = 0; i < 6; ++i) {
+      *reinterpret_cast<f32x2*>(w0 + i * W4N_PS) = f32x2{d[i][0], d[i][2]};
+      *reinterpret_cast<f32x2*>(w0 + 84 * W4N_PS + i * W4N_PS) = f32x2{d[i][1], d[i][3]};
+    }
+  };
+
+  const int grp = wave & 3, nh = wave >> 2;
+  f32x4 acc[9][4];
+#pragma unroll
+  for (int s = 0; s < 9; ++s)
+#pragma unroll
+    for (int q = 0; q < 4; ++q) acc[s][q] = f32x4{0.f, 0.f, 0.f, 0.f};
+
+  const float* const ublock = ug + (long)nb * nk * W4N_U_FLOATS + (grp * 2 + nh) * 36 * 256;
+  f32x4 ub[6] = {{0.f, 0.f, 0.f, 0.f}, {0.f, 0.f, 0.f, 0.f}, {0.f, 0.f, 0.f, 0.f},
+                 {0.f, 0.f, 0.f, 0.f}, {0.f, 0.f, 0.f, 0.f}, {0.f, 0.f, 0.f, 0.f}};
+  const unsigned ulane = lane * 16;
+#define W4N_UL(kk, q)                                                                                                            \
+  asm volatile("global_load_dwordx4 %0, %1, %2 offset:%3"                                                                       \
+               : "=v"(ub[(q) % 6])                                                                                               \
+               : "v"(ulane), "s"((unsigned long long)(ublock + (long)(kk) * W4N_U_FLOATS) + ((q) / 8) * 8192 + 4096),          \
+                 "n"(((q) % 8 - 4) * 1024)                                                                                       \
+               : "memory")
+  if (affine) {
+    for (int c = tid * 4; c < 2 * g.Ci; c += 2048) {
+      const float* src = c < g.Ci ? a.pro_scale + pro_group_off + c : a.pro_shift + pro_group_off + (c - g.Ci);
+      *reinterpret_cast<f32x4*>(pls + c) = *reinterpret_cast<const f32x4*>(src);
+    }
+    __syncthreads();
+  }
+  if (nk > 0) {
+    W4N_UL(0, 0);
+    W4N_UL(0, 1);
+    W4N_UL(0, 2);
+    W4N_UL(0, 3);
+    W4N_UL(0, 4);
+    W4N_UL(0, 5);
+    issue_x(0);
+    wait_inputs0();
+    row_pass(0);
+    col_pass(0);
+  }
+  asm volatile("s_waitcnt vmcnt(0)" ::: "memory");
+  __syncthreads();
+
+  const int fi0 = 3 * (grp >> 1), fj0 = 3 * (grp & 1);
+  const float* const fa_lane = smem + ((lane >> 4) * 42 + 7 * fj0 + fi0) * W4N_PS + (lane & 15) * 4;
+#ifdef DIAGAN_W4_STAMP
+  unsigned tacc[12] = {0, 0, 0, 0, 0, 0, 0, 0, 0, 0, 0, 0};
+  unsigned long long tlast = __builtin_amdgcn_s_memtime();
+  const unsigned long long t_entry = tlast;
+  auto tick = [&](int i) {
+    const unsigned long long now = __builtin_amdgcn_s_memtime();
+    tacc[i] += (unsigned)(now - tlast);
+    tlast = now;
+  };
+#define W4N_TICK(i) tick(i)
+#else
+#define W4N_TICK(i)
+#endif
+  auto kstep = [&](int kk, auto has_next) __attribute__((always_inline)) {
+    constexpr bool HN = decltype(has_next)::value;
+    const int cur = kk & 1;
+    W4N_TICK(9);
+    const float* const fa_base = fa_lane + cur * W4N_VSTAGE;
+    f32x4 fa[2];
+    fa[0] = *reinterpret_cast<const f32x4*>(fa_base);
+    W4N_TICK(0);
+    if (HN) issue_x(kk + 1);
+    static_for<0, 18>([&](auto slot) __attribute__((always_inline)) {
+      constexpr int s = decltype(slot)::value, fs = s >> 1, h = s & 1;
+      if (h == 0 && fs + 1 < 9)
+        fa[(fs + 1) & 1] = *reinterpret_cast<const f32x4*>(fa_base + (7 * ((fs + 1) % 3) + (fs + 1) / 3) * W4N_PS);
+      {
+        constexpr int ahead = HN ? 2 : (17 - s < 2 ? 17 - s : 2);
+        constexpr int NW = 2 * ahead + (HN && s < 3 ? NI : 0);
+        asm volatile("s_waitcnt vmcnt(%2)" : "+v"(ub[(2 * s) % 6]), "+v"(ub[(2 * s + 1) % 6]) : "n"(NW) : "memory");
+      }
+#pragma unroll
+      for (int e = 0; e < 4; ++e) {
+        acc[fs][2 * h] = __builtin_amdgcn_mfma_f32_16x16x4f32(fa[fs & 1][e], ub[(2 * s) % 6][e], acc[fs][2 * h], 0, 0, 0);
+        acc[fs][2 * h + 1] = __builtin_amdgcn_mfma_f32_16x16x4f32(fa[fs & 1][e], ub[(2 * s + 1) % 6][e], acc[fs][2 * h + 1], 0, 0, 0);
+      }
+      __builtin_amdgcn_sched_barrier(0);
+      if (s + 3 < 18) {
+        W4N_UL(kk, 2 * s + 6);
+        W4N_UL(kk, 2 * s + 7);
+      } else if (HN) {
+        W4N_UL(kk + 1, 2 * s + 6 - 36);
+        W4N_UL(kk + 1, 2 * s + 7 - 36);
+      }
+      if (HN) {
+        if (s == W4N_ROW_AT) {
+          W4N_TICK(1);
+          constexpr int NR = 2 * (W4N_ROW_AT + 1);
+          if (UPIN)
+            asm volatile("s_waitcnt vmcnt(%4)" : "+v"(rb[0]), "+v"(rb[1]), "+v"(rb[2]), "+v"(rb[3]) : "n"(NR) : "memory");
+          else
+            asm volatile("s_waitcnt vmcnt(%6)" : "+v"(ra[0]), "+v"(ra[1]), "+v"(ra[2]), "+v"(ra[3]), "+v"(ra[4]), "+v"(ra[5]) : "n"(NR) : "memory");
+          W4N_TICK(2);
+          row_pass(cur ^ 1);
+          W4N_TICK(3);
+        } else if (s == W4N_COL_AT) {
+          W4N_TICK(4);
+          col_pass(cur ^ 1);
+          W4N_TICK(5);
+        }
+      }
+      __builtin_amdgcn_sched_barrier(0);
+    });
+    W4N_TICK(6);
+#ifdef DIAGAN_W4_STAMP
+    asm volatile("s_waitcnt lgkmcnt(0)" ::: "memory");
+    W4N_TICK(7);
+#endif
+    asm volatile("s_waitcnt lgkmcnt(0)\n\ts_barrier" ::: "memory");
+    W4N_TICK(8);
+  };
+  for (int kk = 0; kk + 1 < nk; ++kk) kstep(kk, std::true_type{});
+  if (nk > 0) kstep(nk - 1, std::false_type{});
+#undef W4N_TICK
+#undef W4N_UL
+#ifdef DIAGAN_W4_STAMP
+  if (a.stamps && lane == 0) {
+    unsigned long long* o = a.stamps + ((size_t)blockIdx.x * 8 + wave) * 16;
+    for (int i = 0; i < 12; ++i) o[i] = tacc[i];
+    o[12] = __builtin_amdgcn_s_memtime() - t_entry;
+    o[13] = 2 * nk;
+    o[14] = t_entry - t_kernel;
+  }
+  const unsigned long long t_epi = __builtin_amdgcn_s_memtime();
+#endif
+
+  const float sc0 = a.scale0 ? a.scale0[0] : a.out_scale, sc1 = a.scale1 ? a.scale1[0] : a.out_scale;
+  const int split = a.scale0 ? a.scale_split : 0x7fffffff;
+  const bool hr = a.residual != nullptr, hm = a.mask_src != nullptr, hs = a.stat_partials != nullptr;
+  const int Mout = a.M;
+  float* ydst = a.y;
+  const float rfloor = a.res_relu ? 0.f : -__builtin_huge_valf();
+  const int et = tid >> 5, eq = (tid >> 1) & 15, eh = tid & 1;
+  const int gt = t0 + et;
+  const bool tv = gt < MT;
+  const unsigned q1 = fdiv((unsigned)(tv ? gt : 0), a.dWo);
+  const int tx = (tv ? gt : 0) - (int)q1 * TW;
+  const unsigned eb = fdiv(q1, a.dHo);
+  const int ty = (int)q1 - (int)eb * TH;
+  const int Hy = g.Ho, Wy = g.Wo;
+  const int oy0 = 4 * ty + 2 * eh, ox0 = 4 * tx;
+  const int prow0 = ((int)eb * Hy + oy0) * Wy + ox0;
+  const float scv = prow0 < split ? sc0 : sc1;
+  const int ybytes = (int)((unsigned)Mout * (unsigned)g.Co * 4u);
+  const __amdgpu_buffer_rsrc_t ysrc = __builtin_amdgcn_make_buffer_rsrc(ydst, 0, ybytes, 0x00020000);
+  const __amdgpu_buffer_rsrc_t rsrc =
+      __builtin_amdgcn_make_buffer_rsrc(const_cast<float*>(a.residual), 0, hr && !a.res_up ? ybytes : 0, 0x00020000);
+  const __amdgpu_buffer_rsrc_t msrc = __builtin_amdgcn_make_buffer_rsrc(const_cast<float*>(a.mask_src), 0, hm ? ybytes : 0, 0x00020000);
+  const int pixb = g.Co * 4, rowb = Wy * pixb;
+  float* ss = smem;
+  f32x4 cs1[2] = {{0.f, 0.f, 0.f, 0.f}, {0.f, 0.f, 0.f, 0.f}}, cs2[2] = {{0.f, 0.f, 0.f, 0.f}, {0.f, 0.f, 0.f, 0.f}};
+  const f32x4 z4 = {0.f, 0.f, 0.f, 0.f};
+#pragma unroll
+  for (int p = 0; p < 2; ++p) {
+    if (nh == p) {
+#pragma unroll
+      for (int s = 0; s < 9; ++s) {
+        const int fx = 6 * (fi0 + s / 3) + fj0 + s % 3;
+#pragma unroll
+        for (int q = 0; q < 4; ++q)
+#pragma unroll
+          for (int r = 0; r < 4; ++r) ss[(fx * W4NT + 4 * (lane >> 4) + r) * W4N_XS + q * 16 + (lane & 15)] = acc[s][q][r];
+      }
+    }
+    __syncthreads();
+    const int n = n0 + p * 64 + eq * 4;
+    const bool ok = tv;
+    const unsigned voff = ok ? (unsigned)(prow0 * g.Co + n) * 4u : 0x80000000u;
+    f32x4 bv = z4;
+    if (a.bias && ok) bv = *reinterpret_cast<const f32x4*>(a.bias + n);
+    f32x4 sr[2][6];
+#pragma unroll
+    for (int j = 0; j < 6; ++j) {
+      f32x4 m[6];
+#pragma unroll
+      for (int i = 0; i < 6; ++i) m[i] = *reinterpret_cast<const f32x4*>(ss + ((6 * i + j) * W4NT + et) * W4N_XS + eq * 4);
+      const f32x4 pp = m[1] + m[2], qq = m[1] - m[2], rr = m[3] + m[4], tt = m[3] - m[4];
+      if (eh == 0) {
+        sr[0][j] = m[0] + pp + rr;
+        sr[1][j] = qq + 2.f * tt;
+      } else {
+        sr[0][j] = pp + 4.f * rr;
+        sr[1][j] = qq + 8.f * tt + m[5];
+      }
+    }
+#pragma unroll
+    for (int ar = 0; ar < 2; ++ar) {
+      const f32x4* s6 = sr[ar];
+      const f32x4 pp = s6[1] + s6[2], qq = s6[1] - s6[2], rr = s6[3] + s6[4], tt = s6[3] - s6[4];
+      f32x4 y4[4];
+      y4[0] = s6[0] + pp + rr;
+      y4[1] = qq + 2.f * tt;
+      y4[2] = pp + 4.f * rr;
+      y4[3] = qq + 8.f * tt + s6[5];
+      f32x4 rup[8];
+      if (hr && a.res_up == 2 && ok) {
+        const float* rb = a.residual + (((long)eb * (g.Ho >> 1) + (oy0 >> 1)) * (g.Wo >> 1) + (ox0 >> 1)) * g.Co + n;
+        rup[0] = 0.25f * *reinterpret_cast<const f32x4*>(rb);
+        rup[1] = 0.25f * *reinterpret_cast<const f32x4*>(rb + g.Co);
+      } else if (hr && a.res_up && ok) {
+        const int Hh = g.Ho >> 1, Wh = g.Wo >> 1, jy = oy0 >> 1, jx = ox0 >> 1;
+        const int y0 = ar ? jy : max(jy - 1, 0), y1 = ar ? min(jy + 1, Hh - 1) : jy;
+        const int xx[4] = {max(jx - 1, 0), jx, jx + 1, min(jx + 2, Wh - 1)};
+        const float* rb = a.residual + ((long)eb * Hh * Wh) * g.Co + n;
+#pragma unroll
+        for (int q = 0; q < 4; ++q) {
+          rup[q] = *reinterpret_cast<const f32x4*>(rb + ((long)y0 * Wh + xx[q]) * g.Co);
+          rup[4 + q] = *reinterpret_cast<const f32x4*>(rb + ((long)y1 * Wh + xx[q]) * g.Co);
+        }
+      }
+#pragma unroll
+      for (int bc = 0; bc < 4; ++bc) {
+        const int soff = ar * rowb + bc * pixb;
+        f32x4 y = y4[bc] * scv + bv;
+        if (hr) {
+          f32x4 r;
+          if (a.res_up == 2) {
+            r = rup[bc >> 1];
+          } else if (a.res_up) {
+            const int c0 = bc == 0 ? 0 : (bc == 3 ? 2 : 1);
+            const float wy0 = ar ? 0.75f : 0.25f, wx0 = (bc & 1) ? 0.75f : 0.25f, wy1 = 1.f - wy0, wx1 = 1.f - wx0;
+            const f32x4 top = wx0 * rup[c0] + wx1 * rup[c0 + 1];
+            const f32x4 bot = wx0 * rup[4 + c0] + wx1 * rup[4 + c0 + 1];
+            r = wy0 * top + wy1 * bot;
+          } else {
+            r = __builtin_bit_cast(f32x4, __builtin_amdgcn_raw_buffer_load_b128(rsrc, voff, soff, 0));
+#pragma unroll
+            for (int e = 0; e < 4; ++e) r[e] = fmaxf(r[e], rfloor);
+          }
+          y += r;
+        }
+        if (hm) {
+          const f32x4 mk = __builtin_bit_cast(f32x4, __builtin_amdgcn_raw_buffer_load_b128(msrc, voff, soff, 0));
+#pragma unroll
+          for (int e = 0; e < 4; ++e) y[e] = mk[e] > 0.f ? y[e] : y[e] * a.mask_slope;
+        }
+        __builtin_amdgcn_raw_buffer_store_b128(__builtin_bit_cast(__attribute__((ext_vector_type(4))) unsigned, y), ysrc, voff, soff, 0);
+        if (hs && ok) {
+          cs1[p] += y;
+          cs2[p] += y * y;
+        }
+      }
+    }
+    __syncthreads();
+  }
+  if (hs) {
+    float* red = smem;
+#pragma unroll
+    for (int p = 0; p < 2; ++p) {
+#pragma unroll
+      for (int e = 0; e < 4; ++e) {
+        float v1 = cs1[p][e], v2 = cs2[p][e];
+        v1 += __shfl_xor(v1, 1, 64);
+        v2 += __shfl_xor(v2, 1, 64);
+        v1 += __shfl_xor(v1, 32, 64);
+        v2 += __shfl_xor(v2, 32, 64);
+        cs1[p][e] = v1;
+        cs2[p][e] = v2;
+      }
+      if ((lane & 0x21) == 0) {
+        *reinterpret_cast<f32x4*>(red + ((wave * 2 + p) * 2 + 0) * 64 + eq * 4) = cs1[p];
+        *reinterpret_cast<f32x4*>(red + ((wave * 2 + p) * 2 + 1) * 64 + eq * 4) = cs2[p];
+      }
+    }
+    __syncthreads();
+    const int grp16 = tile / tiles_n, row = grp16 >> 1, half = grp16 & 1;
+    float* const slab = a.slab + ((long)row * tiles_n + nb) * 2048;
+    const __amdgpu_buffer_rsrc_t wsrc = __builtin_amdgcn_make_buffer_rsrc(slab, 0, 2048 * 4, 0x00020000);
+#pragma unroll
+    for (int r = 0; r < 2; ++r) {
+      const int i = tid + 512 * r, q = i >> 8, which = (i >> 7) & 1, col = i & 127, p = col >> 6, c64 = col & 63;
+      const float v = red[(((2 * q) * 2 + p) * 2 + which) * 64 + c64] + red[(((2 * q + 1) * 2 + p) * 2 + which) * 64 + c64];
+      __builtin_amdgcn_raw_buffer_store_b32(__float_as_uint(v), wsrc, (unsigned)(half * 1024 + i) * 4u, 0, 16);
+    }
+    asm volatile("s_waitcnt vmcnt(0)" ::: "memory");
+    __syncthreads();
+    if (tid == 0) {
+      const int need = (2 * row + 1) * W4NT < MT ? 2 : 1;
+      const int tk = __hip_atomic_fetch_add(a.tickets + (long)row * tiles_n + nb, 1, __ATOMIC_RELAXED, __HIP_MEMORY_SCOPE_AGENT);
+      const int last = tk == need - 1 ? 1 : 0;
+      if (last) {
+        __builtin_amdgcn_fence(__ATOMIC_ACQUIRE, "agent");
+        asm volatile("s_waitcnt vmcnt(0)" ::: "memory");
+      }
+      reinterpret_cast<volatile int*>(smem)[4096] = last;
+    }
+    __syncthreads();
+    if (reinterpret_cast<volatile int*>(smem)[4096] && tid < 256) {
+      const int which = tid >> 7, col = tid & 127, nh2 = (2 * row + 1) * W4NT < MT ? 2 : 1;
+      float t = 0.f;
+      for (int h = 0; h < nh2; ++h)
+#pragma unroll
+        for (int q = 0; q < 4; ++q) t += slab[h * 1024 + (q * 2 + which) * 128 + col];
+      a.stat_partials[(long)row * 2 * g.Co + which * g.Co + n0 + col] = t;
+    }
+  }
+#ifdef DIAGAN_W4_STAMP
+  if (a.stamps && lane == 0) a.stamps[((size_t)blockIdx.x * 8 + wave) * 16 + 15] = __builtin_amdgcn_s_memtime() - t_epi;
+#endif
+}
+
 template <int PRO, int MODE = 0, bool X3 = false, int LEFT = 0>
 static int launch_wino4_pro(const ConvGemmArgs& a, const float* ug, hipStream_t st) {
   const int MT = a.g.B * (a.g.Ho >> 2) * (a.g.Wo >> 2);
@@ -1147,6 +1655,65 @@
 static bool wino4_x3_ok(const ConvGemmArgs& a) {
   const int nk = a.g.Ci / W4K, ks = a.ksplit > 0 ? a.ksplit : 1;
   return wino4_get_x3() > 0 && (a.g.Ci % 32) == 0 && nk % ks == 0 && (nk / ks) % 4 == 0;
+}
+
+static int g_wino4n = -1;
+void wino4_set_n128(int mode) { g_wino4n = mode; }
+int wino4_get_n128() {
+  static const int env = getenv("DIAGAN_WINO4_N128") ? atoi(getenv("DIAGAN_WINO4_N128")) : 1;
+  return g_wino4n >= 0 ? g_wino4n : env;
+}
+static thread_local int g_wino4n_last = 0;
+int wino4_last_n128() { return g_wino4n_last; }
+bool wino4_n128_takes(int Ci, int Co, int ks, bool x3) {
+  return wino4_get_n128() > 0 && !x3 && ks == 1 && Co % W4NN == 0 && Ci % W4NK == 0 && Ci >= W4NK && (2 * W4N_VSTAGE + 2 * Ci) <= W4N_XCH;
+}
+static long wino4n_stat_floats(const ConvGemmArgs& a) {
+  const long rows = cdiv(a.g.B * (a.g.Ho >> 2) * (a.g.Wo >> 2), 2 * W4NT) * (a.g.Co / W4NN);
+  return rows * 2049;
+}
+static thread_local long g_w4n_ws_floats = 0;
+void wino4_note_ws(long floats) { g_w4n_ws_floats = floats; }
+static bool wino4n_launch_ok(const ConvGemmArgs& a, bool x3) {
+  return wino4_n128_takes(a.g.Ci, a.g.Co, a.ksplit, x3) &&
+         (!a.stat_partials || (long)a.g.Co * a.g.Ci * 36 + wino4n_stat_floats(a) <= g_w4n_ws_floats);
+}
+
+template <int PRO, int MODE>
+static int launch_wino4n_pro(const ConvGemmArgs& a, const float* ug, hipStream_t st) {
+  const int MT = a.g.B * (a.g.Ho >> 2) * (a.g.Wo >> 2);
+  const int wgs = cdiv(MT, W4NT) * (a.g.Co / W4NN);
+  constexpr bool affine = PRO == PRO_AFFINE_RELU || PRO == PRO_AFFINE;
+  const size_t lds = (size_t)max(W4N_XCH, 2 * W4N_VSTAGE + (affine ? 2 * a.g.Ci : 0)) * sizeof(float);
+  auto kern = conv_wino4n_kernel<PRO, MODE>;
+  if (a.stat_partials) DG_HIP(hipMemsetAsync(a.tickets, 0, (size_t)cdiv(MT, 2 * W4NT) * (a.g.Co / W4NN) * sizeof(int), st));
+  static FuncAttrLatch latch;
+  DG_LDS(latch, kern, lds);
+  hipLaunchKernelGGL(kern, dim3(wgs), dim3(512), lds, st, a, ug);
+  return check_launch("conv_wino4n");
+}
+template <int MODE>
+static int launch_wino4n(ConvGemmArgs a, float* ws, int flip, float scale, hipStream_t st) {
+  const ConvGeom& g = a.g;
+  const long floats = (long)g.Co * g.Ci * 36;
+  if (a.stat_partials) {
+    const long rows = cdiv(g.B * (g.Ho >> 2) * (g.Wo >> 2), 2 * W4NT) * (g.Co / W4NN);
+    a.slab = ws + floats;
+    a.tickets = reinterpret_cast<int*>(ws + floats + rows * 2048);
+  }
+  const float* ug = wino_weights_ready(WK_F4N, flip, scale, floats);
+  if (!ug) {
+    hipLaunchKernelGGL(wino4n_weight_kernel, dim3(cdiv(g.Ci, 32), g.Co / 64), dim3(512), 0, st, a.w, ws, g.Co, g.Ci, g.Kp, flip, scale);
+    ug = ws;
+  }
+  g_wino4n_last = 1;
+  switch (a.pro_mode) {
+    case PRO_NONE: return launch_wino4n_pro<PRO_NONE, MODE>(a, ug, st);
+    case PRO_RELU: return launch_wino4n_pro<PRO_RELU, MODE>(a, ug, st);
+    case PRO_AFFINE_RELU: return launch_wino4n_pro<PRO_AFFINE_RELU, MODE>(a, ug, st);
+    case PRO_LRELU: return launch_wino4n_pro<PRO_LRELU, MODE>(a, ug, st);
+    default: return launch_wino4n_pro<PRO_AFFINE, MODE>(a, ug, st);
+  }
 }
 
 template <int WM>
@@ -1193,6 +1760,8 @@
   const ConvGeom& g = a.g;
   a.dWo = make_fastdiv((unsigned)(g.Wo >> 2));
   a.dHo = make_fastdiv((unsigned)(g.Ho >> 2));
+  g_wino4n_last = 0;
+  if (wino4n_launch_ok(a, wino4_x3_ok(a))) return launch_wino4n<0>(a, ws, g.dr < 0 ? 1 : 0, 1.f, st);
   const long f32 = (long)cdiv(g.Co, W4N) * W4N * g.Ci * 36;
   if (wino4_x3_ok(a)) {
     const float* ug = wino4_weights<0>(a, ws, g.dr < 0 ? 1 : 0, 1.f, f32 + f32 / 2, st, true);
@@ -1260,6 +1829,8 @@
   const ConvGeom& g = a.g;
   a.dWo = make_fastdiv((unsigned)(g.Wo >> 2));
   a.dHo = make_fastdiv((unsigned)(g.Ho >> 2));
+  g_wino4n_last = 0;
+  if (wino4n_launch_ok(a, wino4_x3_ok(a))) return launch_wino4n<3>(a, ws, 0, 0.0625f, st);
   const long f32 = (long)cdiv(g.Co, W4N) * W4N * g.Ci * 36;
   if (wino4_x3_ok(a)) {
     const float* ug = wino4_weights<0>(a, ws, 0, 0.0625f, f32 + f32 / 2, st, true);
diff --git a/self-diagnosing-gan_amd/csrc/wino_weights.h b/self-diagnosing-gan_amd/csrc/wino_weights.h
--- a/self-diagnosing-gan_amd/csrc/wino_weights.h
+++ b/self-diagnosing-gan_amd/csrc/wino_weights.h
@@ -178,4 +178,42 @@
 }
 
 
-}
+typedef float f32x2 __attribute__((ext_vector_type(2)));
+constexpr int W4N_U_FLOATS = 8 * 36 * 256;
+__device__ __forceinline__ void wino4n_weight_body(const float* __restrict__ w, float* __restrict__ ug, int Co, int Ci, int Kp, int flip,
+                                                   float wscale, int bx, int by, f32x4* __restrict__ sg) {
+  f32x4 g[3][3];
+  if (!wino_stage_taps(w, by * 64, bx * 32, Co, Ci, Kp, flip, sg, g)) return;
+  if (wscale != 1.f) {
+#pragma unroll
+    for (int t = 0; t < 9; ++t) g[t / 3][t % 3] *= wscale;
+  }
+  const int col = threadIdx.x & 63, c = bx * 32 + (threadIdx.x >> 6) * 4;
+  constexpr float k4 = 0.25f, k6 = 1.f / 6.f, k12 = 1.f / 12.f, k24 = 1.f / 24.f;
+  auto gt = [&](const f32x4& g0, const f32x4& g1, const f32x4& g2, f32x4* o) {
+    o[0] = k4 * g0;
+    o[1] = -k6 * (g0 + g1 + g2);
+    o[2] = -k6 * (g0 - g1 + g2);
+    o[3] = k24 * g0 + k12 * g1 + k6 * g2;
+    o[4] = k24 * g0 - k12 * g1 + k6 * g2;
+    o[5] = g2;
+  };
+  f32x4 t[3][6];
+#pragma unroll
+  for (int s = 0; s < 3; ++s) gt(g[0][s], g[1][s], g[2][s], t[s]);
+  const int nk = Ci >> 4, ks = c >> 4, kq = (c >> 2) & 3, nh = by & 1, n16 = col >> 4, n = col & 15;
+  float* base = ug + ((long)(by >> 1) * nk + ks) * W4N_U_FLOATS + ((kq & 1) * 16 + n) * 4 + 2 * (kq >> 1);
+#pragma unroll
+  for (int i = 0; i < 6; ++i) {
+    f32x4 u[6];
+    gt(t[0][i], t[1][i], t[2][i], u);
+#pragma unroll
+    for (int j = 0; j < 6; ++j) {
+      const int unit = (((i / 3) * 2 + j / 3) * 2 + nh) * 36 + ((i % 3) * 3 + j % 3) * 4 + n16;
+      *reinterpret_cast<f32x2*>(base + unit * 256) = f32x2{u[j][0], u[j][2]};
+      *reinterpret_cast<f32x2*>(base + unit * 256 + 128) = f32x2{u[j][1], u[j][3]};
+    }
+  }
+}
+
+}
diff --git a/self-diagnosing-gan_amd/diagan/ops/conv.py b/self-diagnosing-gan_amd/diagan/ops/conv.py
--- a/self-diagnosing-gan_amd/diagan/ops/conv.py
+++ b/self-diagnosing-gan_amd/diagan/ops/conv.py
@@ -27,6 +27,9 @@
 nat.register("diagan_conv_wgrad_batch_class", [I] * 14)
 nat.register("diagan_conv_gemm_set_wino4x", [I])
 nat.register("diagan_conv_gemm_get_wino4x", [])
+nat.register("diagan_conv_gemm_set_wino4n", [I])
+nat.register("diagan_conv_gemm_get_wino4n", [])
+nat.register("diagan_conv_gemm_last_wino4n", [])
 nat.register("diagan_conv_wino4_pool_used", [I] * 5 + [I64])
 nat.register("diagan_conv_wino4_upin_supported", [I] * 13 + [I64, I])
 nat.register("diagan_conv_gemm_weights_hint", [P, I, I, F])
@@ -218,6 +221,10 @@
 
 def set_winograd4x(mode):
     nat.call("diagan_conv_gemm_set_wino4x", -1 if mode is None else (1 if mode else 0))
+
+
+def set_winograd4n(mode):
+    nat.call("diagan_conv_gemm_set_wino4n", -1 if mode is None else (1 if mode else 0))
 
 
 def set_winograd4(mode):
```

After: 5462, median of 6. 2.6% higher.
